# muyeon-jo/POI_recommendation_models

Hardware: NVIDIA B200
Metric: fullrank_eval_users_per_sec (higher is better)
Workload: dtype f16+e5m2-corrections/f32-accum

## Files before the change

include/nais_b200.h:

```cpp
#ifndef NAIS_B200_H_
#define NAIS_B200_H_

#include <stddef.h>
#include <stdint.h>

#ifdef __cplusplus
extern "C" {
#endif

#define NAIS_ABI_VERSION 2

#if defined(__GNUC__)
#define NAIS_API __attribute__((visibility("default")))
#else
#define NAIS_API
#endif

#define NAIS_DIST_NONE 0
#define NAIS_DIST_LATLON 1
#define NAIS_DIST_KM 2

#define NAIS_PREC_FP32 0
#define NAIS_PREC_TC_SPLIT 1
#define NAIS_PREC_TC_FAST 2
#define NAIS_PREC_TC_MIX 3
#define NAIS_PREC_TC_AUTO 4
#define NAIS_PREC_MASK 0xff
#define NAIS_PREC_FLAG_GENERIC 0x100
#define NAIS_PREC_FLAG_ONE_CTA 0x200

#define NAIS_PAIRS_AUTO 0
#define NAIS_PAIRS_FP32 1
#define NAIS_PAIRS_TC 2

#define NAIS_ERR_NULL -1
#define NAIS_ERR_SHAPE -2
#define NAIS_ERR_ALIGN -3
#define NAIS_ERR_WORKSPACE -4
#define NAIS_ERR_MODE -5
#define NAIS_ERR_ARCH -6
#define NAIS_ERR_INDEX -7

typedef void* nais_stream_t;

typedef struct NaisBranch {
  const float* hist_poi;
  const float* tgt_poi;
  const float* hist_reg;
  const float* tgt_reg;
  const float* w1;
  const float* b1;
  const float* w2;
  int32_t w_poi;
  int32_t w_reg;
} NaisBranch;

typedef struct NaisParams {
  NaisBranch branch[2];
  int32_t n_branch;
  int32_t hid;
  int32_t item_num;
  int32_t region_num;
  int32_t dist_mode;
  float dist_scale;
  const float* dist_w;
  const float* dist_b;
  const float* dist_embed;
  int32_t dist_buckets;
  float dist_bucket_km;
  float beta;
  float dropout_p;
  uint64_t dropout_seed;
  int32_t pairs_precision;
  int32_t reserved0;
} NaisParams;

typedef struct NaisPairs {
  const int64_t* hist;
  const int64_t* tgt;
  const int64_t* hreg;
  const int64_t* treg;
  const float* aux;
  int64_t B;
  int32_t H;
  int32_t n_seg;
  const int64_t* seg_offsets;
  const int64_t* row_offsets;
  const int64_t* seg_cell_offsets;
  const int32_t* tile_seg;
  const int64_t* tile_row0;
  int64_t n_tiles;
  int64_t n_cells;
  const float* hist_coords;
  const float* tgt_coords;
  float center_lat;
  float center_lon;
} NaisPairs;

typedef struct NaisGrads {
  float* hist_poi[2];
  float* tgt_poi[2];
  float* reg[2];
  float* w1[2];
  float* b1[2];
  float* w2[2];
  float* dist_w;
  float* dist_b;
  float* dist_embed;
  const int32_t* remap_hist_poi[2];
  const int32_t* remap_tgt_poi[2];
  const int32_t* remap_reg[2];
} NaisGrads;

typedef struct NaisCatalog {
  const int32_t* region;
  const float* coords;
  int64_t row_base;
  int64_t n_rows;
  float center_lat;
  float center_lon;
} NaisCatalog;

typedef struct NaisUsers {
  const int64_t* offsets;
  const int32_t* items;
  const int32_t* region;
  const float* coords;
  int32_t n_users;
} NaisUsers;

NAIS_API int nais_abi_version(void);
NAIS_API const char* nais_strerror(int code);
NAIS_API uint64_t nais_launch_count(void);

NAIS_API int nais_pairs_dispatch(const NaisParams* p, const NaisPairs* batch, int32_t* fwd_tc, int32_t* bwd_tc);

NAIS_API int nais_pairs_forward(const NaisParams* p, const NaisPairs* batch, float* score, float* row_sum, float* score_parts,
                       uint64_t* act_mask, nais_stream_t stream);

NAIS_API size_t nais_pairs_backward_workspace_bytes(const NaisParams* p, const NaisPairs* batch);
NAIS_API int nais_pairs_backward(const NaisParams* p, const NaisPairs* batch, const float* score_parts, const float* row_sum,
                        const uint64_t* act_mask, const float* dscore, const NaisGrads* grads, void* workspace,
                        size_t workspace_bytes, nais_stream_t stream);

NAIS_API int nais_pairs_forward_presort(const NaisParams* p, const NaisPairs* batch, const NaisGrads* grads, float* score,
                               float* row_sum, float* score_parts, uint64_t* act_mask, void* bwd_workspace,
                               size_t bwd_workspace_bytes, nais_stream_t stream);
NAIS_API int nais_pairs_backward_presorted(const NaisParams* p, const NaisPairs* batch, const float* score_parts, const float* row_sum,
                                  const uint64_t* act_mask, const float* dscore, const NaisGrads* grads, void* workspace,
                                  size_t workspace_bytes, nais_stream_t stream);

NAIS_API size_t nais_rows_adagrad_workspace_bytes(int64_t n, int32_t w);
NAIS_API int nais_rows_adagrad(const int32_t* keys, const float* rows, int64_t n, int32_t w, int32_t n_rows, float* grad_out,
                               float* param, float* sum, float lr, float eps, void* workspace, size_t workspace_bytes,
                               nais_stream_t stream);

NAIS_API int nais_sample_batch(const int64_t* seg_offsets, const int64_t* hist, int32_t n_seg, const int64_t* row_offsets,
                               int32_t num_ng, int32_t item_num, const int32_t* poi_region, const float* poi_coords, uint64_t seed,
                               int32_t max_hist, int64_t* tgt, float* label, int64_t* treg, float* tgt_coords, nais_stream_t stream);

typedef struct NaisAdagrad {
  float lr, eps;
  float* sum_hist_poi[2];
  float* sum_tgt_poi[2];
  float* sum_reg[2];
} NaisAdagrad;
NAIS_API int nais_pairs_backward_adagrad(const NaisParams* p, const NaisPairs* batch, const float* score_parts,
                                const float* row_sum, const uint64_t* act_mask, const float* dscore, const NaisGrads* grads,
                                const NaisAdagrad* opt, void* workspace, size_t workspace_bytes, nais_stream_t stream);

typedef struct NaisDenseAdagrad {
  float lr, eps;
  float* sum_w1;
  float* sum_b1;
  float* sum_w2;
  float* sum_dist_w;
  float* sum_dist_b;
  float* sum_region_w1;
  float* sum_region_b1;
  float* sum_region_w2;
  float* sum_dist_embed;
} NaisDenseAdagrad;
NAIS_API size_t nais_pairs_train_step_workspace_bytes(const NaisParams* p, const NaisPairs* batch);
NAIS_API int nais_pairs_train_step(const NaisParams* p, const NaisPairs* batch, const float* label, const float* row_weight,
                                   const NaisAdagrad* tables, const NaisDenseAdagrad* dense, float* loss, float* score,
                                   void* workspace, size_t workspace_bytes, nais_stream_t stream);

NAIS_API size_t nais_train_users_workspace_bytes(const NaisParams* p, int32_t max_hist, int32_t num_ng);
NAIS_API int nais_train_users(const NaisParams* p, const int64_t* host_indptr, int64_t n_rows, const int64_t* indices, const int64_t* entry_region,
                              const float* entry_coords, const int32_t* poi_region, const float* poi_coords, const int64_t* host_users,
                              int32_t n_users, int32_t num_ng, uint64_t seed, const NaisAdagrad* tables, const NaisDenseAdagrad* dense,
                              float* losses, void* workspace, size_t workspace_bytes, nais_stream_t stream);
NAIS_API int nais_train_users_centred(const NaisParams* p, const int64_t* host_indptr, int64_t n_rows, const int64_t* indices,
                                      const int64_t* entry_region, const float* entry_coords, const int32_t* poi_region,
                                      const float* poi_coords, const int64_t* host_users, int32_t n_users, int32_t num_ng, uint64_t seed,
                                      const NaisAdagrad* tables, const NaisDenseAdagrad* dense, float* losses, void* workspace,
                                      size_t workspace_bytes, float center_lat, float center_lon, nais_stream_t stream);
NAIS_API int nais_train_users_dropout(const NaisParams* p, const int64_t* host_indptr, int64_t n_rows, const int64_t* indices,
                                      const int64_t* entry_region, const float* entry_coords, const int32_t* poi_region,
                                      const float* poi_coords, const int64_t* host_users, int32_t n_users, int32_t num_ng, uint64_t seed,
                                      const NaisAdagrad* tables, const NaisDenseAdagrad* dense, float* losses, void* workspace,
                                      size_t workspace_bytes, float center_lat, float center_lon, const uint64_t* host_dropout_seeds,
                                      nais_stream_t stream);

NAIS_API size_t nais_fullrank_workspace_bytes(const NaisParams* p, int32_t n_users, int64_t nnz, int64_t poi_begin,
                                     int64_t poi_end, int32_t k, int32_t precision);
NAIS_API int nais_fullrank_topk(const NaisParams* p, const NaisCatalog* cat, const NaisUsers* users, int64_t poi_begin,
                       int64_t poi_end, int32_t k, int32_t exclude_history, int32_t precision, float* out_score, int32_t* out_id, void* workspace, size_t workspace_bytes,
                       nais_stream_t stream);

NAIS_API size_t nais_fullrank_plan_bytes(const NaisParams* p, int64_t poi_begin, int64_t poi_end, int32_t precision);
NAIS_API int nais_fullrank_prepare(const NaisParams* p, const NaisCatalog* cat, int64_t poi_begin, int64_t poi_end,
                                   int32_t precision, void* plan, size_t plan_bytes, nais_stream_t stream);
NAIS_API size_t nais_fullrank_planned_workspace_bytes(const NaisParams* p, int32_t n_users, int64_t nnz, int64_t poi_begin,
                                                      int64_t poi_end, int32_t k, int32_t precision);
NAIS_API int nais_fullrank_topk_planned(const NaisParams* p, const NaisCatalog* cat, const NaisUsers* users, int64_t poi_begin,
                                        int64_t poi_end, int32_t k, int32_t exclude_history, int32_t precision, const void* plan,
                                        size_t plan_bytes, uint64_t* out_keys, float* out_score, int32_t* out_id, void* workspace,
                                        size_t workspace_bytes, nais_stream_t stream);

NAIS_API int nais_topk_merge_keys(const uint64_t* in_keys, int64_t user_stride, int64_t list_stride, int32_t n_users,
                                  int32_t n_lists, int32_t k, uint64_t* out_keys, float* out_score, int32_t* out_id,
                                  nais_stream_t stream);

NAIS_API int nais_poll_bad_index(int32_t* host_flag, nais_stream_t stream);

NAIS_API int nais_topk_merge(const float* in_score, const int32_t* in_id, int32_t n_users, int32_t n_lists, int32_t k,
                    float* out_score, int32_t* out_id, nais_stream_t stream);

NAIS_API int nais_hits_at_k(const int32_t* rec, int32_t n_users, int32_t k_rec, const int64_t* pos_offsets,
                            const int32_t* pos_items, const int32_t* k_list, int32_t n_k, int32_t* hits,
                            nais_stream_t stream);

NAIS_API int nais_powerlaw_logscore(const NaisCatalog* cat, const NaisUsers* users, int64_t poi_begin, int64_t poi_end, float a,
                           float b, float* out_logg, nais_stream_t stream);

typedef struct NaisGeoMix {
  float a, b, alpha;
  const float* user_logmax;
} NaisGeoMix;
NAIS_API int nais_powerlaw_logmax(const NaisCatalog* cat, const NaisUsers* users, int64_t poi_begin, int64_t poi_end, float a,
                                  float b, int32_t exclude_history, float* out_logmax, nais_stream_t stream);
NAIS_API int nais_fullrank_topk_geo_planned(const NaisParams* p, const NaisCatalog* cat, const NaisUsers* users, int64_t poi_begin,
                                            int64_t poi_end, int32_t k, int32_t exclude_history, int32_t precision, const void* plan,
                                            size_t plan_bytes, const NaisGeoMix* geo, uint64_t* out_keys, float* out_score,
                                            int32_t* out_id, void* workspace, size_t workspace_bytes, nais_stream_t stream);

NAIS_API int nais_fullrank_scores(const NaisParams* p, const NaisCatalog* cat, const NaisUsers* users, int64_t poi_begin,
                         int64_t poi_end, int32_t precision, float* all_scores, void* workspace,
                         size_t workspace_bytes, nais_stream_t stream);

#ifdef __cplusplus
}
#endif
#endif
```

poi_recommendation_models_b200/_lib.py:

```python
from __future__ import annotations

import ctypes as C
import os

HERE = os.path.dirname(os.path.abspath(__file__))
LIB_PATH = os.path.join(HERE, "libnais_b200.so")

DIST_NONE, DIST_LATLON, DIST_KM = 0, 1, 2
PREC_FP32, PREC_TC_SPLIT, PREC_TC_FAST, PREC_TC_MIX, PREC_TC_AUTO = 0, 1, 2, 3, 4
PREC_FLAG_GENERIC = 0x100
PRECISIONS = {"fp32": PREC_FP32, "tc_split": PREC_TC_SPLIT, "tc_fast": PREC_TC_FAST, "tc_mix": PREC_TC_MIX,
              "tc_auto": PREC_TC_AUTO}
PREC_FLAG_ONE_CTA = 0x200
PRECISIONS.update({k + "_generic": v | PREC_FLAG_GENERIC for k, v in list(PRECISIONS.items()) if k != "fp32"})
PRECISIONS.update({k + "_onecta": v | PREC_FLAG_ONE_CTA for k, v in list(PRECISIONS.items()) if k in ("tc_auto", "tc_split", "tc_mix")})
PAIRS_PRECISIONS = {"auto": 0, "fp32": 1, "tc": 2}
ERR_INDEX = -7

ABI_VERSION = 2
c_float_p = C.c_void_p


class NaisBranch(C.Structure):
    _fields_ = [("hist_poi", C.c_void_p), ("tgt_poi", C.c_void_p), ("hist_reg", C.c_void_p), ("tgt_reg", C.c_void_p),
                ("w1", C.c_void_p), ("b1", C.c_void_p), ("w2", C.c_void_p), ("w_poi", C.c_int32), ("w_reg", C.c_int32)]


class NaisParams(C.Structure):
    _fields_ = [("branch", NaisBranch * 2), ("n_branch", C.c_int32), ("hid", C.c_int32), ("item_num", C.c_int32),
                ("region_num", C.c_int32), ("dist_mode", C.c_int32), ("dist_scale", C.c_float), ("dist_w", C.c_void_p),
                ("dist_b", C.c_void_p), ("dist_embed", C.c_void_p), ("dist_buckets", C.c_int32),
                ("dist_bucket_km", C.c_float), ("beta", C.c_float), ("dropout_p", C.c_float),
                ("dropout_seed", C.c_uint64), ("pairs_precision", C.c_int32), ("reserved0", C.c_int32)]


class NaisPairs(C.Structure):
    _fields_ = [("hist", C.c_void_p), ("tgt", C.c_void_p), ("hreg", C.c_void_p), ("treg", C.c_void_p),
                ("aux", C.c_void_p), ("B", C.c_int64), ("H", C.c_int32), ("n_seg", C.c_int32), ("seg_offsets", C.c_void_p),
                ("row_offsets", C.c_void_p), ("seg_cell_offsets", C.c_void_p), ("tile_seg", C.c_void_p), ("tile_row0", C.c_void_p),
                ("n_tiles", C.c_int64), ("n_cells", C.c_int64), ("hist_coords", C.c_void_p), ("tgt_coords", C.c_void_p),
                ("center_lat", C.c_float), ("center_lon", C.c_float)]


class NaisGrads(C.Structure):
    _fields_ = [("hist_poi", C.c_void_p * 2), ("tgt_poi", C.c_void_p * 2), ("reg", C.c_void_p * 2),
                ("w1", C.c_void_p * 2), ("b1", C.c_void_p * 2), ("w2", C.c_void_p * 2), ("dist_w", C.c_void_p),
                ("dist_b", C.c_void_p), ("dist_embed", C.c_void_p), ("remap_hist_poi", C.c_void_p * 2),
                ("remap_tgt_poi", C.c_void_p * 2), ("remap_reg", C.c_void_p * 2)]


class NaisAdagrad(C.Structure):
    _fields_ = [("lr", C.c_float), ("eps", C.c_float), ("sum_hist_poi", C.c_void_p * 2), ("sum_tgt_poi", C.c_void_p * 2),
                ("sum_reg", C.c_void_p * 2)]


class NaisDenseAdagrad(C.Structure):
    _fields_ = [("lr", C.c_float), ("eps", C.c_float), ("sum_w1", C.c_void_p), ("sum_b1", C.c_void_p), ("sum_w2", C.c_void_p),
                ("sum_dist_w", C.c_void_p), ("sum_dist_b", C.c_void_p), ("sum_region_w1", C.c_void_p), ("sum_region_b1", C.c_void_p),
                ("sum_region_w2", C.c_void_p), ("sum_dist_embed", C.c_void_p)]


class NaisCatalog(C.Structure):
    _fields_ = [("region", C.c_void_p), ("coords", C.c_void_p), ("row_base", C.c_int64), ("n_rows", C.c_int64),
                ("center_lat", C.c_float), ("center_lon", C.c_float)]


class NaisUsers(C.Structure):
    _fields_ = [("offsets", C.c_void_p), ("items", C.c_void_p), ("region", C.c_void_p), ("coords", C.c_void_p),
                ("n_users", C.c_int32)]


class NaisGeoMix(C.Structure):
    _fields_ = [("a", C.c_float), ("b", C.c_float), ("alpha", C.c_float), ("user_logmax", C.c_void_p)]


SYMBOLS = {
    "nais_abi_version": (C.c_int, []),
    "nais_strerror": (C.c_char_p, [C.c_int]),
    "nais_launch_count": (C.c_uint64, []),
    "nais_pairs_dispatch": (C.c_int, [C.POINTER(NaisParams), C.POINTER(NaisPairs), C.POINTER(C.c_int32), C.POINTER(C.c_int32)]),
    "nais_pairs_forward": (C.c_int, [C.POINTER(NaisParams), C.POINTER(NaisPairs), C.c_void_p, C.c_void_p, C.c_void_p,
                                     C.c_void_p, C.c_void_p]),
    "nais_pairs_backward_workspace_bytes": (C.c_size_t, [C.POINTER(NaisParams), C.POINTER(NaisPairs)]),
    "nais_pairs_train_step_workspace_bytes": (C.c_size_t, [C.POINTER(NaisParams), C.POINTER(NaisPairs)]),
    "nais_pairs_train_step": (C.c_int, [C.POINTER(NaisParams), C.POINTER(NaisPairs), C.c_void_p, C.c_void_p, C.POINTER(NaisAdagrad),
                                        C.POINTER(NaisDenseAdagrad), C.c_void_p, C.c_void_p, C.c_void_p, C.c_size_t, C.c_void_p]),
    "nais_train_users_workspace_bytes": (C.c_size_t, [C.POINTER(NaisParams), C.c_int32, C.c_int32]),
    "nais_train_users": (C.c_int, [C.POINTER(NaisParams), C.c_void_p, C.c_int64, C.c_void_p, C.c_void_p, C.c_void_p, C.c_void_p, C.c_void_p,
                                   C.c_void_p, C.c_int32, C.c_int32, C.c_uint64, C.POINTER(NaisAdagrad), C.POINTER(NaisDenseAdagrad),
                                   C.c_void_p, C.c_void_p, C.c_size_t, C.c_void_p]),
    "nais_train_users_centred": (C.c_int, [C.POINTER(NaisParams), C.c_void_p, C.c_int64, C.c_void_p, C.c_void_p, C.c_void_p, C.c_void_p,
                                           C.c_void_p, C.c_void_p, C.c_int32, C.c_int32, C.c_uint64, C.POINTER(NaisAdagrad),
                                           C.POINTER(NaisDenseAdagrad), C.c_void_p, C.c_void_p, C.c_size_t, C.c_float, C.c_float,
                                           C.c_void_p]),
    "nais_train_users_dropout": (C.c_int, [C.POINTER(NaisParams), C.c_void_p, C.c_int64, C.c_void_p, C.c_void_p, C.c_void_p, C.c_void_p,
                                           C.c_void_p, C.c_void_p, C.c_int32, C.c_int32, C.c_uint64, C.POINTER(NaisAdagrad),
                                           C.POINTER(NaisDenseAdagrad), C.c_void_p, C.c_void_p, C.c_size_t, C.c_float, C.c_float,
                                           C.c_void_p, C.c_void_p]),
    "nais_rows_adagrad_workspace_bytes": (C.c_size_t, [C.c_int64, C.c_int32]),
    "nais_rows_adagrad": (C.c_int, [C.c_void_p, C.c_void_p, C.c_int64, C.c_int32, C.c_int32, C.c_void_p, C.c_void_p, C.c_void_p,
                                    C.c_float, C.c_float, C.c_void_p, C.c_size_t, C.c_void_p]),
    "nais_sample_batch": (C.c_int, [C.c_void_p, C.c_void_p, C.c_int32, C.c_void_p, C.c_int32, C.c_int32, C.c_void_p, C.c_void_p,
                                    C.c_uint64, C.c_int32, C.c_void_p, C.c_void_p, C.c_void_p, C.c_void_p, C.c_void_p]),
    "nais_pairs_backward": (C.c_int, [C.POINTER(NaisParams), C.POINTER(NaisPairs), C.c_void_p, C.c_void_p, C.c_void_p, C.c_void_p,
                                      C.POINTER(NaisGrads), C.c_void_p, C.c_size_t, C.c_void_p]),
    "nais_pairs_forward_presort": (C.c_int, [C.POINTER(NaisParams), C.POINTER(NaisPairs), C.POINTER(NaisGrads), C.c_void_p, C.c_void_p,
                                             C.c_void_p, C.c_void_p, C.c_void_p, C.c_size_t, C.c_void_p]),
    "nais_pairs_backward_presorted": (C.c_int, [C.POINTER(NaisParams), C.POINTER(NaisPairs), C.c_void_p, C.c_void_p, C.c_void_p,
                                                C.c_void_p, C.POINTER(NaisGrads), C.c_void_p, C.c_size_t, C.c_void_p]),
    "nais_pairs_backward_adagrad": (C.c_int, [C.POINTER(NaisParams), C.POINTER(NaisPairs), C.c_void_p, C.c_void_p, C.c_void_p,
                                              C.c_void_p, C.POINTER(NaisGrads), C.POINTER(NaisAdagrad), C.c_void_p, C.c_size_t,
                                              C.c_void_p]),
    "nais_powerlaw_logscore": (C.c_int, [C.POINTER(NaisCatalog), C.POINTER(NaisUsers), C.c_int64, C.c_int64, C.c_float, C.c_float,
                                         C.c_void_p, C.c_void_p]),
    "nais_fullrank_workspace_bytes": (C.c_size_t, [C.POINTER(NaisParams), C.c_int32, C.c_int64, C.c_int64, C.c_int64,
                                                   C.c_int32, C.c_int32]),
    "nais_fullrank_topk": (C.c_int, [C.POINTER(NaisParams), C.POINTER(NaisCatalog), C.POINTER(NaisUsers), C.c_int64,
                                     C.c_int64, C.c_int32, C.c_int32, C.c_int32, C.c_void_p, C.c_void_p, C.c_void_p,
                                     C.c_size_t, C.c_void_p]),
    "nais_fullrank_scores": (C.c_int, [C.POINTER(NaisParams), C.POINTER(NaisCatalog), C.POINTER(NaisUsers), C.c_int64,
                                       C.c_int64, C.c_int32, C.c_void_p, C.c_void_p, C.c_size_t, C.c_void_p]),
    "nais_hits_at_k": (C.c_int, [C.c_void_p, C.c_int32, C.c_int32, C.c_void_p, C.c_void_p, C.c_void_p, C.c_int32, C.c_void_p,
                                 C.c_void_p]),
    "nais_topk_merge": (C.c_int, [C.c_void_p, C.c_void_p, C.c_int32, C.c_int32, C.c_int32, C.c_void_p, C.c_void_p,
                                  C.c_void_p]),
    "nais_fullrank_plan_bytes": (C.c_size_t, [C.POINTER(NaisParams), C.c_int64, C.c_int64, C.c_int32]),
    "nais_fullrank_prepare": (C.c_int, [C.POINTER(NaisParams), C.POINTER(NaisCatalog), C.c_int64, C.c_int64, C.c_int32,
                                        C.c_void_p, C.c_size_t, C.c_void_p]),
    "nais_fullrank_planned_workspace_bytes": (C.c_size_t, [C.POINTER(NaisParams), C.c_int32, C.c_int64, C.c_int64, C.c_int64,
                                                           C.c_int32, C.c_int32]),
    "nais_fullrank_topk_planned": (C.c_int, [C.POINTER(NaisParams), C.POINTER(NaisCatalog), C.POINTER(NaisUsers), C.c_int64,
                                             C.c_int64, C.c_int32, C.c_int32, C.c_int32, C.c_void_p, C.c_size_t, C.c_void_p,
                                             C.c_void_p, C.c_void_p, C.c_void_p, C.c_size_t, C.c_void_p]),
    "nais_powerlaw_logmax": (C.c_int, [C.POINTER(NaisCatalog), C.POINTER(NaisUsers), C.c_int64, C.c_int64, C.c_float, C.c_float,
                                       C.c_int32, C.c_void_p, C.c_void_p]),
    "nais_fullrank_topk_geo_planned": (C.c_int, [C.POINTER(NaisParams), C.POINTER(NaisCatalog), C.POINTER(NaisUsers), C.c_int64,
                                                 C.c_int64, C.c_int32, C.c_int32, C.c_int32, C.c_void_p, C.c_size_t,
                                                 C.POINTER(NaisGeoMix), C.c_void_p, C.c_void_p, C.c_void_p, C.c_void_p, C.c_size_t,
                                                 C.c_void_p]),
    "nais_topk_merge_keys": (C.c_int, [C.c_void_p, C.c_int64, C.c_int64, C.c_int32, C.c_int32, C.c_int32, C.c_void_p,
                                       C.c_void_p, C.c_void_p, C.c_void_p]),
    "nais_poll_bad_index": (C.c_int, [C.c_void_p, C.c_void_p]),
}

_lib = None


def load() -> C.CDLL:
    global _lib
    if _lib is not None:
        return _lib
    if not os.path.isfile(LIB_PATH):
        raise RuntimeError(f"{LIB_PATH} is missing: build it with `python poi_recommendation_models_b200/build_ext.py` "
                           "(nvcc, sm_100a).  There is no CPU / PyTorch fallback for the NAIS ops.")
    lib = C.CDLL(LIB_PATH)
    for name, (res, args) in SYMBOLS.items():
        fn = getattr(lib, name)
        fn.restype = res
        fn.argtypes = args
    if lib.nais_abi_version() != ABI_VERSION:
        raise RuntimeError("libnais_b200.so ABI version mismatch; rebuild")
    _lib = lib
    return lib


def check(rc: int, what: str) -> None:
    if rc != 0:
        msg = load().nais_strerror(rc).decode()
        raise RuntimeError(f"{what} failed ({rc}): {msg}")
```

poi_recommendation_models_b200/csrc/nais_capi.cu:

```cuda
#include <cstdio>

#include <cstring>
#include <mutex>

#include "nais_common.cuh"
#include "nais_pairs_tile.cuh"

namespace nais {
int launch_pairs_fwd(const NaisParams& p, const NaisPairs& b, float* score, float* row_sum, float* parts, cudaStream_t stream);
int launch_fullrank_fp32(const NaisParams& p, const NaisCatalog& cat, const NaisUsers& users, int64_t poi_begin,
                         int64_t poi_end, int k, int exclude, float* out_score, int32_t* out_id, float* all_scores,
                         void* ws, size_t ws_bytes, cudaStream_t stream, const GeoMixArgs* geo = nullptr);
int launch_topk_merge(const unsigned long long* in_keys, const float* in_score, const int32_t* in_id, int n_users,
                      int n_lists, int k, float* out_score, int32_t* out_id, cudaStream_t stream);
int launch_topk_merge_keys_multi(const unsigned long long* keys, unsigned long long* scratch, int64_t user_stride, int64_t list_stride,
                                 int n_users, int n_lists, int k, unsigned long long* out_keys, float* out_score, int32_t* out_id,
                                 cudaStream_t stream);
int merge_scratch_lists(int n_lists, int k);
int choose_splits(int n_users, int64_t range);
size_t pairs_bwd_workspace_bytes(const NaisParams& p, const NaisPairs& b);
int launch_pairs_bwd(const NaisParams& p, const NaisPairs& b, const float* score_parts, const float* row_sum,
                     const unsigned long long* act_mask, const float* dscore, const NaisGrads& g, const NaisAdagrad* opt, void* ws,
                     size_t ws_bytes, cudaStream_t stream, BwdPhase phase = BWD_ALL, const DenseAdagradLaunch* dense = nullptr);
bool pairs_tc_bwd_supported(const NaisParams& p, const NaisPairs& b);
size_t rows_adagrad_workspace_bytes(int64_t n, int w);
int launch_rows_adagrad(const int32_t* keys, const float* rows, int64_t n, int w, int n_rows, float* grad_out, float* param, float* sum,
                        float lr, float eps, void* ws, size_t ws_bytes, cudaStream_t stream);
size_t fullrank_tc_workspace_bytes(const NaisParams& p, int n_users, int64_t nnz, int64_t poi_begin, int64_t poi_end, int k,
                                   int precision);
int launch_fullrank_tc(const NaisParams& p, const NaisCatalog& cat, const NaisUsers& users, int64_t poi_begin,
                       int64_t poi_end, int k, int exclude, int precision, float* out_score, int32_t* out_id,
                       float* all_scores, void* ws, size_t ws_bytes, cudaStream_t stream);
bool tc_supported(const NaisParams& p, int precision);
size_t fullrank_tc_plan_bytes(const NaisParams& p, int64_t poi_begin, int64_t poi_end, int precision);
size_t fullrank_tc_call_workspace_bytes(const NaisParams& p, int n_users, int64_t nnz, int64_t poi_begin, int64_t poi_end, int k,
                                        int precision);
int fullrank_tc_prepare(const NaisParams& p, const NaisCatalog& cat, int64_t poi_begin, int64_t poi_end, int precision, void* plan,
                        size_t plan_bytes, cudaStream_t stream);
int fullrank_tc_run(const NaisParams& p, const NaisCatalog& cat, const NaisUsers& users, int64_t poi_begin, int64_t poi_end, int k,
                    int exclude, int precision, const void* plan, size_t plan_bytes, unsigned long long* out_keys, float* out_score,
                    int32_t* out_id, float* all_scores, void* ws, size_t ws_bytes, cudaStream_t stream,
                    const GeoMixArgs* geo = nullptr);
int launch_sample_batch(const int64_t* seg_offsets, const int64_t* hist, int n_seg, const int64_t* row_offsets, int num_ng, int item_num,
                        const int32_t* poi_region, const float* poi_coords, uint64_t seed, int max_hist, int64_t* tgt, float* label,
                        int64_t* treg, float* tgt_coords, cudaStream_t stream);
bool pairs_tc_supported(const NaisParams& p, const NaisPairs& b);
int launch_bce_dscore(const float* score, const float* label, const float* row_weight, int64_t B, float* dscore, float* loss,
                      cudaStream_t stream);
int launch_dense_adagrad(float* const* param, float* const* sum, const float* const* grad, const int* n, float lr, float eps,
                         cudaStream_t stream);
int launch_pairs_fwd_tc(const NaisParams& p, const NaisPairs& b, float* score, float* row_sum, float* parts,
                        unsigned long long* act_mask, cudaStream_t stream);
}

namespace nais {
unsigned long long g_launches = 0;
__device__ int g_bad_index = 0;
int* bad_index_flag() {
  int* ptr = nullptr;
  cudaGetSymbolAddress(reinterpret_cast<void**>(&ptr), g_bad_index);
  return ptr;
}
}
using namespace nais;

static bool aligned16(const void* p) { return (reinterpret_cast<uintptr_t>(p) & 15u) == 0; }

static int check_params(const NaisParams* p) {
  if (!p) return NAIS_ERR_NULL;
  if (p->n_branch < 1 || p->n_branch > 2) return NAIS_ERR_SHAPE;
  if (p->hid < 1 || p->hid > 1024 || p->item_num < 1) return NAIS_ERR_SHAPE;
  if (p->dist_mode < NAIS_DIST_NONE || p->dist_mode > NAIS_DIST_KM) return NAIS_ERR_MODE;
  for (int i = 0; i < p->n_branch; ++i) {
    const NaisBranch& b = p->branch[i];
    const int D = b.w_poi + b.w_reg;
    if (b.w_poi < 0 || b.w_reg < 0 || D < 4 || D > MAXD || (D & 3)) return NAIS_ERR_SHAPE;
    if (b.w_poi && (!b.hist_poi || !b.tgt_poi)) return NAIS_ERR_NULL;
    if (b.w_reg && (!b.hist_reg || !b.tgt_reg || p->region_num < 1)) return NAIS_ERR_NULL;
    if (!b.w1 || !b.b1 || !b.w2) return NAIS_ERR_NULL;
  }
  if (p->dist_mode == NAIS_DIST_LATLON && (!p->dist_w || !p->dist_b)) return NAIS_ERR_NULL;
  if (p->dist_mode == NAIS_DIST_KM && (!p->dist_embed || p->dist_buckets < 1)) return NAIS_ERR_NULL;
  if (p->dist_mode == NAIS_DIST_KM && p->dist_buckets != 1) return NAIS_ERR_MODE;
  if (p->pairs_precision < NAIS_PAIRS_AUTO || p->pairs_precision > NAIS_PAIRS_TC) return NAIS_ERR_MODE;
  return 0;
}

static int check_pairs(const NaisParams* p, const NaisPairs* b) {
  if (!b) return NAIS_ERR_NULL;
  const bool seg = b->seg_offsets != nullptr;
  if (b->B < 0 || (!seg && b->H < 1)) return NAIS_ERR_SHAPE;
  if (b->B == 0) return 0;
  if (!b->hist || !b->tgt) return NAIS_ERR_NULL;
  bool need_reg = false;
  for (int i = 0; i < p->n_branch; ++i) need_reg |= p->branch[i].w_reg > 0;
  if (need_reg && (!b->hreg || !b->treg)) return NAIS_ERR_NULL;
  if (seg) {
    if (b->n_seg < 1 || b->n_tiles < 0 || b->n_cells < 0) return NAIS_ERR_SHAPE;
    if (!b->row_offsets || !b->seg_cell_offsets || (b->n_tiles && (!b->tile_seg || !b->tile_row0))) return NAIS_ERR_NULL;
    if (b->aux) return NAIS_ERR_MODE;
    if (p->dropout_p > 0.f && p->n_branch != 1) return NAIS_ERR_MODE;
    if (p->dist_mode != NAIS_DIST_NONE && (!b->hist_coords || !b->tgt_coords)) return NAIS_ERR_NULL;
    return 0;
  }
  if (p->dist_mode != NAIS_DIST_NONE && !b->aux) return NAIS_ERR_NULL;
  return 0;
}

static size_t fp32_workspace_bytes(int n_users, int64_t poi_begin, int64_t poi_end, int k) {
  const int s = choose_splits(n_users, poi_end - poi_begin);
  return 1024 + (size_t)n_users * 8 + (s > 1 ? (size_t)n_users * s * k * sizeof(unsigned long long) : 0);
}

__global__ void pack_keys_kernel(const float* __restrict__ s, const int32_t* __restrict__ id, size_t n, unsigned long long* keys) {
  const size_t i = blockIdx.x * (size_t)blockDim.x + threadIdx.x;
  if (i < n) keys[i] = id[i] >= 0 ? make_key(s[i], id[i]) : 0ull;
}

__global__ void fill_empty_topk_kernel(float* s, int32_t* id, size_t n) {
  const size_t i = blockIdx.x * (size_t)blockDim.x + threadIdx.x;
  if (i < n) {
    s[i] = -INFINITY;
    id[i] = -1;
  }
}

template <bool kHist>
__device__ __forceinline__ float powerlaw_logg_block(const NaisCatalog& cat, const NaisUsers& users, int u, int64_t j, bool valid,
                                                     float ln_a, float b, bool* in_hist) {
  __shared__ float s_la[256], s_lo[256], s_cos[256];
  __shared__ int s_id[kHist ? 256 : 1];
  const int64_t hb = users.offsets[u];
  const int H = (int)(users.offsets[u + 1] - hb);
  float cla = 0.f, clo = 0.f, ccos = 1.f;
  if (valid) {
    cla = __ldg(cat.coords + 2 * (j - cat.row_base));
    clo = __ldg(cat.coords + 2 * (j - cat.row_base) + 1);
    ccos = cosf((cat.center_lat + cla) * 0.017453292519943295f);
  }
  float acc = 0.f;
  bool seen = false;
  for (int h0 = 0; h0 < H; h0 += 256) {
    __syncthreads();
    if (h0 + (int)threadIdx.x < H) {
      const float la = __ldg(users.coords + 2 * (hb + h0 + threadIdx.x)), lo = __ldg(users.coords + 2 * (hb + h0 + threadIdx.x) + 1);
      s_la[threadIdx.x] = la;
      s_lo[threadIdx.x] = lo;
      s_cos[threadIdx.x] = cosf((cat.center_lat + la) * 0.017453292519943295f);
      if constexpr (kHist) s_id[threadIdx.x] = __ldg(users.items + hb + h0 + threadIdx.x);
    }
    __syncthreads();
    const int n = min(256, H - h0);
    for (int i = 0; i < n; ++i) {
      acc += powerlaw_log_term(dist_km_f(cla, clo, s_la[i], s_lo[i], ccos, s_cos[i]), ln_a, b);
      if constexpr (kHist) seen = seen || (int64_t)s_id[i] == j;
    }
  }
  if (in_hist) *in_hist = seen;
  return acc;
}

__global__ void powerlaw_logscore_kernel(NaisCatalog cat, NaisUsers users, int64_t poi_begin, int64_t poi_end, float ln_a, float b,
                                         float* __restrict__ out) {
  const int u = blockIdx.x;
  const int64_t j = poi_begin + (int64_t)blockIdx.y * blockDim.x + threadIdx.x;
  const bool valid = j < poi_end;
  const float acc = powerlaw_logg_block<false>(cat, users, u, j, valid, ln_a, b, nullptr);
  if (valid) out[(size_t)u * (poi_end - poi_begin) + (j - poi_begin)] = acc;
}

__device__ __forceinline__ void atomic_max_float(float* addr, float v) {
  if (v != v) return;
  if (__float_as_int(v) >= 0) atomicMax(reinterpret_cast<int*>(addr), __float_as_int(v));
  else atomicMin(reinterpret_cast<unsigned*>(addr), __float_as_uint(v));
}

__global__ void fill_float_kernel(float* out, int n, float v) {
  const int i = blockIdx.x * blockDim.x + threadIdx.x;
  if (i < n) out[i] = v;
}

__global__ void powerlaw_logmax_kernel(NaisCatalog cat, NaisUsers users, int64_t poi_begin, int64_t poi_end, float ln_a, float b,
                                       int exclude, float* __restrict__ out) {
  __shared__ float s_max[8];
  const int u = blockIdx.x;
  float m = -INFINITY;
  for (int64_t j0 = poi_begin + (int64_t)blockIdx.y * blockDim.x; j0 < poi_end; j0 += (int64_t)gridDim.y * blockDim.x) {
    const int64_t j = j0 + threadIdx.x;
    const bool valid = j < poi_end;
    bool in_hist = false;
    const float acc = exclude ? powerlaw_logg_block<true>(cat, users, u, j, valid, ln_a, b, &in_hist)
                              : powerlaw_logg_block<false>(cat, users, u, j, valid, ln_a, b, nullptr);
    if (valid && !in_hist) m = fmaxf(m, acc);
  }
#pragma unroll
  for (int o = 16; o > 0; o >>= 1) m = fmaxf(m, __shfl_xor_sync(0xffffffffu, m, o));
  if ((threadIdx.x & 31) == 0) s_max[threadIdx.x >> 5] = m;
  __syncthreads();
  if (threadIdx.x == 0) {
    for (int w = 1; w < (int)(blockDim.x >> 5); ++w) m = fmaxf(m, s_max[w]);
    if (m > -INFINITY) atomic_max_float(out + u, m);
  }
}

__global__ void hits_at_k_kernel(const int32_t* __restrict__ rec, int n_users, int k_rec, const int64_t* __restrict__ po,
                                 const int32_t* __restrict__ pi, const int32_t* __restrict__ k_list, int n_k, int32_t* hits) {
  const int u = (blockIdx.x * blockDim.x + threadIdx.x) >> 5, lane = threadIdx.x & 31;
  if (u >= n_users) return;
  const int64_t p0 = po[u], p1 = po[u + 1];
  for (int ki = 0; ki < n_k; ++ki) {
    const int k = min(k_list[ki], k_rec);
    int cnt = 0;
    for (int r = lane; r < k; r += 32) {
      const int id = rec[(size_t)u * k_rec + r];
      if (id < 0) continue;
      bool dup = false;
      for (int q = 0; q < r && !dup; ++q) dup = rec[(size_t)u * k_rec + q] == id;
      if (dup) continue;
      bool hit = false;
      for (int64_t q = p0; q < p1 && !hit; ++q) hit = pi[q] == id;
      cnt += hit ? 1 : 0;
    }
#pragma unroll
    for (int o = 16; o > 0; o >>= 1) cnt += __shfl_xor_sync(0xffffffffu, cnt, o);
    if (lane == 0) hits[(size_t)u * n_k + ki] = cnt;
  }
}

extern "C" {

int nais_abi_version(void) { return NAIS_ABI_VERSION; }
uint64_t nais_launch_count(void) { return __atomic_load_n(&nais::g_launches, __ATOMIC_RELAXED); }

const char* nais_strerror(int code) {
  switch (code) {
    case 0: return "ok";
    case NAIS_ERR_NULL: return "nais: required pointer is NULL";
    case NAIS_ERR_SHAPE: return "nais: unsupported or inconsistent dimension";
    case NAIS_ERR_ALIGN: return "nais: pointer or row width not 16-byte aligned";
    case NAIS_ERR_WORKSPACE: return "nais: workspace too small";
    case NAIS_ERR_MODE: return "nais: unknown mode or unsupported flag combination";
    case NAIS_ERR_ARCH: return "nais: tensor path needs an sm_100 device";
    case NAIS_ERR_INDEX: return "nais: index out of range in a POI / region id tensor";
    default: break;
  }
  if (code > 0) return cudaGetErrorString(static_cast<cudaError_t>(code));
  return "nais: unknown error";
}

static bool device_is_sm100() {
  return device_info().major == 10;
}

static int choose_pairs_fwd(const NaisParams& p, const NaisPairs& b, bool* tc) {
  const bool tc_ok = pairs_tc_supported(p, b) && device_is_sm100();
  if (p.pairs_precision == NAIS_PAIRS_TC && !tc_ok) return NAIS_ERR_SHAPE;
  *tc = p.pairs_precision != NAIS_PAIRS_FP32 && tc_ok;
  return 0;
}

static int launch_chosen_fwd(bool tc, const NaisParams& p, const NaisPairs& b, float* score, float* row_sum, float* parts,
                             unsigned long long* act_mask, cudaStream_t stream) {
  return tc ? launch_pairs_fwd_tc(p, b, score, row_sum, parts, act_mask, stream) : launch_pairs_fwd(p, b, score, row_sum, parts, stream);
}

size_t nais_rows_adagrad_workspace_bytes(int64_t n, int32_t w) {
  if (n < 0 || w < 1 || w > 128) return 0;
  return rows_adagrad_workspace_bytes(n, w);
}

int nais_rows_adagrad(const int32_t* keys, const float* rows, int64_t n, int32_t w, int32_t n_rows, float* grad_out, float* param,
                      float* sum, float lr, float eps, void* workspace, size_t workspace_bytes, nais_stream_t stream) {
  if (n < 0 || w < 1 || w > 128 || n_rows < 1) return NAIS_ERR_SHAPE;
  if (n == 0) return 0;
  if (!keys || !rows || !workspace || (sum ? !param : !grad_out)) return NAIS_ERR_NULL;
  if (sum && (!(lr >= 0.f) || !(eps >= 0.f))) return NAIS_ERR_MODE;
  if (!aligned16(workspace)) return NAIS_ERR_ALIGN;
  return launch_rows_adagrad(keys, rows, n, w, n_rows, grad_out, param, sum, lr, eps, workspace, workspace_bytes,
                             static_cast<cudaStream_t>(stream));
}

int nais_sample_batch(const int64_t* seg_offsets, const int64_t* hist, int32_t n_seg, const int64_t* row_offsets, int32_t num_ng,
                      int32_t item_num, const int32_t* poi_region, const float* poi_coords, uint64_t seed, int32_t max_hist,
                      int64_t* tgt, float* label, int64_t* treg, float* tgt_coords, nais_stream_t stream) {
  if (n_seg < 0 || num_ng < 0 || item_num < 1 || max_hist < 0) return NAIS_ERR_SHAPE;
  if (n_seg == 0) return 0;
  if (!seg_offsets || !hist || !row_offsets || !tgt || !label) return NAIS_ERR_NULL;
  if ((treg && !poi_region) || (tgt_coords && !poi_coords)) return NAIS_ERR_NULL;
  if ((int64_t)max_hist * (num_ng + 1) >= item_num) return NAIS_ERR_SHAPE;
  return launch_sample_batch(seg_offsets, hist, n_seg, row_offsets, num_ng, item_num, poi_region, poi_coords, seed, max_hist, tgt,
                             label, treg, tgt_coords, static_cast<cudaStream_t>(stream));
}

int nais_pairs_dispatch(const NaisParams* p, const NaisPairs* batch, int32_t* fwd_tc, int32_t* bwd_tc) {
  int rc = check_params(p);
  if (rc) return rc;
  if (!batch || !fwd_tc || !bwd_tc) return NAIS_ERR_NULL;
  if (batch->B < 0 || (!batch->seg_offsets && batch->H < 1)) return NAIS_ERR_SHAPE;
  NaisPairs b = *batch;
  if (b.B == 0) b.B = 1;
  bool f_tc = false;
  rc = choose_pairs_fwd(*p, b, &f_tc);
  if (rc) return rc;
  *fwd_tc = f_tc ? 1 : 0;
  *bwd_tc = (p->pairs_precision != NAIS_PAIRS_FP32 && pairs_tc_bwd_supported(*p, b)) ? 1 : 0;
  return 0;
}

int nais_pairs_forward(const NaisParams* p, const NaisPairs* batch, float* score, float* row_sum, float* score_parts,
                       uint64_t* act_mask, nais_stream_t stream) {
  int rc = check_params(p);
  if (rc) return rc;
  rc = check_pairs(p, batch);
  if (rc) return rc;
  if (batch->B && !score) return NAIS_ERR_NULL;
  if (batch->B == 0) return 0;
  bool tc = false;
  rc = choose_pairs_fwd(*p, *batch, &tc);
  if (rc) return rc;
  return launch_chosen_fwd(tc, *p, *batch, score, row_sum, score_parts, reinterpret_cast<unsigned long long*>(act_mask),
                           static_cast<cudaStream_t>(stream));
}

size_t nais_pairs_backward_workspace_bytes(const NaisParams* p, const NaisPairs* batch) {
  if (check_params(p) || !batch || batch->B < 0 || (!batch->seg_offsets && batch->H < 1)) return 0;
  return pairs_bwd_workspace_bytes(*p, *batch);
}

int nais_pairs_backward(const NaisParams* p, const NaisPairs* batch, const float* score_parts, const float* row_sum,
                        const uint64_t* act_mask, const float* dscore, const NaisGrads* grads, void* workspace,
                        size_t workspace_bytes, nais_stream_t stream) {
  int rc = check_params(p);
  if (rc) return rc;
  rc = check_pairs(p, batch);
  if (rc) return rc;
  if (!grads) return NAIS_ERR_NULL;
  if (batch->B == 0) return 0;
  if (!score_parts || !row_sum || !dscore || !workspace) return NAIS_ERR_NULL;
  if (!aligned16(workspace)) return NAIS_ERR_ALIGN;
  if (workspace_bytes < pairs_bwd_workspace_bytes(*p, *batch)) return NAIS_ERR_WORKSPACE;
  return launch_pairs_bwd(*p, *batch, score_parts, row_sum, reinterpret_cast<const unsigned long long*>(act_mask), dscore, *grads,
                          nullptr, workspace, workspace_bytes, static_cast<cudaStream_t>(stream));
}

int nais_pairs_forward_presort(const NaisParams* p, const NaisPairs* batch, const NaisGrads* grads, float* score, float* row_sum,
                               float* score_parts, uint64_t* act_mask, void* bwd_workspace, size_t bwd_workspace_bytes,
                               nais_stream_t stream) {
  int rc = check_params(p);
  if (rc) return rc;
  rc = check_pairs(p, batch);
  if (rc) return rc;
  if (!grads) return NAIS_ERR_NULL;
  if (p->n_branch != 1) return NAIS_ERR_MODE;
  if (batch->B && !score) return NAIS_ERR_NULL;
  if (batch->B == 0) return 0;
  if (!bwd_workspace) return NAIS_ERR_NULL;
  if (!aligned16(bwd_workspace)) return NAIS_ERR_ALIGN;
  if (bwd_workspace_bytes < pairs_bwd_workspace_bytes(*p, *batch)) return NAIS_ERR_WORKSPACE;
  bool tc = false;
  rc = choose_pairs_fwd(*p, *batch, &tc);
  if (rc) return rc;
  cudaStream_t st = static_cast<cudaStream_t>(stream);
  rc = launch_pairs_bwd(*p, *batch, nullptr, nullptr, nullptr, nullptr, *grads, nullptr, bwd_workspace, bwd_workspace_bytes, st, BWD_SORTS);
  if (rc) return rc;
  rc = launch_chosen_fwd(tc, *p, *batch, score, row_sum, score_parts, reinterpret_cast<unsigned long long*>(act_mask), st);
  const int rj = launch_pairs_bwd(*p, *batch, nullptr, nullptr, nullptr, nullptr, *grads, nullptr, bwd_workspace, bwd_workspace_bytes, st,
                                  BWD_JOIN_SORTS);
  return rc ? rc : rj;
}

int nais_pairs_backward_presorted(const NaisParams* p, const NaisPairs* batch, const float* score_parts, const float* row_sum,
                                  const uint64_t* act_mask, const float* dscore, const NaisGrads* grads, void* workspace,
                                  size_t workspace_bytes, nais_stream_t stream) {
  int rc = check_params(p);
  if (rc) return rc;
  rc = check_pairs(p, batch);
  if (rc) return rc;
  if (!grads) return NAIS_ERR_NULL;
  if (p->n_branch != 1) return NAIS_ERR_MODE;
  if (batch->B == 0) return 0;
  if (!score_parts || !row_sum || !dscore || !workspace) return NAIS_ERR_NULL;
  if (!aligned16(workspace)) return NAIS_ERR_ALIGN;
  if (workspace_bytes < pairs_bwd_workspace_bytes(*p, *batch)) return NAIS_ERR_WORKSPACE;
  return launch_pairs_bwd(*p, *batch, score_parts, row_sum, reinterpret_cast<const unsigned long long*>(act_mask), dscore, *grads,
                          nullptr, workspace, workspace_bytes, static_cast<cudaStream_t>(stream), BWD_AFTER_JOIN);
}

int nais_pairs_backward_adagrad(const NaisParams* p, const NaisPairs* batch, const float* score_parts, const float* row_sum,
                                const uint64_t* act_mask, const float* dscore, const NaisGrads* grads, const NaisAdagrad* opt,
                                void* workspace, size_t workspace_bytes, nais_stream_t stream) {
  int rc = check_params(p);
  if (rc) return rc;
  rc = check_pairs(p, batch);
  if (rc) return rc;
  if (!grads || !opt) return NAIS_ERR_NULL;
  if (!pairs_fused_layout(*p)) return NAIS_ERR_MODE;
  if (!(opt->lr >= 0.f) || !(opt->eps >= 0.f)) return NAIS_ERR_MODE;
  if (batch->B == 0) return 0;
  if (!score_parts || !row_sum || !dscore || !workspace) return NAIS_ERR_NULL;
  if (!aligned16(workspace)) return NAIS_ERR_ALIGN;
  if (workspace_bytes < pairs_bwd_workspace_bytes(*p, *batch)) return NAIS_ERR_WORKSPACE;
  return launch_pairs_bwd(*p, *batch, score_parts, row_sum, reinterpret_cast<const unsigned long long*>(act_mask), dscore, *grads,
                          opt, workspace, workspace_bytes, static_cast<cudaStream_t>(stream));
}

namespace {
inline size_t ts_al(size_t x) { return (x + 255) / 256 * 256; }
struct TrainStepLayout {
  size_t score, row_sum, parts, dscore, mask, gw1[2], gb1[2], gw2[2], gdw, gdb, gde, bwd, total;
};
TrainStepLayout train_step_layout(const NaisParams& p, const NaisPairs& b) {
  TrainStepLayout L;
  const int64_t B = b.B, cells = pairs_n_cells(b);
  const int lanes = p.dist_mode == NAIS_DIST_LATLON ? 2 : 0;
  size_t o = 0;
  L.score = o, o += ts_al((size_t)B * 4);
  L.row_sum = o, o += ts_al((size_t)p.n_branch * B * 4);
  L.parts = o, o += ts_al((size_t)p.n_branch * B * 4);
  L.dscore = o, o += ts_al((size_t)B * 4);
  L.mask = o, o += ts_al((size_t)cells * 8);
  for (int bi = 0; bi < 2; ++bi) {
    const NaisBranch& br = p.branch[bi];
    const int ldw = br.w_poi + br.w_reg + lanes;
    const bool on = bi < p.n_branch;
    L.gw1[bi] = o, o += on ? ts_al((size_t)p.hid * ldw * 4) : 0;
    L.gb1[bi] = o, o += on ? ts_al((size_t)p.hid * 4) : 0;
    L.gw2[bi] = o, o += on ? ts_al((size_t)p.hid * 4) : 0;
  }
  L.gdw = o, o += 256;
  L.gdb = o, o += 256;
  L.gde = o, o += p.dist_mode == NAIS_DIST_KM ? ts_al((size_t)MAXD * 4) : 0;
  L.bwd = o, o += ts_al(pairs_bwd_workspace_bytes(p, b));
  L.total = o;
  return L;
}
}

size_t nais_pairs_train_step_workspace_bytes(const NaisParams* p, const NaisPairs* batch) {
  if (check_params(p) || !batch || batch->B < 0 || (!batch->seg_offsets && batch->H < 1)) return 0;
  if (!pairs_fused_layout(*p)) return 0;
  return train_step_layout(*p, *batch).total;
}

static int check_train_state(const NaisParams* p, const NaisAdagrad* tables, const NaisDenseAdagrad* dense) {
  if (!tables || !dense) return NAIS_ERR_NULL;
  if (!pairs_fused_layout(*p)) return NAIS_ERR_MODE;
  const bool two = pairs_disentangled(*p);
  if (p->n_branch == 1 && p->dist_mode == NAIS_DIST_KM) return NAIS_ERR_MODE;
  if (!(tables->lr >= 0.f) || !(tables->eps >= 0.f) || !(dense->lr >= 0.f) || !(dense->eps >= 0.f)) return NAIS_ERR_MODE;
  if (!dense->sum_w1 || !dense->sum_b1 || !dense->sum_w2) return NAIS_ERR_NULL;
  if (p->dist_mode == NAIS_DIST_LATLON && (!dense->sum_dist_w || !dense->sum_dist_b)) return NAIS_ERR_NULL;
  if (two && (!dense->sum_region_w1 || !dense->sum_region_b1 || !dense->sum_region_w2)) return NAIS_ERR_NULL;
  if (two && p->dist_mode == NAIS_DIST_KM && !dense->sum_dist_embed) return NAIS_ERR_NULL;
  return 0;
}

enum StepPart { STEP_ALL = 0, STEP_SORTS = 1, STEP_AFTER_SORTS = 2 };

static int train_step_impl(const NaisParams* p, const NaisPairs* batch, const float* label, const float* row_weight,
                           const NaisAdagrad* tables, const NaisDenseAdagrad* dense, float* loss, float* score_out, void* workspace,
                           size_t workspace_bytes, cudaStream_t st, StepPart part = STEP_ALL);

int nais_pairs_train_step(const NaisParams* p, const NaisPairs* batch, const float* label, const float* row_weight,
                          const NaisAdagrad* tables, const NaisDenseAdagrad* dense, float* loss, float* score_out, void* workspace,
                          size_t workspace_bytes, nais_stream_t stream) {
  int rc = check_params(p);
  if (rc) return rc;
  rc = check_pairs(p, batch);
  if (rc) return rc;
  if (!loss) return NAIS_ERR_NULL;
  rc = check_train_state(p, tables, dense);
  if (rc) return rc;
  if (batch->B == 0) return 0;
  if (!label || !workspace) return NAIS_ERR_NULL;
  if (!aligned16(workspace)) return NAIS_ERR_ALIGN;
  return train_step_impl(p, batch, label, row_weight, tables, dense, loss, score_out, workspace, workspace_bytes,
                         static_cast<cudaStream_t>(stream));
}

static int train_step_impl(const NaisParams* p, const NaisPairs* batch, const float* label, const float* row_weight,
                           const NaisAdagrad* tables, const NaisDenseAdagrad* dense, float* loss, float* score_out, void* workspace,
                           size_t workspace_bytes, cudaStream_t st, StepPart part) {
  int rc;
  const TrainStepLayout L = train_step_layout(*p, *batch);
  if (workspace_bytes < L.total) return NAIS_ERR_WORKSPACE;
  char* base = reinterpret_cast<char*>(workspace);
  auto F = [&](size_t off) { return reinterpret_cast<float*>(base + off); };
  NaisGrads g;
  memset(&g, 0, sizeof(g));
  for (int bi = 0; bi < p->n_branch; ++bi) {
    g.w1[bi] = F(L.gw1[bi]);
    g.b1[bi] = F(L.gb1[bi]);
    g.w2[bi] = F(L.gw2[bi]);
  }
  if (p->dist_mode == NAIS_DIST_LATLON) {
    g.dist_w = F(L.gdw);
    g.dist_b = F(L.gdb);
  }
  if (p->dist_mode == NAIS_DIST_KM) g.dist_embed = F(L.gde);
  if (part != STEP_AFTER_SORTS) {
    rc = launch_pairs_bwd(*p, *batch, nullptr, nullptr, nullptr, nullptr, g, tables, base + L.bwd, workspace_bytes - L.bwd, st, BWD_SORTS);
    if (rc) return rc;
  }
  if (part == STEP_SORTS)
    return launch_pairs_bwd(*p, *batch, nullptr, nullptr, nullptr, nullptr, g, tables, base + L.bwd, workspace_bytes - L.bwd, st,
                            BWD_JOIN_SORTS);
  bool fwd_tc = false;
  rc = choose_pairs_fwd(*p, *batch, &fwd_tc);
  if (rc) return rc;
  unsigned long long* mask = (fwd_tc && p->hid <= 64) ? reinterpret_cast<unsigned long long*>(base + L.mask) : nullptr;
  rc = launch_chosen_fwd(fwd_tc, *p, *batch, F(L.score), F(L.row_sum), F(L.parts), mask, st);
  if (rc) return rc;
  if (score_out) {
    cudaError_t e = cudaMemcpyAsync(score_out, F(L.score), (size_t)batch->B * 4, cudaMemcpyDeviceToDevice, st);
    if (e != cudaSuccess) return (int)e;
  }
  rc = launch_bce_dscore(F(L.score), label, row_weight, batch->B, F(L.dscore), loss, st);
  if (rc) return rc;
  const NaisBranch& br = p->branch[0];
  const int lanes = p->dist_mode == NAIS_DIST_LATLON ? 2 : 0, ldw = br.w_poi + br.w_reg + lanes;
  DenseAdagradLaunch da[2] = {{{const_cast<float*>(br.w1), const_cast<float*>(br.b1), const_cast<float*>(br.w2),
                                lanes ? const_cast<float*>(p->dist_w) : nullptr, lanes ? const_cast<float*>(p->dist_b) : nullptr},
                               {dense->sum_w1, dense->sum_b1, dense->sum_w2, dense->sum_dist_w, dense->sum_dist_b},
                               {g.w1[0], g.b1[0], g.w2[0], g.dist_w, g.dist_b},
                               {p->hid * ldw, p->hid, p->hid, 4, 2},
                               dense->lr, dense->eps}};
  if (p->n_branch == 2) {
    const NaisBranch& r = p->branch[1];
    const bool km = p->dist_mode == NAIS_DIST_KM;
    da[1] = {{const_cast<float*>(r.w1), const_cast<float*>(r.b1), const_cast<float*>(r.w2), km ? const_cast<float*>(p->dist_embed) : nullptr,
              nullptr},
             {dense->sum_region_w1, dense->sum_region_b1, dense->sum_region_w2, dense->sum_dist_embed, nullptr},
             {g.w1[1], g.b1[1], g.w2[1], g.dist_embed, nullptr},
             {p->hid * (r.w_poi + r.w_reg), p->hid, p->hid, r.w_poi + r.w_reg, 0},
             dense->lr, dense->eps};
  }
  return launch_pairs_bwd(*p, *batch, F(L.parts), F(L.row_sum), mask, F(L.dscore), g, tables, base + L.bwd, workspace_bytes - L.bwd, st,
                          part == STEP_AFTER_SORTS ? BWD_AFTER_JOIN : BWD_AFTER_SORTS, da);
}

namespace {
__global__ void single_segment_kernel(int H, int R, int rpt, int n_tiles, int64_t* seg_offsets, int64_t* row_offsets, int64_t* cell_offsets,
                                      int32_t* tile_seg, int64_t* tile_row0) {
  const int i = blockIdx.x * blockDim.x + threadIdx.x;
  if (i == 0) {
    seg_offsets[0] = 0, seg_offsets[1] = H;
    row_offsets[0] = 0, row_offsets[1] = R;
    cell_offsets[0] = 0, cell_offsets[1] = (int64_t)R * H;
  }
  if (i < n_tiles) {
    tile_seg[i] = 0;
    tile_row0[i] = (int64_t)i * rpt;
  }
}
struct UsersLayout {
  size_t seg, row, cell, tseg, trow, tgt, label, treg, tco, step, total;
};
inline int host_rows_per_tile(int H) {
  int r = H <= 128 ? 128 / (H > 0 ? H : 1) : 1;
  return r > 16 ? 16 : r;
}
NaisPairs max_user_batch(int max_hist, int num_ng) {
  NaisPairs b;
  memset(&b, 0, sizeof(b));
  static const int64_t dummy[2] = {0, 0};
  b.seg_offsets = dummy;
  b.n_seg = 1;
  b.B = (int64_t)max_hist * (num_ng + 1);
  b.n_cells = b.B * max_hist;
  b.n_tiles = b.B;
  return b;
}
UsersLayout users_layout(const NaisParams& p, int max_hist, int num_ng) {
  UsersLayout L;
  const NaisPairs b = max_user_batch(max_hist, num_ng);
  size_t o = 0;
  L.seg = o, o += 256;
  L.row = o, o += 256;
  L.cell = o, o += 256;
  L.tseg = o, o += ts_al((size_t)b.n_tiles * 4);
  L.trow = o, o += ts_al((size_t)b.n_tiles * 8);
  L.tgt = o, o += ts_al((size_t)b.B * 8);
  L.label = o, o += ts_al((size_t)b.B * 4);
  L.treg = o, o += ts_al((size_t)b.B * 8);
  L.tco = o, o += ts_al((size_t)b.B * 8);
  L.step = o, o += train_step_layout(p, b).total;
  L.total = o;
  return L;
}

std::mutex g_prep_mu;
cudaStream_t prep_stream() {
  static cudaStream_t pool[64] = {};
  int dev = 0;
  if (cudaGetDevice(&dev) != cudaSuccess || dev < 0 || dev >= 64) return nullptr;
  std::lock_guard<std::mutex> lock(g_prep_mu);
  if (!pool[dev] && cudaStreamCreateWithFlags(&pool[dev], cudaStreamNonBlocking) != cudaSuccess) pool[dev] = nullptr;
  return pool[dev];
}
}

size_t nais_train_users_workspace_bytes(const NaisParams* p, int32_t max_hist, int32_t num_ng) {
  if (check_params(p) || !pairs_fused_layout(*p) || max_hist < 1 || num_ng < 0) return 0;
  return 2 * users_layout(*p, max_hist, num_ng).total;
}

int nais_train_users(const NaisParams* p, const int64_t* host_indptr, int64_t n_rows, const int64_t* indices, const int64_t* entry_region,
                     const float* entry_coords, const int32_t* poi_region, const float* poi_coords, const int64_t* host_users,
                     int32_t n_users, int32_t num_ng, uint64_t seed, const NaisAdagrad* tables, const NaisDenseAdagrad* dense, float* losses,
                     void* workspace, size_t workspace_bytes, nais_stream_t stream) {
  return nais_train_users_centred(p, host_indptr, n_rows, indices, entry_region, entry_coords, poi_region, poi_coords, host_users, n_users,
                                  num_ng, seed, tables, dense, losses, workspace, workspace_bytes, 0.f, 0.f, stream);
}

int nais_train_users_centred(const NaisParams* p, const int64_t* host_indptr, int64_t n_rows, const int64_t* indices,
                             const int64_t* entry_region, const float* entry_coords, const int32_t* poi_region, const float* poi_coords,
                             const int64_t* host_users, int32_t n_users, int32_t num_ng, uint64_t seed, const NaisAdagrad* tables,
                             const NaisDenseAdagrad* dense, float* losses, void* workspace, size_t workspace_bytes, float center_lat,
                             float center_lon, nais_stream_t stream) {
  if (p && p->dropout_p > 0.f) return NAIS_ERR_MODE;
  return nais_train_users_dropout(p, host_indptr, n_rows, indices, entry_region, entry_coords, poi_region, poi_coords, host_users, n_users,
                                  num_ng, seed, tables, dense, losses, workspace, workspace_bytes, center_lat, center_lon, nullptr, stream);
}

int nais_train_users_dropout(const NaisParams* p, const int64_t* host_indptr, int64_t n_rows, const int64_t* indices,
                             const int64_t* entry_region, const float* entry_coords, const int32_t* poi_region, const float* poi_coords,
                             const int64_t* host_users, int32_t n_users, int32_t num_ng, uint64_t seed, const NaisAdagrad* tables,
                             const NaisDenseAdagrad* dense, float* losses, void* workspace, size_t workspace_bytes, float center_lat,
                             float center_lon, const uint64_t* host_dropout_seeds, nais_stream_t stream) {
  int rc = check_params(p);
  if (rc) return rc;
  rc = check_train_state(p, tables, dense);
  if (rc) return rc;
  if (n_users < 0 || num_ng < 0) return NAIS_ERR_SHAPE;
  if (p->dropout_p > 0.f && !host_dropout_seeds) return NAIS_ERR_NULL;
  if (n_users == 0) return 0;
  if (!host_indptr || !indices || !host_users || !losses || !workspace) return NAIS_ERR_NULL;
  bool need_reg = false;
  for (int i = 0; i < p->n_branch; ++i) need_reg |= p->branch[i].w_reg > 0;
  const bool need_co = p->dist_mode != NAIS_DIST_NONE;
  if ((need_reg && (!entry_region || !poi_region)) || (need_co && (!entry_coords || !poi_coords))) return NAIS_ERR_NULL;
  if (!aligned16(workspace)) return NAIS_ERR_ALIGN;
  int max_hist = 0;
  for (int i = 0; i < n_users; ++i) {
    const int64_t u = host_users[i];
    if (u < 0 || u >= n_rows) return NAIS_ERR_SHAPE;
    const int64_t H = host_indptr[u + 1] - host_indptr[u];
    if (H < 0 || H > 0x7fffffff / (num_ng + 2)) return NAIS_ERR_SHAPE;
    if ((int)H > max_hist) max_hist = (int)H;
  }
  if (max_hist == 0) return (int)cudaMemsetAsync(losses, 0, (size_t)n_users * 4, static_cast<cudaStream_t>(stream));
  if ((int64_t)max_hist * (num_ng + 1) >= p->item_num) return NAIS_ERR_SHAPE;
  const UsersLayout L = users_layout(*p, max_hist, num_ng);
  if (workspace_bytes < 2 * L.total) return NAIS_ERR_WORKSPACE;
  cudaStream_t st = static_cast<cudaStream_t>(stream);
  cudaStream_t ps = prep_stream();
  if (!ps) return (int)cudaErrorUnknown;
  cudaEvent_t prepared[2] = {nullptr, nullptr}, stepped[2] = {nullptr, nullptr}, begin = nullptr;
  bool ev_ok = cudaEventCreateWithFlags(&begin, cudaEventDisableTiming) == cudaSuccess;
  for (int i = 0; i < 2 && ev_ok; ++i)
    ev_ok = cudaEventCreateWithFlags(&prepared[i], cudaEventDisableTiming) == cudaSuccess &&
            cudaEventCreateWithFlags(&stepped[i], cudaEventDisableTiming) == cudaSuccess;
  auto release = [&]() {
    if (begin) cudaEventDestroy(begin);
    for (int i = 0; i < 2; ++i) {
      if (prepared[i]) cudaEventDestroy(prepared[i]);
      if (stepped[i]) cudaEventDestroy(stepped[i]);
    }
  };
  if (!ev_ok) {
    release();
    return (int)cudaErrorUnknown;
  }
  auto bail = [&](int code) {
    if (cudaEventRecord(begin, ps) == cudaSuccess) cudaStreamWaitEvent(st, begin, 0);
    release();
    return code;
  };
  struct UserBatch {
    NaisPairs b;
    const float* label;
    char* step;
  };
  auto buffers = [&](int i, int slot, UserBatch& ub) {
    char* base = reinterpret_cast<char*>(workspace) + (size_t)slot * L.total;
    auto I64 = [&](size_t off) { return reinterpret_cast<int64_t*>(base + off); };
    const int64_t u = host_users[i], a = host_indptr[u];
    const int H = (int)(host_indptr[u + 1] - a);
    const int R = H * (num_ng + 1), rpt = host_rows_per_tile(H), n_tiles = (R + rpt - 1) / rpt;
    NaisPairs& b = ub.b;
    memset(&b, 0, sizeof(b));
    b.hist = indices + a;
    b.tgt = I64(L.tgt);
    b.hreg = need_reg ? entry_region + a : nullptr;
    b.treg = need_reg ? I64(L.treg) : nullptr;
    b.B = R;
    b.n_seg = 1;
    b.seg_offsets = I64(L.seg);
    b.row_offsets = I64(L.row);
    b.seg_cell_offsets = I64(L.cell);
    b.tile_seg = reinterpret_cast<int32_t*>(base + L.tseg);
    b.tile_row0 = I64(L.trow);
    b.n_tiles = n_tiles;
    b.n_cells = (int64_t)R * H;
    b.hist_coords = need_co ? entry_coords + 2 * a : nullptr;
    b.tgt_coords = need_co ? reinterpret_cast<float*>(base + L.tco) : nullptr;
    b.center_lat = center_lat;
    b.center_lon = center_lon;
    ub.label = reinterpret_cast<float*>(base + L.label);
    ub.step = base + L.step;
  };
  auto prepare = [&](int i, int slot) -> int {
    UserBatch ub;
    buffers(i, slot, ub);
    const int64_t u = host_users[i], a = host_indptr[u];
    const int H = (int)(host_indptr[u + 1] - a);
    char* base = reinterpret_cast<char*>(workspace) + (size_t)slot * L.total;
    single_segment_kernel<<<((int)ub.b.n_tiles + 255) / 256, 256, 0, ps>>>(
        H, (int)ub.b.B, host_rows_per_tile(H), (int)ub.b.n_tiles, const_cast<int64_t*>(ub.b.seg_offsets), const_cast<int64_t*>(ub.b.row_offsets),
        const_cast<int64_t*>(ub.b.seg_cell_offsets), const_cast<int32_t*>(ub.b.tile_seg), const_cast<int64_t*>(ub.b.tile_row0));
    NAIS_COUNT_LAUNCH(1);
    int r = launch_sample_batch(ub.b.seg_offsets, indices + a, 1, ub.b.row_offsets, num_ng, p->item_num, need_reg ? poi_region : nullptr,
                                need_co ? poi_coords : nullptr, seed + (uint64_t)u, H, const_cast<int64_t*>(ub.b.tgt),
                                reinterpret_cast<float*>(base + L.label), need_reg ? const_cast<int64_t*>(ub.b.treg) : nullptr,
                                need_co ? const_cast<float*>(ub.b.tgt_coords) : nullptr, ps);
    if (r) return r;
    return train_step_impl(p, &ub.b, ub.label, nullptr, tables, dense, nullptr, nullptr, ub.step, L.total - L.step, ps, STEP_SORTS);
  };
  int next = 0;
  auto advance = [&](int from) {
    while (from < n_users && host_indptr[host_users[from] + 1] == host_indptr[host_users[from]]) ++from;
    return from;
  };
  for (int i = 0; i < n_users; ++i)
    if (host_indptr[host_users[i] + 1] == host_indptr[host_users[i]]) {
      cudaError_t e = cudaMemsetAsync(losses + i, 0, 4, st);
      if (e != cudaSuccess) return bail((int)e);
    }
  if (cudaEventRecord(begin, st) != cudaSuccess || cudaStreamWaitEvent(ps, begin, 0) != cudaSuccess) return bail((int)cudaErrorUnknown);
  next = advance(0);
  int slot = 0;
  if (next < n_users) {
    rc = prepare(next, slot);
    if (rc) return bail(rc);
    cudaEventRecord(prepared[slot], ps);
  }
  int done = 0;
  while (next < n_users) {
    const int cur = next, cur_slot = slot;
    next = advance(cur + 1);
    slot ^= 1;
    if (next < n_users) {
      if (done >= 1) cudaStreamWaitEvent(ps, stepped[slot], 0);
      rc = prepare(next, slot);
      if (rc) return bail(rc);
      cudaEventRecord(prepared[slot], ps);
    }
    UserBatch ub;
    buffers(cur, cur_slot, ub);
    NaisParams pu = *p;
    if (p->dropout_p > 0.f) pu.dropout_seed = host_dropout_seeds[cur];
    cudaStreamWaitEvent(st, prepared[cur_slot], 0);
    rc = train_step_impl(&pu, &ub.b, ub.label, nullptr, tables, dense, losses + cur, nullptr, ub.step, L.total - L.step, st, STEP_AFTER_SORTS);
    if (rc) return bail(rc);
    cudaEventRecord(stepped[cur_slot], st);
    ++done;
  }
  cudaError_t e = cudaGetLastError();
  release();
  return e == cudaSuccess ? 0 : (int)e;
}

static int check_fullrank(const NaisParams* p, const NaisCatalog* cat, const NaisUsers* users, int64_t poi_begin,
                          int64_t poi_end, int precision) {
  int rc = check_params(p);
  if (rc) return rc;
  if (!cat || !users) return NAIS_ERR_NULL;
  if (users->n_users < 0 || poi_begin < 0 || poi_end < poi_begin || poi_end > p->item_num) return NAIS_ERR_SHAPE;
  if (poi_begin < cat->row_base || poi_end > cat->row_base + cat->n_rows) return NAIS_ERR_SHAPE;
  if (users->n_users && (!users->offsets || !users->items)) return NAIS_ERR_NULL;
  bool need_reg = false;
  for (int i = 0; i < p->n_branch; ++i) need_reg |= p->branch[i].w_reg > 0;
  const bool work = users->n_users > 0 && poi_end > poi_begin;
  if (work && need_reg && (!cat->region || !users->region)) return NAIS_ERR_NULL;
  if (work && p->dist_mode != NAIS_DIST_NONE && (!cat->coords || !users->coords)) return NAIS_ERR_NULL;
  const int prec = precision & NAIS_PREC_MASK;
  if (precision & ~(NAIS_PREC_MASK | NAIS_PREC_FLAG_GENERIC | NAIS_PREC_FLAG_ONE_CTA)) return NAIS_ERR_MODE;
  if (prec < NAIS_PREC_FP32 || prec > NAIS_PREC_TC_AUTO) return NAIS_ERR_MODE;
  if (prec != NAIS_PREC_FP32 && !tc_supported(*p, precision)) return NAIS_ERR_SHAPE;
  return 0;
}

size_t nais_fullrank_workspace_bytes(const NaisParams* p, int32_t n_users, int64_t nnz, int64_t poi_begin,
                                     int64_t poi_end, int32_t k, int32_t precision) {
  if (check_params(p) || n_users < 0 || poi_end < poi_begin || k < 1) return 0;
  if ((precision & NAIS_PREC_MASK) != NAIS_PREC_FP32) return fullrank_tc_workspace_bytes(*p, n_users, nnz, poi_begin, poi_end, k, precision);
  return fp32_workspace_bytes(n_users, poi_begin, poi_end, k);
}

size_t nais_fullrank_plan_bytes(const NaisParams* p, int64_t poi_begin, int64_t poi_end, int32_t precision) {
  if (check_params(p) || poi_end < poi_begin || (precision & NAIS_PREC_MASK) == NAIS_PREC_FP32) return 0;
  return fullrank_tc_plan_bytes(*p, poi_begin, poi_end, precision);
}

size_t nais_fullrank_planned_workspace_bytes(const NaisParams* p, int32_t n_users, int64_t nnz, int64_t poi_begin, int64_t poi_end,
                                             int32_t k, int32_t precision) {
  if (check_params(p) || n_users < 0 || poi_end < poi_begin || k < 1) return 0;
  if ((precision & NAIS_PREC_MASK) != NAIS_PREC_FP32)
    return fullrank_tc_call_workspace_bytes(*p, n_users, nnz, poi_begin, poi_end, k, precision) + 1024 + (size_t)n_users * 8;
  return fp32_workspace_bytes(n_users, poi_begin, poi_end, k) + (size_t)n_users * k * 12 + 512;
}

int nais_fullrank_prepare(const NaisParams* p, const NaisCatalog* cat, int64_t poi_begin, int64_t poi_end, int32_t precision,
                          void* plan, size_t plan_bytes, nais_stream_t stream) {
  NaisUsers none = {};
  int rc = check_fullrank(p, cat, &none, poi_begin, poi_end, precision);
  if (rc) return rc;
  if ((precision & NAIS_PREC_MASK) == NAIS_PREC_FP32 || poi_end == poi_begin) return 0;
  if (!plan) return NAIS_ERR_NULL;
  if (!aligned16(plan)) return NAIS_ERR_ALIGN;
  const NaisBranch& br = p->branch[0];
  if (br.w_reg > 0 && !cat->region) return NAIS_ERR_NULL;
  return fullrank_tc_prepare(*p, *cat, poi_begin, poi_end, precision, plan, plan_bytes, static_cast<cudaStream_t>(stream));
}

static int check_geo(const NaisCatalog* cat, const NaisUsers* users, int64_t poi_begin, int64_t poi_end, const NaisGeoMix* geo) {
  if (!geo) return NAIS_ERR_NULL;
  if (!(geo->a > 0.f) || !isfinite(geo->a) || !isfinite(geo->b) || !isfinite(geo->alpha)) return NAIS_ERR_MODE;
  if (users->n_users > 0 && poi_end > poi_begin && (!cat->coords || !users->coords || !geo->user_logmax)) return NAIS_ERR_NULL;
  return 0;
}

static int fullrank_topk_planned_impl(const NaisParams* p, const NaisCatalog* cat, const NaisUsers* users, int64_t poi_begin,
                                      int64_t poi_end, int32_t k, int32_t exclude_history, int32_t precision, const void* plan,
                                      size_t plan_bytes, const NaisGeoMix* geo, uint64_t* out_keys, float* out_score, int32_t* out_id,
                                      void* workspace, size_t workspace_bytes, nais_stream_t stream) {
  int rc = check_fullrank(p, cat, users, poi_begin, poi_end, precision);
  if (rc) return rc;
  if (k < 1 || k > KCAP) return NAIS_ERR_SHAPE;
  if (geo && (rc = check_geo(cat, users, poi_begin, poi_end, geo))) return rc;
  if (users->n_users == 0) return 0;
  if ((!out_score) != (!out_id) || (!out_score && !out_keys) || !workspace) return NAIS_ERR_NULL;
  if (!aligned16(workspace)) return NAIS_ERR_ALIGN;
  GeoMixArgs gm = {};
  if (geo) gm = GeoMixArgs{logf(geo->a), geo->b, geo->alpha, geo->user_logmax};
  const GeoMixArgs* gp = geo ? &gm : nullptr;
  cudaStream_t st = static_cast<cudaStream_t>(stream);
  unsigned long long* keys = reinterpret_cast<unsigned long long*>(out_keys);
  const size_t n = (size_t)users->n_users * k;
  if (poi_end == poi_begin) {
    if (out_score) {
      fill_empty_topk_kernel<<<(unsigned)((n + 255) / 256), 256, 0, st>>>(out_score, out_id, n);
      NAIS_COUNT_LAUNCH(1);
    }
    if (keys) {
      cudaError_t e = cudaMemsetAsync(keys, 0, n * 8, st);
      if (e != cudaSuccess) return (int)e;
    }
    return (int)cudaGetLastError();
  }
  if ((precision & NAIS_PREC_MASK) != NAIS_PREC_FP32)
    return fullrank_tc_run(*p, *cat, *users, poi_begin, poi_end, k, exclude_history, precision, plan, plan_bytes, keys, out_score,
                           out_id, nullptr, workspace, workspace_bytes, st, gp);
  float* sc = out_score;
  int32_t* id = out_id;
  char* rest = reinterpret_cast<char*>(workspace);
  size_t rest_bytes = workspace_bytes;
  if (!sc) {
    const size_t head = (n * 8 + 255) & ~size_t(255);
    if (workspace_bytes < head) return NAIS_ERR_WORKSPACE;
    sc = reinterpret_cast<float*>(workspace);
    id = reinterpret_cast<int32_t*>(sc + n);
    rest += head;
    rest_bytes -= head;
  }
  rc = launch_fullrank_fp32(*p, *cat, *users, poi_begin, poi_end, k, exclude_history, sc, id, nullptr, rest, rest_bytes, st, gp);
  if (rc || !keys) return rc;
  pack_keys_kernel<<<(unsigned)((n + 255) / 256), 256, 0, st>>>(sc, id, n, keys);
  NAIS_COUNT_LAUNCH(1);
  return (int)cudaGetLastError();
}

int nais_fullrank_topk_planned(const NaisParams* p, const NaisCatalog* cat, const NaisUsers* users, int64_t poi_begin,
                               int64_t poi_end, int32_t k, int32_t exclude_history, int32_t precision, const void* plan,
                               size_t plan_bytes, uint64_t* out_keys, float* out_score, int32_t* out_id, void* workspace,
                               size_t workspace_bytes, nais_stream_t stream) {
  return fullrank_topk_planned_impl(p, cat, users, poi_begin, poi_end, k, exclude_history, precision, plan, plan_bytes, nullptr, out_keys,
                                    out_score, out_id, workspace, workspace_bytes, stream);
}

int nais_fullrank_topk_geo_planned(const NaisParams* p, const NaisCatalog* cat, const NaisUsers* users, int64_t poi_begin,
                                   int64_t poi_end, int32_t k, int32_t exclude_history, int32_t precision, const void* plan,
                                   size_t plan_bytes, const NaisGeoMix* geo, uint64_t* out_keys, float* out_score, int32_t* out_id,
                                   void* workspace, size_t workspace_bytes, nais_stream_t stream) {
  if (!geo) return NAIS_ERR_NULL;
  return fullrank_topk_planned_impl(p, cat, users, poi_begin, poi_end, k, exclude_history, precision, plan, plan_bytes, geo, out_keys,
                                    out_score, out_id, workspace, workspace_bytes, stream);
}

int nais_topk_merge_keys(const uint64_t* in_keys, int64_t user_stride, int64_t list_stride, int32_t n_users, int32_t n_lists,
                         int32_t k, uint64_t* out_keys, float* out_score, int32_t* out_id, nais_stream_t stream) {
  if (n_users < 0 || n_lists < 1 || k < 1 || k > KCAP || user_stride < k || list_stride < k) return NAIS_ERR_SHAPE;
  if (n_users == 0) return 0;
  if (!in_keys || (!out_score) != (!out_id) || (!out_score && !out_keys)) return NAIS_ERR_NULL;
  if (merge_scratch_lists(n_lists, k) != 0) return NAIS_ERR_SHAPE;
  return launch_topk_merge_keys_multi(reinterpret_cast<const unsigned long long*>(in_keys), nullptr, user_stride, list_stride, n_users,
                                      n_lists, k, reinterpret_cast<unsigned long long*>(out_keys), out_score, out_id,
                                      static_cast<cudaStream_t>(stream));
}

int nais_poll_bad_index(int32_t* host_flag, nais_stream_t stream) {
  if (!host_flag) return NAIS_ERR_NULL;
  cudaStream_t st = static_cast<cudaStream_t>(stream);
  int* flag = bad_index_flag();
  if (!flag) return (int)cudaGetLastError();
  cudaError_t e = cudaMemcpyAsync(host_flag, flag, sizeof(int), cudaMemcpyDeviceToHost, st);
  if (e != cudaSuccess) return (int)e;
  e = cudaMemsetAsync(flag, 0, sizeof(int), st);
  return (int)e;
}

int nais_fullrank_topk(const NaisParams* p, const NaisCatalog* cat, const NaisUsers* users, int64_t poi_begin,
                       int64_t poi_end, int32_t k, int32_t exclude_history, int32_t precision, float* out_score,
                       int32_t* out_id, void* workspace, size_t workspace_bytes, nais_stream_t stream) {
  int rc = check_fullrank(p, cat, users, poi_begin, poi_end, precision);
  if (rc) return rc;
  if (k < 1 || k > KCAP) return NAIS_ERR_SHAPE;
  if (users->n_users && (!out_score || !out_id || !workspace)) return NAIS_ERR_NULL;
  if (!aligned16(workspace)) return NAIS_ERR_ALIGN;
  cudaStream_t st = static_cast<cudaStream_t>(stream);
  if (users->n_users && poi_end == poi_begin) {
    const size_t n = (size_t)users->n_users * k;
    fill_empty_topk_kernel<<<(unsigned)((n + 255) / 256), 256, 0, st>>>(out_score, out_id, n);
    NAIS_COUNT_LAUNCH(1);
    return (int)cudaGetLastError();
  }
  if ((precision & NAIS_PREC_MASK) == NAIS_PREC_FP32)
    return launch_fullrank_fp32(*p, *cat, *users, poi_begin, poi_end, k, exclude_history, out_score, out_id, nullptr,
                                workspace, workspace_bytes, st);
  return launch_fullrank_tc(*p, *cat, *users, poi_begin, poi_end, k, exclude_history, precision, out_score, out_id,
                            nullptr, workspace, workspace_bytes, st);
}

int nais_fullrank_scores(const NaisParams* p, const NaisCatalog* cat, const NaisUsers* users, int64_t poi_begin,
                         int64_t poi_end, int32_t precision, float* all_scores, void* workspace,
                         size_t workspace_bytes, nais_stream_t stream) {
  int rc = check_fullrank(p, cat, users, poi_begin, poi_end, precision);
  if (rc) return rc;
  if (users->n_users && (!all_scores || !workspace)) return NAIS_ERR_NULL;
  if (!aligned16(workspace)) return NAIS_ERR_ALIGN;
  const size_t head = ((size_t)users->n_users * (sizeof(float) + sizeof(int32_t)) + 255) & ~size_t(255);
  if (workspace_bytes < head) return NAIS_ERR_WORKSPACE;
  float* sc = reinterpret_cast<float*>(workspace);
  int32_t* id = reinterpret_cast<int32_t*>(sc + users->n_users);
  char* rest = reinterpret_cast<char*>(workspace) + head;
  cudaStream_t st = static_cast<cudaStream_t>(stream);
  if ((precision & NAIS_PREC_MASK) == NAIS_PREC_FP32)
    return launch_fullrank_fp32(*p, *cat, *users, poi_begin, poi_end, 1, 0, sc, id, all_scores, rest,
                                workspace_bytes - head, st);
  return launch_fullrank_tc(*p, *cat, *users, poi_begin, poi_end, 1, 0, precision, sc, id, all_scores, rest,
                            workspace_bytes - head, st);
}

int nais_hits_at_k(const int32_t* rec, int32_t n_users, int32_t k_rec, const int64_t* pos_offsets, const int32_t* pos_items,
                   const int32_t* k_list, int32_t n_k, int32_t* hits, nais_stream_t stream) {
  if (n_users < 0 || k_rec < 1 || n_k < 1) return NAIS_ERR_SHAPE;
  if (n_users == 0) return 0;
  if (!rec || !pos_offsets || !k_list || !hits) return NAIS_ERR_NULL;
  const int64_t threads = (int64_t)n_users * 32;
  hits_at_k_kernel<<<(unsigned)((threads + 255) / 256), 256, 0, static_cast<cudaStream_t>(stream)>>>(rec, n_users, k_rec, pos_offsets,
                                                                                                  pos_items, k_list, n_k, hits);
  NAIS_COUNT_LAUNCH(1);
  return (int)cudaGetLastError();
}

int nais_powerlaw_logscore(const NaisCatalog* cat, const NaisUsers* users, int64_t poi_begin, int64_t poi_end, float a, float b,
                           float* out_logg, nais_stream_t stream) {
  if (!cat || !users) return NAIS_ERR_NULL;
  if (users->n_users < 0 || poi_begin < cat->row_base || poi_end < poi_begin || poi_end > cat->row_base + cat->n_rows) return NAIS_ERR_SHAPE;
  if (!(a > 0.f)) return NAIS_ERR_MODE;
  if (users->n_users == 0 || poi_end == poi_begin) return 0;
  if (!cat->coords || !users->coords || !users->offsets || !out_logg) return NAIS_ERR_NULL;
  if ((poi_end - poi_begin + 255) / 256 > 65535) return NAIS_ERR_SHAPE;
  dim3 grid((unsigned)users->n_users, (unsigned)((poi_end - poi_begin + 255) / 256));
  powerlaw_logscore_kernel<<<grid, 256, 0, static_cast<cudaStream_t>(stream)>>>(*cat, *users, poi_begin, poi_end, logf(a), b, out_logg);
  NAIS_COUNT_LAUNCH(1);
  return (int)cudaGetLastError();
}

int nais_powerlaw_logmax(const NaisCatalog* cat, const NaisUsers* users, int64_t poi_begin, int64_t poi_end, float a, float b,
                         int32_t exclude_history, float* out_logmax, nais_stream_t stream) {
  if (!cat || !users) return NAIS_ERR_NULL;
  if (users->n_users < 0 || poi_begin < cat->row_base || poi_end < poi_begin || poi_end > cat->row_base + cat->n_rows) return NAIS_ERR_SHAPE;
  if (!(a > 0.f) || !isfinite(a) || !isfinite(b)) return NAIS_ERR_MODE;
  if (users->n_users == 0) return 0;
  if (!out_logmax || !users->offsets) return NAIS_ERR_NULL;
  if (poi_end > poi_begin && (!cat->coords || !users->coords || (exclude_history && !users->items))) return NAIS_ERR_NULL;
  cudaStream_t st = static_cast<cudaStream_t>(stream);
  fill_float_kernel<<<(users->n_users + 255) / 256, 256, 0, st>>>(out_logmax, users->n_users, -INFINITY);
  NAIS_COUNT_LAUNCH(1);
  if (poi_end > poi_begin) {
    const int64_t blocks = (poi_end - poi_begin + 255) / 256;
    dim3 grid((unsigned)users->n_users, (unsigned)(blocks < 64 ? blocks : 64));
    powerlaw_logmax_kernel<<<grid, 256, 0, st>>>(*cat, *users, poi_begin, poi_end, logf(a), b, exclude_history ? 1 : 0, out_logmax);
    NAIS_COUNT_LAUNCH(1);
  }
  return (int)cudaGetLastError();
}

int nais_topk_merge(const float* in_score, const int32_t* in_id, int32_t n_users, int32_t n_lists, int32_t k,
                    float* out_score, int32_t* out_id, nais_stream_t stream) {
  if (n_users < 0 || n_lists < 1 || k < 1) return NAIS_ERR_SHAPE;
  if (n_users == 0) return 0;
  if (!in_score || !in_id || !out_score || !out_id) return NAIS_ERR_NULL;
  return launch_topk_merge(nullptr, in_score, in_id, n_users, n_lists, k, out_score, out_id,
                           static_cast<cudaStream_t>(stream));
}

}
```

poi_recommendation_models_b200/csrc/nais_tc.cu:

```cuda
#include <cuda_fp16.h>
#include <cuda_fp8.h>

#include <type_traits>

#include "nais_common.cuh"
#include "umma.cuh"

namespace nais {

using namespace umma;

namespace tc {

constexpr int TM = 128;
constexpr int NBUF = 3;
constexpr int ACC_STRIDE = 160;
constexpr int TPC = 3;
constexpr int EPI_WARPS = 16;
constexpr int EPI_THREADS = EPI_WARPS * 32;
constexpr int ARRIVE_WARPS = 8;
constexpr int THREADS = (EPI_WARPS + 2) * 32;
constexpr int MAX_STAGES = 4;
constexpr int SORTN = 512;
constexpr int HMETA = 512;

struct Geo {
  int D, hid, lanes, split;
  int pair;
  int km;
  int mix;
  int kx;
  int hsplit;
  int hch;
  int aux0;
  int nrow;
  int tpc;
  int stages;
  int kp;
  int kc_part;
  int part_bytes, part_last_bytes, stage_bytes;
  int a_plane, a_tile;
  int b_hi, b_lo, b_chunk;
  int smem_bytes;
};

__host__ __device__ inline int pad16(int x) { return (x + 15) / 16 * 16; }

__host__ inline bool make_geo(const NaisParams& p, int precision, Geo& g) {
  if (p.n_branch != 1) return false;
  const NaisBranch& br = p.branch[0];
  g.D = br.w_poi + br.w_reg;
  g.hsplit = p.hid == 256 ? 2 : 1;
  g.hid = p.hid / g.hsplit;
  g.lanes = p.dist_mode == NAIS_DIST_LATLON ? 2 : 0;
  g.split = precision == NAIS_PREC_TC_SPLIT;
  g.mix = precision == NAIS_PREC_TC_MIX;
  g.pair = 0;
  g.km = p.dist_mode == NAIS_DIST_KM ? 1 : 0;
  if (g.km && p.dist_buckets != 1) return false;
  if (precision == NAIS_PREC_TC_AUTO) {
    g.mix = g.D % 32 == 0;
    g.split = !g.mix;
  }
  if (g.mix && g.D % 32) return false;
  if (g.D % 16 || g.D < 16 || g.D > 256 || (g.D > 64 && g.D % 32) || g.hid % 16 || g.hid < 16 || g.hid > 128) return false;
  g.hch = g.hid <= 64 ? 2 : 1;
  if (g.hch == 1 && g.hid % 32) return false;
  g.kx = g.D / 8;
  g.aux0 = g.hch * g.hid;
  g.nrow = pad16(g.aux0 + 2 * g.hch);
  if (g.nrow < g.aux0 + 16) g.nrow = g.aux0 + 16;
  if (g.nrow > ACC_STRIDE) return false;
  g.a_plane = g.kx * TM * 16;
  g.a_tile = 2 * g.a_plane;
  g.b_hi = (g.kx + 1 + g.mix) * g.nrow * 16;
  g.b_lo = g.split ? g.b_hi : (g.mix ? g.kx * g.nrow * 16 : (g.kx + 1) * 16 * 16);
  g.b_chunk = g.b_hi + g.b_lo;
  if (g.D <= 64) {
    g.kp = 1;
    g.kc_part = g.kx;
    g.part_bytes = g.part_last_bytes = g.stage_bytes = g.b_chunk;
    g.stages = (g.split || g.mix) ? 2 : 3;
  } else {
    g.kp = g.D / 32;
    g.kc_part = 4;
    const int lo4 = (g.split || g.mix) ? 4 * g.nrow * 16 : 4 * 16 * 16;
    const int lo5 = g.split ? 5 * g.nrow * 16 : (g.mix ? lo4 : 5 * 16 * 16);
    g.part_bytes = 4 * g.nrow * 16 + lo4;
    g.part_last_bytes = g.stage_bytes = (5 + g.mix) * g.nrow * 16 + lo5;
    g.stages = 3;
  }
  g.tpc = g.kp == 1 ? TPC : (g.D > 128 ? 1 : 2);
  g.smem_bytes = g.tpc * g.a_tile + g.stages * g.stage_bytes + NBUF * 2 * TM * 16 + 4096 + SORTN * 8 + 3 * HMETA * 4 + 6 * TM * 4 + 256 + 128 +
                 (g.kp == 1 ? 9 * TPC * TM * 4 : 0) +
                 (g.km ? HMETA * 4 : 0);
  return g.smem_bytes <= 227 * 1024;
}

struct Scales {
  float sA, sS, sB, sAe, sBe, inv_sigma, inv_s;
  int npos;
  float omega0, omega1, omegab;
  float rho;
  int use_mix;
};
constexpr float kMixRhoMax = 128.f;
constexpr int kMixMinHist = 16;
__device__ __forceinline__ bool user_in_pass(int gate, int use_mix, int H) {
  return gate < 0 || ((use_mix && H >= kMixMinHist) ? 1 : 0) == gate;
}
constexpr int HDR_BYTES = 4096;
constexpr int HDR_PERM = 128, HDR_CK = HDR_PERM + 256 * 4, HDR_U = HDR_CK + 256 * 4;
static_assert(HDR_U + 256 * 4 <= HDR_BYTES, "header");

__global__ void absmax_kernel(const float* __restrict__ x, size_t n, unsigned* out) {
  float m = 0.f;
  for (size_t i = blockIdx.x * (size_t)blockDim.x + threadIdx.x; i < n; i += (size_t)gridDim.x * blockDim.x) m = fmaxf(m, fabsf(x[i]));
#pragma unroll
  for (int o = 16; o > 0; o >>= 1) m = fmaxf(m, __shfl_xor_sync(0xffffffffu, m, o));
  if ((threadIdx.x & 31) == 0) atomicMax(out, __float_as_uint(m));
}

__device__ __forceinline__ float pow2floor(float x) { return exp2f(floorf(log2f(x))); }

__global__ void scales_kernel(NaisParams p, unsigned char* hdr) {
  const NaisBranch& br = p.branch[0];
  const int D = br.w_poi + br.w_reg, hid = p.hid;
  const int lanes = p.dist_mode == NAIS_DIST_LATLON ? 2 : 0, ldw = D + lanes;
  const unsigned* mx = reinterpret_cast<const unsigned*>(hdr);
  Scales* sc = reinterpret_cast<Scales*>(hdr + 64);
  int* perm = reinterpret_cast<int*>(hdr + HDR_PERM);
  float* ck = reinterpret_cast<float*>(hdr + HDR_CK);
  float* u = reinterpret_cast<float*>(hdr + HDR_U);
  __shared__ float red[8];
  __shared__ int s_npos;
  if (threadIdx.x == 0) {
    int n = 0;
    for (int k = 0; k < hid; ++k)
      if (br.w2[k] >= 0.f) perm[n++] = k;
    s_npos = n;
    for (int k = 0; k < hid; ++k)
      if (!(br.w2[k] >= 0.f)) perm[n++] = k;
    for (int i = 0; i < 8; ++i) red[i] = 0.f;
  }
  __syncthreads();
  for (int k = threadIdx.x; k < hid; k += blockDim.x) ck[k] = 0.5f * fabsf(br.w2[k]);
  for (int d = threadIdx.x; d < D; d += blockDim.x) {
    float a = 0.f;
    for (int k = 0; k < hid; ++k) a += 0.5f * br.w2[k] * br.w1[(size_t)k * ldw + d];
    u[d] = a;
  }
  __syncthreads();
  float mcw = 0.f, mbe = 0.f;
  for (int i = threadIdx.x; i < hid * D; i += blockDim.x) {
    int k = i / D, d = i - k * D;
    mcw = fmaxf(mcw, fabsf(ck[k] * br.w1[(size_t)k * ldw + d]));
  }
  for (int d = threadIdx.x; d < D; d += blockDim.x) mcw = fmaxf(mcw, fabsf(u[d]));
  for (int k = threadIdx.x; k < hid; k += blockDim.x) {
    mbe = fmaxf(mbe, fabsf(ck[k] * br.b1[k]));
    if (lanes) {
      mbe = fmaxf(mbe, fabsf(ck[k] * br.w1[(size_t)k * ldw + D]));
      mbe = fmaxf(mbe, fabsf(ck[k] * br.w1[(size_t)k * ldw + D + 1]));
    }
  }
  atomicMax(reinterpret_cast<unsigned*>(&red[0]), __float_as_uint(mcw));
  atomicMax(reinterpret_cast<unsigned*>(&red[1]), __float_as_uint(mbe));
  __syncthreads();
  if (threadIdx.x == 0) {
    float o0 = 0.f, o1 = 0.f, ob = 0.f;
    for (int k = 0; k < hid; ++k) {
      const float hv = 0.5f * br.w2[k];
      ob += hv * br.b1[k];
      if (lanes) {
        o0 += hv * br.w1[(size_t)k * ldw + D];
        o1 += hv * br.w1[(size_t)k * ldw + D + 1];
      }
    }
    const float tiny = 1e-30f;
    const float maxP = fmaxf(fmaxf(__uint_as_float(mx[0]), __uint_as_float(mx[1])), tiny);
    const float maxQ = fmaxf(fmaxf(__uint_as_float(mx[2]), __uint_as_float(mx[3])), tiny);
    const float maxB = fmaxf(maxQ * red[0], tiny);
    const float maxBe = fmaxf(fmaxf(red[1], fmaxf(fabsf(o0), fmaxf(fabsf(o1), fabsf(ob)))), tiny);
    float sA = pow2floor(512.f / maxP), sS = pow2floor(512.f / maxQ), sB = pow2floor(512.f / maxB);
    const float sAe = 256.f;
    float sBe = sA * sB / sAe;
    while (maxBe * sBe > 16384.f) {
      sB *= 0.5f;
      sBe *= 0.5f;
    }
    sc->sA = sA;
    sc->sS = sS;
    sc->sB = sB;
    sc->sAe = sAe;
    sc->sBe = sBe;
    sc->inv_sigma = 1.f / (sA * sB);
    sc->inv_s = 1.f / (sA * sS);
    sc->npos = s_npos;
    sc->omega0 = o0;
    sc->omega1 = o1;
    sc->omegab = ob;
    sc->rho = maxP * maxB * sqrtf((float)(hid * D));
    sc->use_mix = sc->rho <= kMixRhoMax ? 1 : 0;
  }
}

__device__ __forceinline__ uint2 pack_e5m2(const __half* h) {
  unsigned char b[8];
#pragma unroll
  for (int e = 0; e < 8; ++e) b[e] = (unsigned char)__nv_cvt_halfraw_to_fp8(static_cast<__half_raw>(h[e]), __NV_SATFINITE, __NV_E5M2);
  uint2 r;
  r.x = b[0] | (b[1] << 8) | (b[2] << 16) | ((unsigned)b[3] << 24);
  r.y = b[4] | (b[5] << 8) | (b[6] << 16) | ((unsigned)b[7] << 24);
  return r;
}

__global__ void pack_candidates_kernel(NaisParams p, NaisCatalog cat, int64_t poi_begin, int64_t poi_end, Geo g,
                                       const unsigned char* hdr, unsigned char* Pimg) {
  const NaisBranch& br = p.branch[0];
  const Scales* sc = reinterpret_cast<const Scales*>(hdr + 64);
  const float sA = sc->sA;
  const int tile = blockIdx.x;
  for (int i = threadIdx.x; i < TM * g.kx; i += blockDim.x) {
    const int c = i / TM, r = i - c * TM;
    const int64_t j = poi_begin + (int64_t)tile * TM + r;
    __half hi[8], lo[8];
    if (j < poi_end) {
      const int64_t jl = j - cat.row_base;
      for (int e = 0; e < 8; ++e) {
        const int d = c * 8 + e;
        const float v = (d < br.w_poi) ? __ldg(br.tgt_poi + (size_t)j * br.w_poi + d)
                                       : __ldg(br.tgt_reg + (size_t)__ldg(cat.region + jl) * br.w_reg + (d - br.w_poi));
        split_f16(v * sA, hi[e], lo[e]);
      }
    } else {
      for (int e = 0; e < 8; ++e) hi[e] = lo[e] = __float2half(0.f);
    }
    unsigned char* base = Pimg + (size_t)tile * g.a_tile + ((size_t)c * TM + r) * 16;
    *reinterpret_cast<uint4*>(base) = *reinterpret_cast<uint4*>(hi);
    if (g.mix) {
      unsigned char* b8 = Pimg + (size_t)tile * g.a_tile + g.a_plane + ((size_t)(c >> 1) * TM + r) * 16 + (c & 1) * 8;
      *reinterpret_cast<uint2*>(b8) = pack_e5m2(hi);
      *reinterpret_cast<uint2*>(b8 + g.a_plane / 2) = pack_e5m2(lo);
    } else {
      *reinterpret_cast<uint4*>(base + g.a_plane) = *reinterpret_cast<uint4*>(lo);
    }
  }
}

__device__ __forceinline__ int64_t chunk_base(const int64_t* offsets, int u, int hch, int hsplit = 1) {
  return hch == 2 ? (offsets[u] + u) >> 1 : offsets[u] * hsplit;
}

__global__ void pack_users_kernel(NaisParams p, NaisUsers users, Geo g_mix, Geo g_split, int two_pass, const unsigned char* hdr,
                                  unsigned char* Bimg, int64_t max_chunks, int* pass_flags, int* bad) {
  const NaisBranch& br = p.branch[0];
  const Scales* sc = reinterpret_cast<const Scales*>(hdr + 64);
  const int* perm = reinterpret_cast<const int*>(hdr + HDR_PERM);
  const float* ck = reinterpret_cast<const float*>(hdr + HDR_CK);
  const float* uu = reinterpret_cast<const float*>(hdr + HDR_U);
  const int u = blockIdx.x;
  const int64_t hb = users.offsets[u];
  const int H = (int)(users.offsets[u + 1] - hb);
  int pass = 1;
  if (two_pass) {
    pass = user_in_pass(1, sc->use_mix, H) ? 1 : 0;
    if (threadIdx.x == 0 && blockIdx.y == 0) pass_flags[pass] = 1;
  }
  const Geo& g = pass ? g_mix : g_split;
  const int hch = g.hch, aux0 = g.aux0, hsplit = g.hsplit;
  const int nchunks = (H + hch - 1) / hch * hsplit;
  const int D = g.D, hid = g.hid, ldw = D + g.lanes;
  __shared__ float q[2][256];
  for (int chunk = blockIdx.y; chunk < nchunks; chunk += gridDim.y) {
    const int hc = chunk / hsplit, half = chunk - hc * hsplit;
    __syncthreads();
    for (int i = threadIdx.x; i < hch * D; i += blockDim.x) {
      const int hs = i / D, d = i - hs * D, h = hch * hc + hs;
      float v = 0.f;
      if (h < H) {
        const int64_t e = hb + h;
        v = (d < br.w_poi) ? __ldg(br.hist_poi + (size_t)checked_id(__ldg(users.items + e), p.item_num, bad) * br.w_poi + d)
                           : __ldg(br.hist_reg + (size_t)checked_id(__ldg(users.region + e), p.region_num, bad) * br.w_reg + (d - br.w_poi));
      }
      q[hs][d] = v;
    }
    __syncthreads();
    const int64_t slot = chunk_base(users.offsets, u, hch, hsplit) - chunk_base(users.offsets, 0, hch, hsplit) + chunk;
    if (slot >= max_chunks) continue;
    unsigned char* cb = Bimg + (size_t)slot * g.b_chunk;
    for (int i = threadIdx.x; i < g.nrow * (g.kx + 1); i += blockDim.x) {
      const int c = i / g.nrow, n = i - c * g.nrow;
      float v[8];
#pragma unroll
      for (int e = 0; e < 8; ++e) v[e] = 0.f;
      int hs = -1, kind = -1, k = 0;
      if (n < aux0) {
        hs = n / hid;
        kind = 0;
        k = perm[half * hid + n - hs * hid];
      } else if (n < aux0 + 2 * hch && half == 0) {
        hs = (n - aux0) >> 1;
        kind = 1 + ((n - aux0) & 1);
      }
      if (kind >= 0 && hch * hc + hs < H) {
        if (c < g.kx) {
#pragma unroll
          for (int e = 0; e < 8; ++e) {
            const int d = c * 8 + e;
            const float qd = q[hs][d];
            if (kind == 0) v[e] = ck[k] * __ldg(br.w1 + (size_t)k * ldw + d) * qd * sc->sB;
            else if (kind == 1) v[e] = qd * sc->sS;
            else v[e] = uu[d] * qd * sc->sB;
          }
        } else if (g.mix) {
        } else {
          if (kind == 0) {
            if (g.lanes) {
              v[2 * hs] = ck[k] * __ldg(br.w1 + (size_t)k * ldw + D) * sc->sBe;
              v[2 * hs + 1] = ck[k] * __ldg(br.w1 + (size_t)k * ldw + D + 1) * sc->sBe;
            }
            v[4] = ck[k] * __ldg(br.b1 + k) * sc->sBe;
          } else if (kind == 2) {
            v[2 * hs] = sc->omega0 * sc->sBe;
            v[2 * hs + 1] = sc->omega1 * sc->sBe;
            v[4] = sc->omegab * sc->sBe;
          }
        }
      }
      __half hi[8], lo[8];
#pragma unroll
      for (int e = 0; e < 8; ++e) split_f16(v[e], hi[e], lo[e]);
      const int part = g.kp == 1 ? 0 : min(c / g.kc_part, g.kp - 1);
      const int cp = c - part * g.kc_part;
      const int nkc = g.kc_part + (part == g.kp - 1 ? 1 + g.mix : 0);
      const int nrw = g.pair ? g.nrow / 2 : g.nrow;
      const int nn = g.pair ? n % nrw : n;
      unsigned char* pb = cb + (size_t)part * g.part_bytes + (g.pair ? (size_t)(n / nrw) * (g.b_chunk / 2) : 0);
      unsigned char* lb = pb + (size_t)nkc * nrw * 16;
      if (g.mix && c == g.kx) {
        float w0 = 0.f, w1 = 0.f, wb = 0.f;
        if (kind == 0 && hch * hc + hs < H) {
          if (g.lanes) {
            w0 = ck[k] * __ldg(br.w1 + (size_t)k * ldw + D) * sc->sBe;
            w1 = ck[k] * __ldg(br.w1 + (size_t)k * ldw + D + 1) * sc->sBe;
          }
          wb = ck[k] * __ldg(br.b1 + k) * sc->sBe;
        } else if (kind == 2 && hch * hc + hs < H) {
          w0 = sc->omega0 * sc->sBe;
          w1 = sc->omega1 * sc->sBe;
          wb = sc->omegab * sc->sBe;
        }
        __half e0[8], e1[8], h0, l0, h1, l1, hb, lb2;
#pragma unroll
        for (int e = 0; e < 8; ++e) e0[e] = e1[e] = __float2half(0.f);
        split_f16(w0, h0, l0);
        split_f16(w1, h1, l1);
        split_f16(wb, hb, lb2);
        if (hs >= 0) {
          e0[2 * hs] = h0;
          e0[2 * hs + 1] = h1;
          e0[4] = hb;
          e0[5] = lb2;
          e1[2 * hs] = h0;
          e1[2 * hs + 1] = h1;
          e1[4 + 2 * hs] = l0;
          e1[5 + 2 * hs] = l1;
        }
        *reinterpret_cast<uint4*>(pb + ((size_t)cp * nrw + nn) * 16) = *reinterpret_cast<uint4*>(e0);
        *reinterpret_cast<uint4*>(pb + ((size_t)(cp + 1) * nrw + nn) * 16) = *reinterpret_cast<uint4*>(e1);
        continue;
      }
      *reinterpret_cast<uint4*>(pb + ((size_t)cp * nrw + nn) * 16) = *reinterpret_cast<uint4*>(hi);
      if (g.mix) {
        unsigned char* b8 = lb + ((size_t)(cp >> 1) * nrw + nn) * 16 + (cp & 1) * 8;
        *reinterpret_cast<uint2*>(b8) = pack_e5m2(hi);
        *reinterpret_cast<uint2*>(b8 + (size_t)(g.kc_part / 2) * nrw * 16) = pack_e5m2(lo);
      } else if (g.split) {
        *reinterpret_cast<uint4*>(lb + ((size_t)cp * nrw + nn) * 16) = *reinterpret_cast<uint4*>(lo);
      } else if (n >= aux0 && n < aux0 + 16) {
        *reinterpret_cast<uint4*>(lb + ((size_t)cp * 16 + (n - aux0)) * 16) = *reinterpret_cast<uint4*>(lo);
      }
    }
  }
}

__device__ __forceinline__ int user_chunks(const int64_t* offsets, int u, int hch, int64_t cb0, int64_t max_chunks, int hsplit = 1) {
  const int H = (int)(offsets[u + 1] - offsets[u]);
  const int64_t room = max_chunks - (chunk_base(offsets, u, hch, hsplit) - cb0);
  const int n = (H + hch - 1) / hch * hsplit;
  const int m = (int)(room < n ? (room < 0 ? 0 : room) : n);
  return m - m % hsplit;
}

struct MainArgs {
  NaisParams p;
  NaisCatalog cat;
  NaisUsers users;
  Geo g;
  int64_t poi_begin, poi_end;
  int k, exclude, groups;
  int groups_real;
  int64_t n_items;
  const unsigned char* hdr;
  const unsigned char* Pimg;
  const unsigned char* Bimg;
  unsigned long long* part_keys;
  float* all_scores;
  const float* score_in;
  int64_t max_chunks;
  int gate;
  const int* pass_flags;
  GeoMixArgs geo;
};

__device__ __forceinline__ void epi_bar() { asm volatile("bar.sync 1, 512;" ::: "memory"); }

__device__ __forceinline__ unsigned long long warp_sort_desc(unsigned long long v, int lane) {
#pragma unroll
  for (int k = 2; k <= 32; k <<= 1) {
#pragma unroll
    for (int j = k >> 1; j > 0; j >>= 1) {
      const unsigned long long o = __shfl_xor_sync(0xffffffffu, v, j);
      const bool desc = k == 32 || (lane & k) == 0, lower = (lane & j) == 0;
      v = (lower == desc) ? (v > o ? v : o) : (v < o ? v : o);
    }
  }
  return v;
}
__device__ __forceinline__ unsigned long long warp_fold_top32(unsigned long long a, unsigned long long b, int lane) {
  const unsigned long long br = __shfl_sync(0xffffffffu, b, 31 - lane);
  unsigned long long v = a > br ? a : br;
#pragma unroll
  for (int j = 16; j > 0; j >>= 1) {
    const unsigned long long o = __shfl_xor_sync(0xffffffffu, v, j);
    v = ((lane & j) == 0) ? (v > o ? v : o) : (v < o ? v : o);
  }
  return v;
}

template <bool kSinglePart, int kHch, int kFix, int kS = 64, bool kGeo = false>
__global__ void __launch_bounds__(THREADS, 1) fullrank_tc_kernel(const __grid_constant__ MainArgs A) {
  constexpr bool kPair = kFix == 5 || kFix == 6;
  constexpr bool kFastEpi = kFix == 1 || kFix == 2 || kPair;
  constexpr bool kD128 = kFix == 3;
  static_assert(!kGeo || kFix == 0 || kFix == 4, "geo mode lives in the run-time-shape epilogue");
  constexpr int kCombA = kGeo ? 4 : 3, kCombT = (kGeo && !kSinglePart) ? 2 : TPC;
  extern __shared__ __align__(128) unsigned char smem[];
  const Geo& g = A.g;
  unsigned char* sA = smem;
  unsigned char* sB = sA + g.tpc * g.a_tile;
  unsigned char* sE = sB + g.stages * g.stage_bytes;
  unsigned char* sZ = sE + NBUF * 2 * TM * 16;
  unsigned long long* keys = reinterpret_cast<unsigned long long*>(sZ + 4096);
  float* comb = kSinglePart ? reinterpret_cast<float*>(keys + SORTN) : reinterpret_cast<float*>(sE);
  int* hm_id = reinterpret_cast<int*>(reinterpret_cast<unsigned char*>(keys + SORTN) + (kSinglePart ? 3 * kCombA * TPC * TM * 4 : 0));
  float* hm_la = reinterpret_cast<float*>(hm_id + HMETA);
  float* hm_lo = hm_la + HMETA;
  float* xch = hm_lo + HMETA;
  uint64_t* bars = reinterpret_cast<uint64_t*>(xch + 6 * TM);
  uint64_t* a_full = bars + 0;
  uint64_t* a_empty = bars + 1;
  uint64_t* b_full = bars + 2;
  uint64_t* b_empty = bars + 2 + MAX_STAGES;
  uint64_t* e_full = bars + 2 + 2 * MAX_STAGES;
  uint64_t* acc_full = e_full + NBUF;
  uint64_t* acc_empty = acc_full + 2 * NBUF;
  uint32_t* tslot = reinterpret_cast<uint32_t*>(acc_empty + NBUF);
  float* hm_cos = reinterpret_cast<float*>(reinterpret_cast<unsigned char*>(bars) + 384);
  uint64_t* a_full_peer = reinterpret_cast<uint64_t*>(tslot + 2);
  uint64_t* b_full_peer = a_full_peer + 1;
  uint32_t crank = 0;
  if constexpr (kPair) asm volatile("mov.u32 %0, %%cluster_ctarank;" : "=r"(crank));
  const int64_t item0 = kPair ? (int64_t)(blockIdx.x >> 1) : (int64_t)blockIdx.x, item_step = kPair ? (int64_t)(gridDim.x >> 1) : (int64_t)gridDim.x;
  const int groups_it = kPair ? A.groups / 2 : A.groups;

  const int tid = threadIdx.x, warp = tid >> 5, lane = tid & 31;
  const Scales sc = *reinterpret_cast<const Scales*>(A.hdr + 64);
  if (A.gate >= 0 && !A.pass_flags[A.gate]) return;

  auto init_ext_word = [&](int i) {
    const int byte = i * 4, in_buf = byte % (2 * TM * 16);
    const bool bias = byte < NBUF * 2 * TM * 16 && in_buf < TM * 16 && (in_buf & 15) == 8;
    const uint32_t one = (uint32_t)__half_as_ushort(__float2half(sc.sAe));
    reinterpret_cast<uint32_t*>(sE)[i] = bias ? (g.mix ? (one | (one << 16)) : one) : 0u;
  };
  for (int i = tid; i < (NBUF * 2 * TM * 16 + 4096) / 4; i += THREADS) init_ext_word(i);
  if (kFastEpi && tid < 16) xch[tid] = ((sc.npos & ~15) + tid < sc.npos) ? 1.f : -1.f;
  if (tid == 0) {
    mbar_init(a_full, 1);
    mbar_init(a_empty, 1);
    for (int i = 0; i < MAX_STAGES; ++i) {
      mbar_init(&b_full[i], 1);
      mbar_init(&b_empty[i], 1);
    }
    for (int i = 0; i < NBUF; ++i) {
      mbar_init(&e_full[i], kPair ? 2 * ARRIVE_WARPS : ARRIVE_WARPS);
      mbar_init(&acc_full[i], 1);
      mbar_init(&acc_full[NBUF + i], 1);
      mbar_init(&acc_empty[i], kPair ? 2 * ARRIVE_WARPS : ARRIVE_WARPS);
    }
    if (kPair) {
      mbar_init(a_full_peer, 1);
      for (int i = 0; i < MAX_STAGES; ++i) mbar_init(&b_full_peer[i], 1);
    }
    fence_barrier_init();
  }
  if (warp == EPI_WARPS) {
    if constexpr (kPair) tmem_alloc2(tslot, 512);
    else tmem_alloc(tslot, 512);
  }
  fence_proxy_async();
  tc_fence_before();
  __syncthreads();
  if constexpr (kPair) cluster_sync_all();
  tc_fence_after();
  const uint32_t tmem = *tslot;

  constexpr int tpc = kSinglePart ? TPC : (kFix == 4 ? 1 : 2);
  const int hsplit = kHch == 1 ? g.hsplit : 1;
  const int64_t cb0 = chunk_base(A.users.offsets, 0, kHch, hsplit);

  if (warp == EPI_WARPS + 1) {
    {
      uint32_t it_n = 0, bstep = 0;
      for (int64_t item = item0; item < A.n_items; item += item_step) {
        const int u = (int)(item / groups_it), grp = kPair ? 2 * (int)(item % groups_it) + (int)crank : (int)(item % groups_it);
        if (!user_in_pass(A.gate, sc.use_mix, (int)(A.users.offsets[u + 1] - A.users.offsets[u]))) continue;
        const uint32_t it = it_n++;
        const int64_t cbu = __shfl_sync(0xffffffffu, chunk_base(A.users.offsets, u, kHch, hsplit) - cb0, 0);
        const int nchunks = __shfl_sync(0xffffffffu, user_chunks(A.users.offsets, u, kHch, cb0, A.max_chunks, hsplit), 0);
        mbar_wait(a_empty, (it & 1) ^ 1);
        if (elect_one()) {
          mbar_expect_tx(a_full, (uint32_t)(tpc * g.a_tile));
          for (int t = 0; t < tpc; ++t)
            bulk_g2s(sA + (size_t)t * g.a_tile, A.Pimg + ((size_t)grp * tpc + t) * g.a_tile, (uint32_t)g.a_tile, a_full);
        }
        __syncwarp();
        const unsigned char* src = A.Bimg + (size_t)cbu * g.b_chunk + (kPair ? (size_t)crank * (g.b_chunk / 2) : 0);
        for (int c = 0; c < nchunks; ++c) {
          const int kp_t = kSinglePart ? 1 : g.kp;
          for (int pp = 0; pp < kp_t; ++pp, ++bstep) {
            const int st = bstep % g.stages;
            const uint32_t bytes = kPair ? (uint32_t)(g.b_chunk / 2) : (uint32_t)(pp == kp_t - 1 ? g.part_last_bytes : g.part_bytes);
            mbar_wait(&b_empty[st], ((bstep / g.stages) & 1) ^ 1);
            if (elect_one()) {
              mbar_expect_tx(&b_full[st], bytes);
              bulk_g2s(sB + (size_t)st * g.stage_bytes, src + (size_t)c * g.b_chunk + (size_t)pp * g.part_bytes, bytes, &b_full[st]);
            }
            __syncwarp();
          }
        }
      }
    }
  } else if (warp == EPI_WARPS) {
    if constexpr (kFastEpi) {
      constexpr bool kMix = kFix == 2 || kFix == 6;
      constexpr uint32_t kStages = kPair ? 4u : 2u;
      constexpr uint32_t kKx = kS / 8, kK16 = kS / 16, kK32 = kS / 32;
      constexpr uint32_t kNrow = 2 * kS + 16, kALbo = TM * 16;
      constexpr uint32_t kBLbo = (kPair ? kNrow / 2 : kNrow) * 16;
      constexpr uint32_t kAStep = (2 * kALbo) >> 4, kBStep = (2 * kBLbo) >> 4;
      constexpr uint32_t kAPlane = kKx * TM * 16, kATile = (2 * kAPlane) >> 4;
      constexpr uint32_t kStage = (2 * (kKx + 1) * kBLbo) >> 4;
      constexpr uint32_t kExtBuf = (2 * TM * 16) >> 4;
      constexpr uint32_t idN = idesc_f16(kPair ? 2 * TM : TM, kNrow), idN8 = idesc_e5m2(kPair ? 2 * TM : TM, kNrow);
      auto mmaH = [](uint32_t d, uint64_t a, uint64_t b, uint32_t id, uint32_t acc) {
        if constexpr (kPair) mma2_f16(d, a, b, id, acc);
        else mma_f16(d, a, b, id, acc);
      };
      auto mmaQ = [](uint32_t d, uint64_t a, uint64_t b, uint32_t id, uint32_t acc) {
        if constexpr (kPair) mma2_f8(d, a, b, id, acc);
        else mma_f8(d, a, b, id, acc);
      };
      auto commit = [](uint64_t* bar) {
        if constexpr (kPair) mma2_commit_multicast(bar, 3);
        else mma_commit(bar);
      };
      const uint32_t zaddr = smem_u32(sZ);
      const uint32_t hi_word = (uint32_t)(smem_desc(0, 0, 128) >> 32);
      auto lo_of = [](uint32_t addr, uint32_t lbo) { return ((addr >> 4) & 0x3FFFu) | (((lbo >> 4) & 0x3FFFu) << 16); };
      auto mk = [&](uint32_t lo) { return ((uint64_t)hi_word << 32) | lo; };
      const uint32_t sa0 = smem_u32(sA), sb0 = smem_u32(sB), se0 = smem_u32(sE);
      const uint32_t A_hi = lo_of(sa0, kALbo);
      const uint32_t A_lo = lo_of(sa0 + kAPlane, kALbo);
      const uint32_t A_l8 = lo_of(sa0 + kAPlane + kAPlane / 2, kALbo);
      const uint32_t E_hi = lo_of(se0, zaddr - se0), E_lo = lo_of(se0 + TM * 16, zaddr - se0 - TM * 16);
      constexpr uint32_t kEz = kExtBuf - (kExtBuf << 16), kBz = kStage - (kStage << 16);
      const uint32_t E_mx = lo_of(se0, TM * 16);
      const uint32_t B_hi = lo_of(sb0, kBLbo);
      const uint32_t Bx_hi = lo_of(sb0 + kKx * kBLbo, zaddr - (sb0 + kKx * kBLbo));
      const uint32_t Bx_lo = lo_of(sb0 + (2 * kKx + 1) * kBLbo, zaddr - (sb0 + (2 * kKx + 1) * kBLbo));
      uint32_t it_n = 0, cc = 0, st = 0, stph = 0;
      for (int64_t item = item0; item < A.n_items; item += item_step) {
        const int u = (int)(item / groups_it);
        if (!user_in_pass(A.gate, sc.use_mix, (int)(A.users.offsets[u + 1] - A.users.offsets[u]))) continue;
        const uint32_t it = it_n++;
        const int nchunks = __shfl_sync(0xffffffffu, user_chunks(A.users.offsets, u, kHch, cb0, A.max_chunks, hsplit), 0);
        mbar_wait(a_full, it & 1);
        if constexpr (kPair) {
          if (crank != 0) {
            if (elect_one()) mbar_arrive_cluster(a_full_peer, 0);
            __syncwarp();
            for (int c = 0; c < nchunks; ++c) {
              mbar_wait(&b_full[st], stph);
              if (elect_one()) mbar_arrive_cluster(&b_full_peer[st], 0);
              __syncwarp();
              st = (st + 1u) % kStages;
              stph ^= (st == 0);
            }
            continue;
          }
          mbar_wait_cluster(a_full_peer, it & 1);
        }
        for (int c = 0; c < nchunks; ++c, ++cc) {
          mbar_wait(&b_full[st], stph);
          if constexpr (kPair) mbar_wait_cluster(&b_full_peer[st], stph);
          const uint32_t cph = cc & 1u;
          const uint32_t bh = B_hi + st * kStage;
          const uint32_t bxh = Bx_hi + st * kBz, bxl = Bx_lo + st * kBz;
          uint64_t* const accf = &acc_full[(c & 1) * NBUF];
#pragma unroll
          for (int t = 0; t < TPC; ++t) {
            const uint32_t d_t = tmem + t * ACC_STRIDE;
            const uint32_t ah = A_hi + t * kATile, al = A_lo + t * kATile, al8 = A_l8 + t * kATile;
            if constexpr (kPair) {
              mbar_wait_cluster(&acc_empty[t], cph ^ 1u);
              mbar_wait_cluster(&e_full[t], cph);
            } else {
              mbar_wait(&acc_empty[t], cph ^ 1u);
              mbar_wait(&e_full[t], cph);
            }
            tc_fence_after();
            if (elect_one()) {
#pragma unroll
              for (int s2 = 0; s2 < (int)kK16; ++s2) mmaH(d_t, mk(ah + s2 * kAStep), mk(bh + s2 * kBStep), idN, s2 != 0);
              if constexpr (kMix) {
                mmaH(d_t, mk(E_mx + t * kExtBuf), mk(bh + kK16 * kBStep), idN, 1);
                constexpr uint32_t b8h = ((kKx + 2) * kBLbo) >> 4, b8l = ((kKx + 2 + kKx / 2) * kBLbo) >> 4;
#pragma unroll
                for (int s8 = 0; s8 < (int)kK32; ++s8) mmaQ(d_t, mk(al + s8 * kAStep), mk(bh + b8l + s8 * kBStep), idN8, 1);
#pragma unroll
                for (int s8 = 0; s8 < (int)kK32; ++s8) mmaQ(d_t, mk(al8 + s8 * kAStep), mk(bh + b8h + s8 * kBStep), idN8, 1);
              } else {
                constexpr uint32_t blo = ((kKx + 1) * kBLbo) >> 4;
                mmaH(d_t, mk(E_hi + t * kEz), mk(bxh), idN, 1);
#pragma unroll
                for (int s2 = 0; s2 < (int)kK16; ++s2) mmaH(d_t, mk(ah + s2 * kAStep), mk(bh + blo + s2 * kBStep), idN, 1);
                mmaH(d_t, mk(E_hi + t * kEz), mk(bxl), idN, 1);
#pragma unroll
                for (int s2 = 0; s2 < (int)kK16; ++s2) mmaH(d_t, mk(al + s2 * kAStep), mk(bh + s2 * kBStep), idN, 1);
                mmaH(d_t, mk(E_lo + t * kEz), mk(bxh), idN, 1);
              }
              commit(&accf[t]);
            }
            __syncwarp();
          }
          if (elect_one()) commit(&b_empty[st]);
          __syncwarp();
          st = (st + 1u) % kStages;
          stph ^= (st == 0);
        }
        if (elect_one()) commit(a_empty);
        __syncwarp();
      }
    } else
    {
      const int nrow_c = kD128 ? 144 : g.nrow, a_plane_c = kD128 ? 16 * TM * 16 : g.a_plane, a_tile_c = kD128 ? 32 * TM * 16 : g.a_tile;
      const int stage_bytes_c = kD128 ? 10 * 144 * 16 : g.stage_bytes, stages_c = kD128 ? 3 : g.stages;
      const uint32_t idN = idesc_f16(TM, nrow_c), id16 = idesc_f16(TM, 16), idN8 = idesc_e5m2(TM, nrow_c);
      const uint32_t zaddr = smem_u32(sZ);
      const uint32_t a_lbo = TM * 16, b_lbo = nrow_c * 16, l_lbo = 16 * 16;
      const uint32_t a_step = (2 * a_lbo) >> 4, b_step = (2 * b_lbo) >> 4, l_step = (2 * l_lbo) >> 4;
      const uint32_t hi_word = (uint32_t)(smem_desc(0, 0, 128) >> 32);
      auto lo_of = [](uint32_t addr, uint32_t lbo) { return ((addr >> 4) & 0x3FFFu) | (((lbo >> 4) & 0x3FFFu) << 16); };
      auto mk = [&](uint32_t lo) { return ((uint64_t)hi_word << 32) | lo; };
      const uint32_t sa0 = smem_u32(sA), sb0 = smem_u32(sB), se0 = smem_u32(sE);
      const uint32_t A_hi0 = lo_of(sa0, a_lbo), A_lo0 = lo_of(sa0 + a_plane_c, a_lbo), A_d = (uint32_t)a_tile_c >> 4;
      const uint32_t E_hi0 = lo_of(se0, zaddr - se0), E_lo0 = lo_of(se0 + TM * 16, zaddr - se0 - TM * 16);
      const uint32_t E_d = (uint32_t)((2 * TM * 16) >> 4) - ((uint32_t)((2 * TM * 16) >> 4) << 16);
      const uint32_t sbytes = (uint32_t)stage_bytes_c >> 4;
      const uint32_t B_d = sbytes, Bz_d = sbytes - (sbytes << 16);
      const int kcp = kD128 ? 4 : g.kc_part, ks_part = kcp / 2;
      const bool split = g.split != 0, mix = g.mix != 0;
      const uint32_t B_hi0 = lo_of(sb0, b_lbo);
      const uint32_t lo_off_mid = (uint32_t)kcp * b_lbo, lo_off_last = (uint32_t)(kcp + 1 + g.mix) * b_lbo;
      const int ks8 = kcp / 4;
      const uint32_t A8_0 = lo_of(sa0 + a_plane_c, a_lbo), A8l_0 = lo_of(sa0 + a_plane_c + a_plane_c / 2, a_lbo);
      const uint32_t Em_0 = lo_of(se0, TM * 16), Em_d = (uint32_t)((2 * TM * 16) >> 4);
      const uint32_t Bem_0 = lo_of(sb0 + kcp * b_lbo, b_lbo);
      const uint32_t bex = sb0 + kcp * b_lbo;
      const uint32_t Be_hi0 = lo_of(bex, zaddr - bex);
      const uint32_t belx = sb0 + lo_off_last + kcp * b_lbo;
      const uint32_t Be_lo0 = lo_of(belx, zaddr - belx);
      const uint32_t bha = sb0 + g.aux0 * 16;
      const uint32_t Ba_hi0 = lo_of(bha, b_lbo), Bae_hi0 = lo_of(bha + kcp * b_lbo, zaddr - (bha + kcp * b_lbo));
      const uint32_t baelx = sb0 + lo_off_last + kcp * l_lbo;
      const uint32_t Bae_lo0 = lo_of(baelx, zaddr - baelx);
      uint32_t it_n = 0, n = 0, st = 0, stph = 0;
      for (int64_t item = blockIdx.x; item < A.n_items; item += gridDim.x) {
        const int u = (int)(item / A.groups);
        if (!user_in_pass(A.gate, sc.use_mix, (int)(A.users.offsets[u + 1] - A.users.offsets[u]))) continue;
        const uint32_t it = it_n++;
        const int nchunks = __shfl_sync(0xffffffffu, user_chunks(A.users.offsets, u, kHch, cb0, A.max_chunks, hsplit), 0);
        mbar_wait(a_full, it & 1);
        for (int c = 0; c < nchunks; ++c, n += (uint32_t)tpc) {
          const int kp_m = kSinglePart ? 1 : (kD128 ? 4 : g.kp);
#pragma unroll
          for (int pp = 0; pp < (kD128 ? 4 : kp_m); ++pp) {
            const bool lastp = kSinglePart ? true : pp == kp_m - 1;
            mbar_wait(&b_full[st], stph);
            const uint32_t lo_off = lastp ? lo_off_last : lo_off_mid;
            const uint32_t bh = B_hi0 + st * B_d;
            const uint32_t bl = lo_of(sb0 + lo_off, b_lbo) + st * B_d;
            const uint32_t bal = lo_of(sb0 + lo_off, l_lbo) + st * B_d;
            const uint32_t bah = Ba_hi0 + st * B_d;
            const uint32_t beh = Be_hi0 + st * Bz_d, bel = Be_lo0 + st * Bz_d;
            const uint32_t baeh = Bae_hi0 + st * Bz_d, bael = Bae_lo0 + st * Bz_d;
            const uint32_t ka = (uint32_t)(pp * ks_part) * a_step;
            const uint32_t ka8 = (uint32_t)(pp * ks8) * a_step;
            const uint32_t b8h = bl, b8l = bl + (uint32_t)((kcp / 2) * b_lbo >> 4);
            const uint32_t bem = Bem_0 + st * B_d;
#pragma unroll
            for (int t = 0; t < TPC; ++t) {
              if (t >= tpc) break;
              const uint32_t nn = n + (uint32_t)t, buf = nn % NBUF, ph = (nn / NBUF) & 1u;
              const uint32_t ah = A_hi0 + t * A_d + ka, al = A_lo0 + t * A_d + ka;
              const uint32_t eh = E_hi0 + buf * E_d, el = E_lo0 + buf * E_d;
              const uint32_t d_t = tmem + buf * ACC_STRIDE, d_aux = d_t + g.aux0;
              if (pp == 0) mbar_wait(&acc_empty[buf], ph ^ 1);
              if (lastp) mbar_wait(&e_full[buf], ph);
              tc_fence_after();
              if (elect_one()) {
                for (int s2 = 0; s2 < ks_part; ++s2) mma_f16(d_t, mk(ah + s2 * a_step), mk(bh + s2 * b_step), idN, (pp | s2) != 0);
                if (mix) {
                  if (lastp) mma_f16(d_t, mk(Em_0 + buf * Em_d), mk(bem), idN, 1);
                  const uint32_t a8h = A8_0 + t * A_d + ka8, a8l = A8l_0 + t * A_d + ka8;
                  for (int s8 = 0; s8 < ks8; ++s8) mma_f8(d_t, mk(a8h + s8 * a_step), mk(b8l + s8 * b_step), idN8, 1);
                  for (int s8 = 0; s8 < ks8; ++s8) mma_f8(d_t, mk(a8l + s8 * a_step), mk(b8h + s8 * b_step), idN8, 1);
                } else if (split) {
                  if (lastp) mma_f16(d_t, mk(eh), mk(beh), idN, 1);
                  for (int s2 = 0; s2 < ks_part; ++s2) mma_f16(d_t, mk(ah + s2 * a_step), mk(bl + s2 * b_step), idN, 1);
                  if (lastp) mma_f16(d_t, mk(eh), mk(bel), idN, 1);
                  for (int s2 = 0; s2 < ks_part; ++s2) mma_f16(d_t, mk(al + s2 * a_step), mk(bh + s2 * b_step), idN, 1);
                  if (lastp) mma_f16(d_t, mk(el), mk(beh), idN, 1);
                } else {
                  if (lastp) mma_f16(d_t, mk(eh), mk(beh), idN, 1);
                  for (int s2 = 0; s2 < ks_part; ++s2) mma_f16(d_aux, mk(ah + s2 * a_step), mk(bal + s2 * l_step), id16, 1);
                  if (lastp) mma_f16(d_aux, mk(eh), mk(bael), id16, 1);
                  for (int s2 = 0; s2 < ks_part; ++s2) mma_f16(d_aux, mk(al + s2 * a_step), mk(bah + s2 * b_step), id16, 1);
                  if (lastp) mma_f16(d_aux, mk(el), mk(baeh), id16, 1);
                }
                if (lastp) mma_commit(&acc_full[(c & 1) * NBUF + buf]);
              }
              __syncwarp();
            }
            if (elect_one()) mma_commit(&b_empty[st]);
            __syncwarp();
            if (++st == (uint32_t)stages_c) {
              st = 0;
              stph ^= 1;
            }
          }
        }
        if (elect_one()) mma_commit(a_empty);
        __syncwarp();
      }
    }
  } else {
    const int egrp = warp >> 3;
    const int qd = warp & 3, hs = (warp >> 2) & 1;
    const int r = qd * 32 + lane;
    const uint32_t lane_addr = (uint32_t)(qd * 32) << 16;
    const float nl2e = -1.4426950408889634f, dsc = A.p.dist_scale * nl2e;
    const float w00 = g.lanes ? __ldg(A.p.dist_w + 0) * dsc : 0.f, w01 = g.lanes ? __ldg(A.p.dist_w + 1) * dsc : 0.f;
    const float w10 = g.lanes ? __ldg(A.p.dist_w + 2) * dsc : 0.f, w11 = g.lanes ? __ldg(A.p.dist_w + 3) * dsc : 0.f;
    const float bd0 = g.lanes ? __ldg(A.p.dist_b + 0) * nl2e : 0.f, bd1 = g.lanes ? __ldg(A.p.dist_b + 1) * nl2e : 0.f;
    const float beta = A.p.beta;
    const bool geo = g.lanes || g.km;
    float ckm = 0.f;
    if constexpr (!kFastEpi)
      if (g.km)
        for (int d = 0; d < g.D; ++d) ckm += __ldg(A.p.dist_embed + d);
    const int npos = sc.npos, hid = g.hid;
    constexpr int hch = kHch;
    const int ncols = hch == 2 ? hid : hid / 2;
    const int col0 = hs * ncols;
    const int kidx0 = hch == 2 ? 0 : col0 + (hsplit == 2 ? egrp * hid : 0);
    auto div_tpc = [&](int x) { return x / tpc; };
    uint32_t n0 = 0;
    uint32_t phbits = 0;
    uint32_t fph = 0;
    const float c_a2 = sc.inv_sigma * 1.4426950408889634f, inv_sAe = 1.f / sc.sAe;
    const float bd0s = bd0 - log2f(sc.sAe), bd1s = bd1 - log2f(sc.sAe);
    const int nposb = npos >> 4, nposm = npos & 15;
    const float* sgn_mixed = xch;

    auto arrive_mma = [&](uint64_t* bar) {
      if constexpr (kPair) mbar_arrive_cluster(bar, 0);
      else mbar_arrive(bar);
    };
    for (int64_t item = item0; item < A.n_items; item += item_step) {
      const int u = (int)(item / groups_it), grp = kPair ? 2 * (int)(item % groups_it) + (int)crank : (int)(item % groups_it);
      const int64_t hb = A.users.offsets[u];
      const int H = (int)(A.users.offsets[u + 1] - hb);
      if (!user_in_pass(A.gate, sc.use_mix, H)) continue;
      const int nchunks = user_chunks(A.users.offsets, u, hch, cb0, A.max_chunks, hsplit);
      const int nsteps = nchunks * tpc;
      epi_bar();
      for (int i = tid; i < H && i < HMETA; i += EPI_THREADS) {
        hm_id[i] = __ldg(A.users.items + hb + i);
        hm_la[i] = (geo || kGeo) ? __ldg(A.users.coords + 2 * (hb + i)) : 0.f;
        hm_lo[i] = (geo || kGeo) ? __ldg(A.users.coords + 2 * (hb + i) + 1) : 0.f;
        if constexpr (!kFastEpi)
          if (g.km || kGeo) hm_cos[i] = cosf((A.cat.center_lat + hm_la[i]) * 0.017453292519943295f);
      }
      float clat[TPC], clon[TPC], ccos[TPC], sumE[TPC], sumES[TPC], sumL[TPC];
      int64_t jid[TPC];
      bool excl[TPC];
#pragma unroll
      for (int t = 0; t < TPC; ++t) {
        jid[t] = t < tpc ? A.poi_begin + ((int64_t)grp * tpc + t) * TM + r : A.poi_end;
        const bool v = jid[t] < A.poi_end;
        clat[t] = (v && (geo || kGeo)) ? __ldg(A.cat.coords + 2 * (jid[t] - A.cat.row_base)) : 0.f;
        clon[t] = (v && (geo || kGeo)) ? __ldg(A.cat.coords + 2 * (jid[t] - A.cat.row_base) + 1) : 0.f;
        ccos[t] = 1.f;
        if constexpr (!kFastEpi)
          if (g.km || kGeo) ccos[t] = cosf((A.cat.center_lat + clat[t]) * 0.017453292519943295f);
        sumE[t] = 0.f;
        sumES[t] = 0.f;
        sumL[t] = 0.f;
        excl[t] = false;
      }
      epi_bar();
      if constexpr (kFastEpi) {
        const unsigned char* ebase = sE + r * 16 + hs * 4;
        auto produce_f = [&](int t, bool on, float hla, float hlo, float cla, float clo) {
          float g0 = 0.f, g1 = 0.f;
          if (on) {
            const float l0 = fabsf(cla - hla), l1 = fabsf(clo - hlo);
            const float z0 = fmaf(l1, w01, fmaf(l0, w00, bd0s)), z1 = fmaf(l1, w11, fmaf(l0, w10, bd1s));
            g0 = rcp_approx(ex2_approx(z0) + inv_sAe);
            g1 = rcp_approx(ex2_approx(z1) + inv_sAe);
          }
          const __half2 hi2 = __floats2half2_rn(g0, g1);
          const float2 hif = __half22float2(hi2);
          const __half2 lo2 = __floats2half2_rn(g0 - hif.x, g1 - hif.y);
          unsigned char* eb = const_cast<unsigned char*>(ebase) + t * (2 * TM * 16);
          *reinterpret_cast<__half2*>(eb) = hi2;
          *reinterpret_cast<__half2*>(eb + TM * 16) = lo2;
          if (g.mix) *reinterpret_cast<__half2*>(eb + TM * 16 + 8) = hi2;
          fence_proxy_async();
          __syncwarp();
          if (lane == 0) arrive_mma(&e_full[t]);
        };
        auto hist_coords = [&](int h, float& la, float& lo) {
          if (h < HMETA) {
            la = hm_la[h];
            lo = hm_lo[h];
          } else {
            la = __ldg(A.users.coords + 2 * (hb + h));
            lo = __ldg(A.users.coords + 2 * (hb + h) + 1);
          }
        };
        int jt[TPC];
#pragma unroll
        for (int t = 0; t < TPC; ++t) jt[t] = jid[t] < A.poi_end ? (int)jid[t] : -2;
        if (egrp == 0 && nchunks > 0) {
          const bool on = g.lanes && hs < H;
          float la = 0.f, lo = 0.f;
          if (on) hist_coords(hs, la, lo);
#pragma unroll
          for (int t = 0; t < TPC; ++t) produce_f(t, on, la, lo, clat[t], clon[t]);
        }
        const uint32_t tb_main = tmem + lane_addr + (uint32_t)(hs * kS), tb_aux = tmem + lane_addr + (uint32_t)(2 * kS) + (uint32_t)(2 * hs);
        for (int c = egrp; c < nchunks; c += 2) {
          const int h = 2 * c + hs;
          const bool hvalid = h < H;
          int hist_id = -1;
          if (hvalid) hist_id = h < HMETA ? hm_id[h] : __ldg(A.users.items + hb + h);
          const bool pn = c + 1 < nchunks;
          const bool pon = pn && g.lanes && (h + 2 < H);
          float nla = 0.f, nlo = 0.f;
          if (pon) hist_coords(h + 2, nla, nlo);
#pragma unroll
          for (int t = 0; t < TPC; ++t) {
            mbar_wait(&acc_full[egrp * NBUF + t], fph);
            tc_fence_after();
            uint32_t aux[2], va[16], vb[16];
            float p0 = 0.f, p1 = 0.f, p2 = 0.f, p3 = 0.f, q0 = 0.f, q1 = 0.f, q2 = 0.f, q3 = 0.f;
            auto blk = [&](const uint32_t(&v)[16], int b) {
              if (b < nposb) {
#pragma unroll
                for (int i = 0; i < 16; i += 4) {
                  p0 += fabsf(__uint_as_float(v[i]));
                  p1 += fabsf(__uint_as_float(v[i + 1]));
                  p2 += fabsf(__uint_as_float(v[i + 2]));
                  p3 += fabsf(__uint_as_float(v[i + 3]));
                }
              } else if (b > nposb || nposm == 0) {
#pragma unroll
                for (int i = 0; i < 16; i += 4) {
                  q0 += fabsf(__uint_as_float(v[i]));
                  q1 += fabsf(__uint_as_float(v[i + 1]));
                  q2 += fabsf(__uint_as_float(v[i + 2]));
                  q3 += fabsf(__uint_as_float(v[i + 3]));
                }
              } else {
#pragma unroll
                for (int i = 0; i < 16; i += 4) {
                  const float4 sg = *reinterpret_cast<const float4*>(sgn_mixed + i);
                  p0 = fmaf(fabsf(__uint_as_float(v[i])), sg.x, p0);
                  p1 = fmaf(fabsf(__uint_as_float(v[i + 1])), sg.y, p1);
                  p2 = fmaf(fabsf(__uint_as_float(v[i + 2])), sg.z, p2);
                  p3 = fmaf(fabsf(__uint_as_float(v[i + 3])), sg.w, p3);
                }
              }
            };
            tmem_ld2(tb_aux + t * ACC_STRIDE, aux);
            tmem_ld16(tb_main + t * ACC_STRIDE, va);
            tmem_ld16(tb_main + t * ACC_STRIDE + 16, vb);
            if (pn) produce_f(t, pon, nla, nlo, clat[t], clon[t]);
            tmem_wait_ld16(va);
            tmem_wait_ld16(vb);
            if constexpr (kS == 64) {
              blk(va, 0);
              tmem_ld16(tb_main + t * ACC_STRIDE + 32, va);
              blk(vb, 1);
              tmem_ld16(tb_main + t * ACC_STRIDE + 48, vb);
              tmem_wait_ld16(va);
              tmem_wait_ld16(vb);
            }
            tc_fence_before();
            __syncwarp();
            if (lane == 0) arrive_mma(&acc_empty[t]);
            if constexpr (kS == 64) {
              blk(va, 2);
              blk(vb, 3);
            } else {
              blk(va, 0);
              blk(vb, 1);
            }
            const float asum = ((p0 + p1) + (p2 + p3)) - ((q0 + q1) + (q2 + q3));
            const float S = __uint_as_float(aux[0]) * sc.inv_s;
            const float a2 = (__uint_as_float(aux[1]) + asum) * c_a2;
            const bool same = hist_id == jt[t];
            const float e = (hvalid && !same) ? ex2_approx(a2) : 0.f;
            sumE[t] += e;
            sumES[t] = fmaf(e, S, sumES[t]);
            excl[t] = excl[t] || (hvalid && same);
          }
          fph ^= 1u;
        }
      } else {
        auto produce = [&](int m) {
          const int pc = div_tpc(m), pt = m - pc * tpc;
          const uint32_t pbuf = (n0 + (uint32_t)m) % NBUF;
          const int h = hch == 2 ? 2 * pc + hs : pc / hsplit;
          float g0 = 0.f, g1 = 0.f;
          if (g.lanes && h < H && (hch == 2 || hs == 0)) {
            float hla, hlo;
            if (h < HMETA) {
              hla = hm_la[h];
              hlo = hm_lo[h];
            } else {
              hla = __ldg(A.users.coords + 2 * (hb + h));
              hlo = __ldg(A.users.coords + 2 * (hb + h) + 1);
            }
            const float ct_la = pt == 0 ? clat[0] : (pt == 1 ? clat[1] : clat[2]);
            const float ct_lo = pt == 0 ? clon[0] : (pt == 1 ? clon[1] : clon[2]);
            const float l0 = fabsf(ct_la - hla), l1 = fabsf(ct_lo - hlo);
            const float z0 = fmaf(l1, w01, fmaf(l0, w00, bd0)), z1 = fmaf(l1, w11, fmaf(l0, w10, bd1));
            g0 = __fdividef(sc.sAe, 1.f + exp2f(z0));
            g1 = __fdividef(sc.sAe, 1.f + exp2f(z1));
          }
          const __half2 hi2 = __floats2half2_rn(g0, g1);
          const float2 hif = __half22float2(hi2);
          const __half2 lo2 = __floats2half2_rn(g0 - hif.x, g1 - hif.y);
          if (hch == 2 || hs == 0) {
            unsigned char* eb = sE + (size_t)pbuf * 2 * TM * 16 + r * 16 + hs * 4;
            *reinterpret_cast<__half2*>(eb) = hi2;
            *reinterpret_cast<__half2*>(eb + TM * 16) = lo2;
            if (g.mix) *reinterpret_cast<__half2*>(eb + TM * 16 + 8) = hi2;
          }
          fence_proxy_async();
          __syncwarp();
          if (lane == 0) mbar_arrive(&e_full[pbuf]);
        };
        if (egrp == 0)
          for (int m = 0; m < NBUF && m < nsteps; ++m) produce(m);

        for (int c = egrp, t = 0; c < nchunks; (t + 1 == tpc) ? (t = 0, c += 2) : ++t) {
          const int ls = c * tpc + t;
          const uint32_t n = n0 + (uint32_t)ls;
          const uint32_t buf = n % NBUF;
          const int h = hch == 2 ? 2 * c + hs : c / hsplit;
          int hist_id = -1;
          if (h < H) hist_id = h < HMETA ? hm_id[h] : __ldg(A.users.items + hb + h);
          mbar_wait(&acc_full[egrp * NBUF + buf], (phbits >> buf) & 1u);
          phbits ^= 1u << buf;
          tc_fence_after();
          if (ls + NBUF < nsteps) produce(ls + NBUF);
          const uint32_t t_main = tmem + lane_addr + buf * ACC_STRIDE + col0;
          uint32_t aux[2], v[32];
          float accp = 0.f, accn = 0.f;
          tmem_ld2(tmem + lane_addr + buf * ACC_STRIDE + g.aux0 + (hch == 2 ? 2 * hs : 0), aux);
          if (ncols >= 32) tmem_ld32(t_main, v);
          else tmem_ld16(t_main, *reinterpret_cast<uint32_t(*)[16]>(&v[0]));
          tmem_wait_ld();
          auto absum = [&](int c0, int cnt) {
  #pragma unroll
            for (int g16 = 0; g16 < 32; g16 += 16) {
              if (g16 < cnt) {
                const int cc = kidx0 + c0 + g16;
                if (cc + 16 <= npos || cc >= npos) {
                  float s0 = 0.f, s1 = 0.f, s2 = 0.f, s3 = 0.f;
  #pragma unroll
                  for (int i = 0; i < 16; i += 4) {
                    s0 += fabsf(__uint_as_float(v[g16 + i]));
                    s1 += fabsf(__uint_as_float(v[g16 + i + 1]));
                    s2 += fabsf(__uint_as_float(v[g16 + i + 2]));
                    s3 += fabsf(__uint_as_float(v[g16 + i + 3]));
                  }
                  const float ssum = (s0 + s1) + (s2 + s3);
                  if (cc >= npos) accn += ssum;
                  else accp += ssum;
                } else {
  #pragma unroll
                  for (int i = 0; i < 16; ++i) {
                    const float av = fabsf(__uint_as_float(v[g16 + i]));
                    if (cc + i < npos) accp += av;
                    else accn += av;
                  }
                }
              }
            }
          };
          absum(0, ncols >= 32 ? 32 : 16);
          if (ncols > 32) {
            if (ncols >= 64) tmem_ld32(t_main + 32, v);
            else tmem_ld16(t_main + 32, *reinterpret_cast<uint32_t(*)[16]>(&v[0]));
            tmem_wait_ld();
          }
          tc_fence_before();
          __syncwarp();
          if (lane == 0) mbar_arrive(&acc_empty[buf]);
          if (ncols > 32) absum(32, ncols >= 64 ? 32 : 16);
          float asum = accp - accn;
          if (hch == 1 && hsplit == 1) {
            float* slot = xch + ((ls & 1) * 2 + egrp) * TM + r;
            if (hs == 1) *slot = asum;
            asm volatile("bar.sync %0, 64;" ::"r"(2 + egrp * 4 + qd) : "memory");
            if (hs == 0) asum += *slot;
          } else if (hch == 1) {
            const int par = ((c >> 1) * tpc + t) & 1;
            float* slots = xch + par * 3 * TM + r;
            const int sender = egrp * 2 + hs - 1;
            if (sender >= 0) slots[sender * TM] = asum;
            asm volatile("bar.sync %0, 128;" ::"r"(10 + qd) : "memory");
            if (sender < 0) asum = ((asum + slots[0]) + slots[TM]) + slots[2 * TM];
          }
          const float S = __uint_as_float(aux[0]) * sc.inv_s;
          const float a = (__uint_as_float(aux[1]) + asum) * sc.inv_sigma;
          if (h < H && (hch == 2 || hs == 0) && (hsplit == 1 || egrp == 0)) {
            const int64_t j = t == 0 ? jid[0] : (t == 1 ? jid[1] : jid[2]);
            if constexpr (kGeo) {
              float hla, hlo, hcs;
              if (h < HMETA) {
                hla = hm_la[h];
                hlo = hm_lo[h];
                hcs = hm_cos[h];
              } else {
                hla = __ldg(A.users.coords + 2 * (hb + h));
                hlo = __ldg(A.users.coords + 2 * (hb + h) + 1);
                hcs = cosf((A.cat.center_lat + hla) * 0.017453292519943295f);
              }
              const float cla = t == 0 ? clat[0] : (t == 1 ? clat[1] : clat[2]), clo = t == 0 ? clon[0] : (t == 1 ? clon[1] : clon[2]);
              const float ccs = t == 0 ? ccos[0] : (t == 1 ? ccos[1] : ccos[2]);
              const float lt = powerlaw_log_term(dist_km_f(cla, clo, hla, hlo, ccs, hcs), A.geo.ln_a, A.geo.b);
              if (t == 0) sumL[0] += lt;
              else if (t == 1) sumL[1] += lt;
              else sumL[2] += lt;
            }
            if ((int64_t)hist_id != j) {
              float a_km = a;
              if (g.km) {
                float hla, hlo, hcs;
                if (h < HMETA) {
                  hla = hm_la[h];
                  hlo = hm_lo[h];
                  hcs = hm_cos[h];
                } else {
                  hla = __ldg(A.users.coords + 2 * (hb + h));
                  hlo = __ldg(A.users.coords + 2 * (hb + h) + 1);
                  hcs = cosf((A.cat.center_lat + hla) * 0.017453292519943295f);
                }
                const float cla = t == 0 ? clat[0] : (t == 1 ? clat[1] : clat[2]), clo = t == 0 ? clon[0] : (t == 1 ? clon[1] : clon[2]);
                const float ccs = t == 0 ? ccos[0] : (t == 1 ? ccos[1] : ccos[2]);
                const float km = dist_km_f(cla, clo, hla, hlo, ccs, hcs);
                a_km = fmaf(km, ckm, a);
              }
              const float e = g.km ? expf(a_km) : __expf(a);
              if (t == 0) { sumE[0] += e; sumES[0] = fmaf(e, S, sumES[0]); }
              else if (t == 1) { sumE[1] += e; sumES[1] = fmaf(e, S, sumES[1]); }
              else { sumE[2] += e; sumES[2] = fmaf(e, S, sumES[2]); }
            } else {
              if (t == 0) excl[0] = true;
              else if (t == 1) excl[1] = true;
              else excl[2] = true;
            }
          }
        }
        n0 += (uint32_t)nsteps;
      }
      const int part = egrp * 2 + hs;
      const bool small_k = A.k <= 32;
      unsigned long long kreg[TPC];
      if (!kSinglePart) epi_bar();
      if (part != 0) {
#pragma unroll
        for (int t2 = 0; t2 < kCombT; ++t2) {
          comb[((part - 1) * kCombA + 0) * kCombT * TM + t2 * TM + r] = sumE[t2];
          comb[((part - 1) * kCombA + 1) * kCombT * TM + t2 * TM + r] = sumES[t2];
          comb[((part - 1) * kCombA + 2) * kCombT * TM + t2 * TM + r] = excl[t2] ? 1.f : 0.f;
          if constexpr (kGeo) comb[((part - 1) * kCombA + 3) * kCombT * TM + t2 * TM + r] = sumL[t2];
        }
      }
      epi_bar();
      if (part == 0) {
#pragma unroll
        for (int t2 = 0; t2 < TPC; ++t2) {
          float E = sumE[t2], ES = sumES[t2], Lg = sumL[t2];
          bool ex = excl[t2];
          if (t2 < kCombT) {
#pragma unroll
            for (int q = 0; q < 3; ++q) {
              E += comb[(q * kCombA + 0) * kCombT * TM + t2 * TM + r];
              ES += comb[(q * kCombA + 1) * kCombT * TM + t2 * TM + r];
              ex = ex || comb[(q * kCombA + 2) * kCombT * TM + t2 * TM + r] != 0.f;
              if constexpr (kGeo) Lg += comb[(q * kCombA + 3) * kCombT * TM + t2 * TM + r];
            }
          }
          float score = ES / powf(E, beta);
          const bool valid = jid[t2] < A.poi_end;
          if (A.score_in && valid) score += A.score_in[(size_t)u * (A.poi_end - A.poi_begin) + (jid[t2] - A.poi_begin)];
          if constexpr (kGeo) score = geo_mixed(score, Lg, __ldg(A.geo.user_logmax + u), A.geo.alpha);
          if (A.all_scores && valid) A.all_scores[(size_t)u * (A.poi_end - A.poi_begin) + (jid[t2] - A.poi_begin)] = score;
          kreg[t2] = (valid && !(A.exclude && ex)) ? make_key(score, (int)jid[t2]) : 0ull;
          if (!small_k) keys[t2 * TM + r] = kreg[t2];
        }
        if (small_k) {
          unsigned long long a = warp_sort_desc(kreg[0], lane);
          a = warp_fold_top32(a, warp_sort_desc(kreg[1], lane), lane);
          a = warp_fold_top32(a, warp_sort_desc(kreg[2], lane), lane);
          keys[r] = a;
        } else {
          for (int i = TPC * TM + r; i < SORTN; i += TM) keys[i] = 0ull;
        }
      }
      epi_bar();
      if (!kSinglePart) {
        for (int i = tid; i < (NBUF * 2 * TM * 16 + 4096) / 4; i += EPI_THREADS) init_ext_word(i);
        fence_proxy_async();
      }
      if (small_k) {
        if (warp == 0) {
          unsigned long long a = warp_fold_top32(keys[lane], keys[32 + lane], lane);
          a = warp_fold_top32(a, warp_fold_top32(keys[64 + lane], keys[96 + lane], lane), lane);
          if (lane < A.k && grp < A.groups_real) A.part_keys[((size_t)u * A.groups_real + grp) * A.k + lane] = a;
        }
        continue;
      }
      for (int kk = 2; kk <= SORTN; kk <<= 1) {
        for (int jj = kk >> 1; jj > 0; jj >>= 1) {
          for (int i = tid; i < SORTN; i += EPI_THREADS) {
            const int ixj = i ^ jj;
            if (ixj > i) {
              const unsigned long long x = keys[i], y = keys[ixj];
              const bool desc = (i & kk) == 0;
              if (desc ? (x < y) : (x > y)) {
                keys[i] = y;
                keys[ixj] = x;
              }
            }
          }
          epi_bar();
        }
      }
      if (grp < A.groups_real)
        for (int i = tid; i < A.k; i += EPI_THREADS) A.part_keys[((size_t)u * A.groups_real + grp) * A.k + i] = keys[i];
    }
  }
  tc_fence_before();
  __syncthreads();
  if constexpr (kPair) cluster_sync_all();
  if (warp == EPI_WARPS) {
    if constexpr (kPair) tmem_dealloc2(tmem, 512);
    else tmem_dealloc(tmem, 512);
  }
}


}

int launch_topk_merge(const unsigned long long* in_keys, const float* in_score, const int32_t* in_id, int n_users,
                      int n_lists, int k, float* out_score, int32_t* out_id, cudaStream_t stream);
int launch_topk_merge_keys_multi(const unsigned long long* keys, unsigned long long* scratch, int64_t user_stride, int64_t list_stride,
                                 int n_users, int n_lists, int k, unsigned long long* out_keys, float* out_score, int32_t* out_id,
                                 cudaStream_t stream);
int merge_scratch_lists(int n_lists, int k);

static inline size_t al256(size_t x) { return (x + 255) / 256 * 256; }

struct PlanLayout {
  tc::Geo g, gs;
  bool two_pass;
  bool pair;
  tc::Geo gp, gsp;
  int groups, n_tiles_pad;
  size_t hdr, pimg, pimg2, total;
};

static bool plan_layout(const NaisParams& p, int64_t poi_begin, int64_t poi_end, int precision, PlanLayout& L) {
  const int prec = precision & NAIS_PREC_MASK;
  if (!tc::make_geo(p, prec, L.g)) return false;
  L.two_pass = false;
  if (prec == NAIS_PREC_TC_AUTO) {
    if (!tc::make_geo(p, NAIS_PREC_TC_SPLIT, L.gs)) return false;
    L.two_pass = L.g.mix != 0;
    if (L.two_pass && (L.gs.a_tile != L.g.a_tile || L.gs.b_chunk != L.g.b_chunk || L.gs.tpc != L.g.tpc || L.gs.hch != L.g.hch ||
                       L.gs.hsplit != L.g.hsplit))
      return false;
  } else {
    L.gs = L.g;
  }
  const int64_t range = poi_end - poi_begin;
  const int64_t tiles = (range + tc::TM - 1) / tc::TM;
  L.groups = (int)((tiles + L.g.tpc - 1) / L.g.tpc);
  if (L.groups < 1) L.groups = 1;
  auto pair_shape = [](const tc::Geo& q) {
    return q.D == 64 && q.hid == 64 && q.nrow == 144 && q.kp == 1 && q.hch == 2 && q.stages == 2 && !q.km && (q.mix || q.split);
  };
  L.pair = !(precision & (NAIS_PREC_FLAG_ONE_CTA | NAIS_PREC_FLAG_GENERIC)) && pair_shape(L.g) && pair_shape(L.gs) && L.groups >= 2;
  L.gp = L.g;
  L.gsp = L.gs;
  if (L.pair)
    for (tc::Geo* q : {&L.gp, &L.gsp}) {
      q->pair = 1;
      q->smem_bytes -= q->stages * q->stage_bytes;
      q->stage_bytes = q->b_chunk / 2;
      q->stages = 4;
      q->smem_bytes += q->stages * q->stage_bytes;
    }
  L.n_tiles_pad = (L.pair ? (L.groups + 1) / 2 * 2 : L.groups) * L.g.tpc;
  size_t o = 0;
  L.hdr = o;
  o += tc::HDR_BYTES;
  L.pimg = o;
  o += al256((size_t)L.n_tiles_pad * L.g.a_tile);
  L.pimg2 = o;
  if (L.two_pass) o += al256((size_t)L.n_tiles_pad * L.g.a_tile);
  L.total = o;
  return true;
}

static inline size_t call_keys_bytes(int n_users, int groups, int k) { return al256((size_t)n_users * groups * k * 8); }
static inline size_t call_scratch_bytes(int n_users, int groups, int k) {
  return al256((size_t)n_users * merge_scratch_lists(groups, k) * k * 8 + 8);
}

static NaisParams branch_view(const NaisParams& p, int bi) {
  NaisParams q = p;
  q.n_branch = 1;
  q.branch[0] = p.branch[bi];
  return q;
}
static inline size_t branch_scores_bytes(const NaisParams& p, int n_users, int64_t poi_begin, int64_t poi_end) {
  return p.n_branch > 1 ? al256((size_t)n_users * (size_t)(poi_end - poi_begin) * 4) : 0;
}

bool tc_supported(const NaisParams& p, int precision) {
  for (int bi = 0; bi < p.n_branch; ++bi) {
    tc::Geo g;
    if (!tc::make_geo(branch_view(p, bi), precision & NAIS_PREC_MASK, g)) return false;
  }
  return true;
}

static size_t plan_bytes_1(const NaisParams& p, int64_t poi_begin, int64_t poi_end, int precision) {
  PlanLayout L;
  return plan_layout(p, poi_begin, poi_end, precision, L) ? L.total : 0;
}
size_t fullrank_tc_plan_bytes(const NaisParams& p, int64_t poi_begin, int64_t poi_end, int precision) {
  size_t total = 0;
  for (int bi = 0; bi < p.n_branch; ++bi) {
    const size_t b = plan_bytes_1(branch_view(p, bi), poi_begin, poi_end, precision);
    if (!b) return 0;
    total += b;
  }
  return total;
}

static size_t call_workspace_bytes_1(const NaisParams& p, int n_users, int64_t nnz, int64_t poi_begin, int64_t poi_end, int k,
                                     int precision) {
  PlanLayout L;
  if (!plan_layout(p, poi_begin, poi_end, precision, L)) return 0;
  const int64_t max_chunks = (L.g.hch == 2 ? (nnz + n_users) / 2 : nnz * L.g.hsplit) + 2;
  return 256 + al256((size_t)max_chunks * L.g.b_chunk) + call_keys_bytes(n_users, L.groups, k) + call_scratch_bytes(n_users, L.groups, k);
}
size_t fullrank_tc_call_workspace_bytes(const NaisParams& p, int n_users, int64_t nnz, int64_t poi_begin, int64_t poi_end, int k,
                                        int precision) {
  size_t most = 0;
  for (int bi = 0; bi < p.n_branch; ++bi) {
    const size_t b = call_workspace_bytes_1(branch_view(p, bi), n_users, nnz, poi_begin, poi_end, k, precision);
    if (!b) return 0;
    most = b > most ? b : most;
  }
  return most + branch_scores_bytes(p, n_users, poi_begin, poi_end);
}

size_t fullrank_tc_workspace_bytes(const NaisParams& p, int n_users, int64_t nnz, int64_t poi_begin, int64_t poi_end, int k,
                                   int precision) {
  const size_t a = fullrank_tc_plan_bytes(p, poi_begin, poi_end, precision);
  const size_t b = fullrank_tc_call_workspace_bytes(p, n_users, nnz, poi_begin, poi_end, k, precision);
  return (a && b) ? a + b + 1024 + (size_t)n_users * 8 : 0;
}

static int check_arch(int& sms) {
  int dev = 0, major = 0;
  cudaGetDevice(&dev);
  cudaDeviceGetAttribute(&major, cudaDevAttrComputeCapabilityMajor, dev);
  if (major != 10) return NAIS_ERR_ARCH;
  sms = 148;
  cudaDeviceGetAttribute(&sms, cudaDevAttrMultiProcessorCount, dev);
  return 0;
}

static int prepare_1(const NaisParams& p, const NaisCatalog& cat, int64_t poi_begin, int64_t poi_end, int precision, void* plan,
                     size_t plan_bytes, cudaStream_t stream) {
  if (poi_end <= poi_begin) return 0;
  int sms;
  int rc = check_arch(sms);
  if (rc) return rc;
  PlanLayout L;
  if (!plan_layout(p, poi_begin, poi_end, precision, L)) return NAIS_ERR_SHAPE;
  if (plan_bytes < L.total) return NAIS_ERR_WORKSPACE;
  unsigned char* base = reinterpret_cast<unsigned char*>(plan);
  unsigned char* hdr = base + L.hdr;
  const NaisBranch& br = p.branch[0];
  cudaError_t e = cudaMemsetAsync(hdr, 0, tc::HDR_BYTES, stream);
  if (e != cudaSuccess) return (int)e;
  unsigned* mx = reinterpret_cast<unsigned*>(hdr);
  auto amax = [&](const float* x, size_t n, unsigned* out) {
    if (!x || n == 0) return;
    int blocks = (int)((n + 255) / 256);
    if (blocks > 4 * sms) blocks = 4 * sms;
    tc::absmax_kernel<<<blocks, 256, 0, stream>>>(x, n, out);
    NAIS_COUNT_LAUNCH(1);
  };
  amax(br.tgt_poi, (size_t)p.item_num * br.w_poi, mx + 0);
  amax(br.tgt_reg, (size_t)p.region_num * br.w_reg, mx + 1);
  amax(br.hist_poi, (size_t)p.item_num * br.w_poi, mx + 2);
  amax(br.hist_reg, (size_t)p.region_num * br.w_reg, mx + 3);
  tc::scales_kernel<<<1, 256, 0, stream>>>(p, hdr);
  NAIS_COUNT_LAUNCH(1);
  tc::pack_candidates_kernel<<<L.n_tiles_pad, 256, 0, stream>>>(p, cat, poi_begin, poi_end, L.g, hdr, base + L.pimg);
  NAIS_COUNT_LAUNCH(1);
  if (L.two_pass) {
    tc::pack_candidates_kernel<<<L.n_tiles_pad, 256, 0, stream>>>(p, cat, poi_begin, poi_end, L.gs, hdr, base + L.pimg2);
    NAIS_COUNT_LAUNCH(1);
  }
  e = cudaGetLastError();
  return e == cudaSuccess ? 0 : (int)e;
}

int fullrank_tc_prepare(const NaisParams& p, const NaisCatalog& cat, int64_t poi_begin, int64_t poi_end, int precision, void* plan,
                        size_t plan_bytes, cudaStream_t stream) {
  size_t off = 0;
  for (int bi = 0; bi < p.n_branch; ++bi) {
    const NaisParams q = branch_view(p, bi);
    const size_t b = plan_bytes_1(q, poi_begin, poi_end, precision);
    if (!b) return NAIS_ERR_SHAPE;
    if (plan_bytes < off + b) return NAIS_ERR_WORKSPACE;
    const int rc = prepare_1(q, cat, poi_begin, poi_end, precision, reinterpret_cast<unsigned char*>(plan) + off, b, stream);
    if (rc) return rc;
    off += b;
  }
  return 0;
}

typedef void (*MainKernel)(const tc::MainArgs);

static MainKernel pick_kernel(const tc::Geo& gg, bool generic) {
  const bool s64 = gg.D == 64 && gg.hid == 64 && gg.nrow == 144, s32 = gg.D == 32 && gg.hid == 32 && gg.nrow == 80;
  if (gg.km) generic = true;
  const int fix = ((s64 || s32) && gg.kp == 1 && gg.hch == 2 && gg.stages == 2 && !generic) ? (gg.mix ? 2 : (gg.split ? 1 : 0)) : 0;
  if (gg.pair) return gg.mix ? tc::fullrank_tc_kernel<true, 2, 6, 64> : tc::fullrank_tc_kernel<true, 2, 5, 64>;
  if (gg.kp == 1) {
    if (gg.hch != 2) return tc::fullrank_tc_kernel<true, 1, 0>;
    if (fix == 2) return s64 ? tc::fullrank_tc_kernel<true, 2, 2, 64> : tc::fullrank_tc_kernel<true, 2, 2, 32>;
    if (fix == 1) return s64 ? tc::fullrank_tc_kernel<true, 2, 1, 64> : tc::fullrank_tc_kernel<true, 2, 1, 32>;
    return tc::fullrank_tc_kernel<true, 2, 0>;
  }
  if (gg.tpc == 1) return gg.hch == 2 ? tc::fullrank_tc_kernel<false, 2, 4> : tc::fullrank_tc_kernel<false, 1, 4>;
  if (gg.hch == 2) return tc::fullrank_tc_kernel<false, 2, 0>;
  if (gg.D == 128 && gg.hid == 128 && gg.kp == 4 && gg.nrow == 144 && gg.stages == 3 && (gg.mix || gg.split) && !generic)
    return tc::fullrank_tc_kernel<false, 1, 3>;
  return tc::fullrank_tc_kernel<false, 1, 0>;
}

static MainKernel pick_geo_kernel(const tc::Geo& gg) {
  if (gg.kp == 1) return gg.hch == 2 ? tc::fullrank_tc_kernel<true, 2, 0, 64, true> : tc::fullrank_tc_kernel<true, 1, 0, 64, true>;
  if (gg.tpc == 1) return gg.hch == 2 ? tc::fullrank_tc_kernel<false, 2, 4, 64, true> : tc::fullrank_tc_kernel<false, 1, 4, 64, true>;
  return gg.hch == 2 ? tc::fullrank_tc_kernel<false, 2, 0, 64, true> : tc::fullrank_tc_kernel<false, 1, 0, 64, true>;
}
static int geo_extra_smem(const tc::Geo& gg) { return (gg.kp == 1 ? 3 * tc::TPC * tc::TM * 4 : 0) + (gg.km ? 0 : tc::HMETA * 4); }

static int run_1(const NaisParams& p, const NaisCatalog& cat, const NaisUsers& users, int64_t poi_begin, int64_t poi_end, int k,
                 int exclude, int precision, const void* plan, size_t plan_bytes, unsigned long long* out_keys, float* out_score,
                 int32_t* out_id, float* all_scores, const float* score_in, bool merge, void* ws, size_t ws_bytes, cudaStream_t stream,
                 const GeoMixArgs* geo = nullptr) {
  if (users.n_users == 0 || poi_end <= poi_begin) return 0;
  int sms;
  int rc = check_arch(sms);
  if (rc) return rc;
  PlanLayout L;
  if (!plan_layout(p, poi_begin, poi_end, precision, L)) return NAIS_ERR_SHAPE;
  if (!plan || plan_bytes < L.total) return NAIS_ERR_WORKSPACE;
  const unsigned char* pbase = reinterpret_cast<const unsigned char*>(plan);
  const unsigned char* hdr = pbase + L.hdr;
  const size_t keys_bytes = call_keys_bytes(users.n_users, L.groups, k), scratch_bytes = call_scratch_bytes(users.n_users, L.groups, k);
  if (ws_bytes < 256 + keys_bytes + scratch_bytes + (size_t)L.g.b_chunk) return NAIS_ERR_WORKSPACE;
  unsigned char* base = reinterpret_cast<unsigned char*>(ws);
  int* pass_flags = reinterpret_cast<int*>(base);
  const size_t bimg_bytes = (ws_bytes - 256 - keys_bytes - scratch_bytes) / 256 * 256;
  unsigned char* bimg = base + 256;
  unsigned long long* keys = reinterpret_cast<unsigned long long*>(base + 256 + bimg_bytes);
  unsigned long long* scratch = reinterpret_cast<unsigned long long*>(base + 256 + bimg_bytes + keys_bytes);
  const int64_t max_chunks = (int64_t)(bimg_bytes / L.g.b_chunk);
  cudaError_t e;
  if (L.two_pass) {
    e = cudaMemsetAsync(pass_flags, 0, 8, stream);
    if (e != cudaSuccess) return (int)e;
  }
  const bool generic = (precision & NAIS_PREC_FLAG_GENERIC) != 0;
  bool use_pair = L.pair && !geo;
  if (geo) {
    if (L.g.smem_bytes + geo_extra_smem(L.g) > 227 * 1024 || (L.two_pass && L.gs.smem_bytes + geo_extra_smem(L.gs) > 227 * 1024))
      return NAIS_ERR_SHAPE;
  }
  if (use_pair) {
    static int pair_ok[64];
    int dev = 0;
    cudaGetDevice(&dev);
    int& st = pair_ok[dev & 63];
    if (st == 0) {
      cudaLaunchConfig_t cfg = {};
      cfg.gridDim = dim3(2);
      cfg.blockDim = dim3(tc::THREADS);
      cfg.dynamicSmemBytes = L.gp.smem_bytes;
      cudaLaunchAttribute at[1];
      at[0].id = cudaLaunchAttributeClusterDimension;
      at[0].val.clusterDim.x = 2;
      at[0].val.clusterDim.y = 1;
      at[0].val.clusterDim.z = 1;
      cfg.attrs = at;
      cfg.numAttrs = 1;
      MainKernel kp = pick_kernel(L.gp, false);
      int n = 0;
      const bool ok = cudaFuncSetAttribute(kp, cudaFuncAttributeMaxDynamicSharedMemorySize, L.gp.smem_bytes) == cudaSuccess &&
                      cudaOccupancyMaxActiveClusters(&n, kp, &cfg) == cudaSuccess && n >= 1;
      if (!ok) cudaGetLastError();
      st = ok ? 1 : -1;
    }
    use_pair = st == 1;
  }
  const tc::Geo& g1 = use_pair ? L.gp : L.g;
  const tc::Geo& g2 = use_pair ? L.gsp : L.gs;
  {
    dim3 grid(users.n_users, 64);
    tc::pack_users_kernel<<<grid, 256, 0, stream>>>(p, users, g1, g2, L.two_pass ? 1 : 0, hdr, bimg, max_chunks, pass_flags,
                                                   bad_index_flag());
    NAIS_COUNT_LAUNCH(1);
  }
  auto run = [&](const tc::Geo& gg, const unsigned char* pimg, int gate) -> int {
    tc::MainArgs A;
    A.p = p;
    A.cat = cat;
    A.users = users;
    A.g = gg;
    A.poi_begin = poi_begin;
    A.poi_end = poi_end;
    A.k = k;
    A.exclude = exclude;
    A.groups = gg.pair ? (L.groups + 1) / 2 * 2 : L.groups;
    A.groups_real = L.groups;
    A.n_items = (int64_t)users.n_users * (gg.pair ? A.groups / 2 : A.groups);
    A.hdr = hdr;
    A.Pimg = pimg;
    A.Bimg = bimg;
    A.part_keys = keys;
    A.all_scores = all_scores;
    A.score_in = score_in;
    A.max_chunks = max_chunks;
    A.gate = gate;
    A.pass_flags = pass_flags;
    A.geo = geo ? *geo : GeoMixArgs{};
    MainKernel kern = geo ? pick_geo_kernel(gg) : pick_kernel(gg, generic);
    const int smem = gg.smem_bytes + (geo ? geo_extra_smem(gg) : 0);
    cudaError_t e2 = cudaFuncSetAttribute(kern, cudaFuncAttributeMaxDynamicSharedMemorySize, smem);
    if (e2 != cudaSuccess) return (int)e2;
    if (gg.pair) {
      const int pairs = (int)(A.n_items < sms / 2 ? A.n_items : sms / 2);
      cudaLaunchConfig_t cfg = {};
      cfg.gridDim = dim3(2 * pairs);
      cfg.blockDim = dim3(tc::THREADS);
      cfg.dynamicSmemBytes = gg.smem_bytes;
      cfg.stream = stream;
      cudaLaunchAttribute at[1];
      at[0].id = cudaLaunchAttributeClusterDimension;
      at[0].val.clusterDim.x = 2;
      at[0].val.clusterDim.y = 1;
      at[0].val.clusterDim.z = 1;
      cfg.attrs = at;
      cfg.numAttrs = 1;
      e2 = cudaLaunchKernelEx(&cfg, kern, A);
      NAIS_COUNT_LAUNCH(1);
      return e2 == cudaSuccess ? 0 : (int)e2;
    }
    const int grid = (int)(A.n_items < sms ? A.n_items : sms);
    kern<<<grid, tc::THREADS, smem, stream>>>(A);
    NAIS_COUNT_LAUNCH(1);
    e2 = cudaGetLastError();
    return e2 == cudaSuccess ? 0 : (int)e2;
  };
  if (L.two_pass) {
    rc = run(g1, pbase + L.pimg, 1);
    if (rc) return rc;
    rc = run(g2, pbase + L.pimg2, 0);
  } else {
    rc = run(g1, pbase + L.pimg, -1);
  }
  if (rc || !merge) return rc;
  return launch_topk_merge_keys_multi(keys, scratch, (int64_t)L.groups * k, k, users.n_users, L.groups, k, out_keys, out_score, out_id,
                                      stream);
}

int fullrank_tc_run(const NaisParams& p, const NaisCatalog& cat, const NaisUsers& users, int64_t poi_begin, int64_t poi_end, int k,
                    int exclude, int precision, const void* plan, size_t plan_bytes, unsigned long long* out_keys, float* out_score,
                    int32_t* out_id, float* all_scores, void* ws, size_t ws_bytes, cudaStream_t stream, const GeoMixArgs* geo) {
  if (users.n_users == 0 || poi_end <= poi_begin) return 0;
  if (p.n_branch == 1)
    return run_1(p, cat, users, poi_begin, poi_end, k, exclude, precision, plan, plan_bytes, out_keys, out_score, out_id, all_scores,
                 nullptr, true, ws, ws_bytes, stream, geo);
  const size_t sbytes = branch_scores_bytes(p, users.n_users, poi_begin, poi_end);
  if (!plan || ws_bytes < sbytes + 512) return NAIS_ERR_WORKSPACE;
  float* sbuf = reinterpret_cast<float*>(ws);
  unsigned char* rest = reinterpret_cast<unsigned char*>(ws) + sbytes;
  size_t off = 0;
  for (int bi = 0; bi < p.n_branch; ++bi) {
    const NaisParams q = branch_view(p, bi);
    const size_t b = plan_bytes_1(q, poi_begin, poi_end, precision);
    if (!b) return NAIS_ERR_SHAPE;
    if (plan_bytes < off + b) return NAIS_ERR_WORKSPACE;
    const bool last = bi == p.n_branch - 1;
    const int rc = run_1(q, cat, users, poi_begin, poi_end, k, exclude, precision, reinterpret_cast<const unsigned char*>(plan) + off, b,
                         out_keys, out_score, out_id, last ? all_scores : sbuf, bi ? sbuf : nullptr, last, rest, ws_bytes - sbytes, stream,
                         last ? geo : nullptr);
    if (rc) return rc;
    off += b;
  }
  return 0;
}

int launch_fullrank_tc(const NaisParams& p, const NaisCatalog& cat, const NaisUsers& users, int64_t poi_begin,
                       int64_t poi_end, int k, int exclude, int precision, float* out_score, int32_t* out_id,
                       float* all_scores, void* ws, size_t ws_bytes, cudaStream_t stream) {
  if (users.n_users == 0 || poi_end <= poi_begin) return 0;
  const size_t plan_bytes = fullrank_tc_plan_bytes(p, poi_begin, poi_end, precision);
  if (!plan_bytes) return NAIS_ERR_SHAPE;
  if (ws_bytes < plan_bytes + 512) return NAIS_ERR_WORKSPACE;
  int rc = fullrank_tc_prepare(p, cat, poi_begin, poi_end, precision, ws, plan_bytes, stream);
  if (rc) return rc;
  return fullrank_tc_run(p, cat, users, poi_begin, poi_end, k, exclude, precision, ws, plan_bytes, nullptr, out_score, out_id,
                         all_scores, reinterpret_cast<unsigned char*>(ws) + plan_bytes, ws_bytes - plan_bytes, stream, nullptr);
}

}
```

Measured before the change: 12450.

## Add bound-based tile screening pass to skip candidate tiles in fullrank TC eval

Adds a two-phase screened full-rank path. A cheap high-precision-only pass computes approximate scores and per-tile error bounds. A top-k merge then gives a per-user threshold, and a compaction kernel keeps only tiles whose upper bound can reach that threshold. A list-driven main kernel then runs the full mixed-precision scoring only over the surviving tiles. This aims to cut most of the expensive correction MMA work and B traffic, but it adds extra kernels, workspace and a merge. It relies on rigorous error-bound constants to stay exact.

```diff
diff --git a/include/nais_b200.h b/include/nais_b200.h
--- a/include/nais_b200.h
+++ b/include/nais_b200.h
@@ -28,6 +28,7 @@
 #define NAIS_PREC_MASK 0xff
 #define NAIS_PREC_FLAG_GENERIC 0x100
 #define NAIS_PREC_FLAG_ONE_CTA 0x200
+#define NAIS_PREC_NO_SCREEN 0x400
 
 #define NAIS_PAIRS_AUTO 0
 #define NAIS_PAIRS_FP32 1
diff --git a/poi_recommendation_models_b200/_lib.py b/poi_recommendation_models_b200/_lib.py
--- a/poi_recommendation_models_b200/_lib.py
+++ b/poi_recommendation_models_b200/_lib.py
@@ -14,6 +14,9 @@
 PREC_FLAG_ONE_CTA = 0x200
 PRECISIONS.update({k + "_generic": v | PREC_FLAG_GENERIC for k, v in list(PRECISIONS.items()) if k != "fp32"})
 PRECISIONS.update({k + "_onecta": v | PREC_FLAG_ONE_CTA for k, v in list(PRECISIONS.items()) if k in ("tc_auto", "tc_split", "tc_mix")})
+PREC_FLAG_NO_SCREEN = 0x400
+PRECISIONS.update({k + "_noscreen": v | PREC_FLAG_NO_SCREEN for k, v in list(PRECISIONS.items())
+                   if k in ("tc_auto", "tc_mix", "tc_auto_onecta", "tc_mix_onecta")})
 PAIRS_PRECISIONS = {"auto": 0, "fp32": 1, "tc": 2}
 ERR_INDEX = -7
 
diff --git a/poi_recommendation_models_b200/csrc/nais_capi.cu b/poi_recommendation_models_b200/csrc/nais_capi.cu
--- a/poi_recommendation_models_b200/csrc/nais_capi.cu
+++ b/poi_recommendation_models_b200/csrc/nais_capi.cu
@@ -785,7 +785,7 @@
   if (work && need_reg && (!cat->region || !users->region)) return NAIS_ERR_NULL;
   if (work && p->dist_mode != NAIS_DIST_NONE && (!cat->coords || !users->coords)) return NAIS_ERR_NULL;
   const int prec = precision & NAIS_PREC_MASK;
-  if (precision & ~(NAIS_PREC_MASK | NAIS_PREC_FLAG_GENERIC | NAIS_PREC_FLAG_ONE_CTA)) return NAIS_ERR_MODE;
+  if (precision & ~(NAIS_PREC_MASK | NAIS_PREC_FLAG_GENERIC | NAIS_PREC_FLAG_ONE_CTA | NAIS_PREC_NO_SCREEN)) return NAIS_ERR_MODE;
   if (prec < NAIS_PREC_FP32 || prec > NAIS_PREC_TC_AUTO) return NAIS_ERR_MODE;
   if (prec != NAIS_PREC_FP32 && !tc_supported(*p, precision)) return NAIS_ERR_SHAPE;
   return 0;
diff --git a/poi_recommendation_models_b200/csrc/nais_tc.cu b/poi_recommendation_models_b200/csrc/nais_tc.cu
--- a/poi_recommendation_models_b200/csrc/nais_tc.cu
+++ b/poi_recommendation_models_b200/csrc/nais_tc.cu
@@ -182,7 +182,8 @@
     const float maxQ = fmaxf(fmaxf(__uint_as_float(mx[2]), __uint_as_float(mx[3])), tiny);
     const float maxB = fmaxf(maxQ * red[0], tiny);
     const float maxBe = fmaxf(fmaxf(red[1], fmaxf(fabsf(o0), fmaxf(fabsf(o1), fabsf(ob)))), tiny);
-    float sA = pow2floor(512.f / maxP), sS = pow2floor(512.f / maxQ), sB = pow2floor(512.f / maxB);
+    const float smax = 0x1p40f;
+    float sA = fminf(pow2floor(512.f / maxP), smax), sS = fminf(pow2floor(512.f / maxQ), smax), sB = fminf(pow2floor(512.f / maxB), smax);
     const float sAe = 256.f;
     float sBe = sA * sB / sAe;
     while (maxBe * sBe > 16384.f) {
@@ -412,6 +413,14 @@
   int gate;
   const int* pass_flags;
   GeoMixArgs geo;
+  const float* alpha;
+  const float4* ubc;
+  unsigned* tile_ub;
+  int n_tiles_pad;
+  const int* tile_list;
+  const int* tile_count;
+  const int2* list_items;
+  const int* list_n;
 };
 
 __device__ __forceinline__ void epi_bar() { asm volatile("bar.sync 1, 512;" ::: "memory"); }
@@ -439,13 +448,160 @@
   return v;
 }
 
+constexpr float kScreenKappa = 3.25f;
+
+__device__ __forceinline__ float screen_bound(float score, float E, float ES, float EA, float pw, float alpha, float4 c, int H,
+                                              float beta) {
+  if (!(fabsf(score) < INFINITY) || !(E >= 0x1p-60f) || !(E <= 0x1p60f)) return INFINITY;
+  const float rs = fmaf((float)H, 0.25f, 8.f) * 0x1p-24f;
+  const float eps = fmaf(alpha, c.x, c.y) + 0x1p-20f + 2.f * rs;
+  const float eta = fmaf(alpha, c.z, c.w);
+  const float x = expm1f(eps) * 1.0001f, y = expm1f(fabsf(beta) * eps) * 1.0001f;
+  const float dES = fmaf(x, EA, fmaf((1.f + x) * E, eta, 2.f * rs * EA));
+  const float B0 = fmaf(1.f + y, dES, fabsf(ES) * y) / pw;
+  return (B0 + 0x1p-19f * (fabsf(score) + B0)) * 1.0001f;
+}
+
+__global__ void screen_bounds_kernel(NaisParams p, NaisUsers users, const unsigned char* hdr, float4* ubc, unsigned* tile_ub,
+                                     int n_tiles_pad, int* list_n) {
+  const NaisBranch& br = p.branch[0];
+  const Scales* sc = reinterpret_cast<const Scales*>(hdr + 64);
+  const float* ck = reinterpret_cast<const float*>(hdr + HDR_CK);
+  const float* uu = reinterpret_cast<const float*>(hdr + HDR_U);
+  const int D = br.w_poi + br.w_reg, hid = p.hid, lanes = p.dist_mode == NAIS_DIST_LATLON ? 2 : 0, ldw = D + lanes;
+  const int u = blockIdx.x, tid = threadIdx.x, lane = tid & 31, warp = tid >> 5, nw = blockDim.x >> 5;
+  __shared__ float wbar[256];
+  __shared__ float red[4][32];
+  for (int i = tid; i < n_tiles_pad; i += blockDim.x) tile_ub[(size_t)u * n_tiles_pad + i] = 0u;
+  if (u == 0 && tid == 0) *list_n = 0;
+  for (int d = tid; d < D; d += blockDim.x) {
+    float a = fabsf(uu[d]);
+    for (int k = 0; k < hid; ++k) a += ck[k] * fabsf(__ldg(br.w1 + (size_t)k * ldw + d));
+    wbar[d] = a;
+  }
+  __syncthreads();
+  const int64_t hb = users.offsets[u];
+  const int H = (int)(users.offsets[u + 1] - hb);
+  float m_w2 = 0.f, m_w1 = 0.f, m_q2 = 0.f, m_q1 = 0.f;
+  for (int h = warp; h < H; h += nw) {
+    const int64_t e = hb + h;
+    const int it = checked_id(__ldg(users.items + e), p.item_num, nullptr);
+    const int rg = br.w_reg ? checked_id(__ldg(users.region + e), p.region_num, nullptr) : 0;
+    float w2 = 0.f, w1 = 0.f, q2 = 0.f, q1 = 0.f;
+    for (int d = lane; d < D; d += 32) {
+      const float q = fabsf(d < br.w_poi ? __ldg(br.hist_poi + (size_t)it * br.w_poi + d) : __ldg(br.hist_reg + (size_t)rg * br.w_reg + (d - br.w_poi)));
+      const float qw = q * wbar[d];
+      w2 = fmaf(qw, qw, w2);
+      w1 += qw;
+      q2 = fmaf(q, q, q2);
+      q1 += q;
+    }
+#pragma unroll
+    for (int o = 16; o > 0; o >>= 1) {
+      w2 += __shfl_xor_sync(0xffffffffu, w2, o);
+      w1 += __shfl_xor_sync(0xffffffffu, w1, o);
+      q2 += __shfl_xor_sync(0xffffffffu, q2, o);
+      q1 += __shfl_xor_sync(0xffffffffu, q1, o);
+    }
+    m_w2 = fmaxf(m_w2, w2);
+    m_w1 = fmaxf(m_w1, w1);
+    m_q2 = fmaxf(m_q2, q2);
+    m_q1 = fmaxf(m_q1, q1);
+  }
+  if (lane == 0) {
+    red[0][warp] = m_w2;
+    red[1][warp] = m_w1;
+    red[2][warp] = m_q2;
+    red[3][warp] = m_q1;
+  }
+  __syncthreads();
+  if (tid == 0) {
+    for (int w = 1; w < nw; ++w) {
+      m_w2 = fmaxf(m_w2, red[0][w]);
+      m_w1 = fmaxf(m_w1, red[1][w]);
+      m_q2 = fmaxf(m_q2, red[2][w]);
+      m_q1 = fmaxf(m_q1, red[3][w]);
+    }
+    float X = fabsf(sc->omegab) + (lanes ? fabsf(sc->omega0) + fabsf(sc->omega1) : 0.f);
+    for (int k = 0; k < hid; ++k) {
+      X += ck[k] * fabsf(__ldg(br.b1 + k));
+      if (lanes) X += ck[k] * (fabsf(__ldg(br.w1 + (size_t)k * ldw + D)) + fabsf(__ldg(br.w1 + (size_t)k * ldw + D + 1)));
+    }
+    const float rows = (float)(hid + 1), sq = sqrtf((float)D), up = 1.0001f;
+    float4 c;
+    c.x = (kScreenKappa * 0x1p-11f * sqrtf(m_w2) + rows * sq * 0x1p-16f / sc->sB) * up;
+    c.y = (0x1p-16f * m_w1 / sc->sA + 0x1p-12f * X + rows * (float)D * 0x1p-32f * sc->inv_sigma) * up;
+    c.z = (kScreenKappa * 0x1p-11f * sqrtf(m_q2) + sq * 0x1p-16f / sc->sS) * up;
+    c.w = (0x1p-16f * m_q1 / sc->sA + (float)D * 0x1p-32f * sc->inv_s) * up;
+    ubc[u] = c;
+  }
+}
+
+__global__ void candidate_norms_kernel(NaisParams p, NaisCatalog cat, int64_t poi_begin, int64_t poi_end, int64_t n_rows, float* alpha) {
+  const NaisBranch& br = p.branch[0];
+  const int64_t i = blockIdx.x * (int64_t)blockDim.x + threadIdx.x;
+  if (i >= n_rows) return;
+  const int64_t j = poi_begin + i;
+  float s = 0.f;
+  if (j < poi_end) {
+    for (int d = 0; d < br.w_poi; ++d) {
+      const float v = __ldg(br.tgt_poi + (size_t)j * br.w_poi + d);
+      s = fmaf(v, v, s);
+    }
+    const int rg = br.w_reg ? __ldg(cat.region + (j - cat.row_base)) : 0;
+    for (int d = 0; d < br.w_reg; ++d) {
+      const float v = __ldg(br.tgt_reg + (size_t)rg * br.w_reg + d);
+      s = fmaf(v, v, s);
+    }
+  }
+  alpha[i] = sqrtf(s) * 1.0001f;
+}
+
+__global__ void screen_compact_kernel(NaisUsers users, const unsigned char* hdr, int gate, int k, const unsigned long long* tau,
+                                      const unsigned* tile_ub, int n_tiles_pad, int n_tiles, int groups_real, int pair,
+                                      unsigned long long* part_keys, int* tile_list, int* tile_count, int2* list_items, int* list_n) {
+  const Scales* sc = reinterpret_cast<const Scales*>(hdr + 64);
+  const int u = blockIdx.x, tid = threadIdx.x, lane = tid & 31, warp = tid >> 5;
+  if (!user_in_pass(gate, sc->use_mix, (int)(users.offsets[u + 1] - users.offsets[u]))) return;
+  const unsigned long long kth = tau[(size_t)u * k + k - 1];
+  const unsigned thr = kth ? (unsigned)(kth >> 32) : 1u;
+  for (int i = tid; i < groups_real * k; i += blockDim.x) part_keys[(size_t)u * groups_real * k + i] = 0ull;
+  __shared__ int wcnt[32];
+  __shared__ int s_base;
+  if (tid == 0) s_base = 0;
+  __syncthreads();
+  for (int i0 = 0; i0 < n_tiles; i0 += blockDim.x) {
+    const int i = i0 + tid;
+    const bool keep = i < n_tiles && tile_ub[(size_t)u * n_tiles_pad + i] >= thr;
+    const unsigned bal = __ballot_sync(0xffffffffu, keep);
+    if (lane == 0) wcnt[warp] = __popc(bal);
+    __syncthreads();
+    int before = s_base;
+    for (int w = 0; w < warp; ++w) before += wcnt[w];
+    if (keep) tile_list[(size_t)u * n_tiles_pad + before + __popc(bal & ((1u << lane) - 1u))] = i;
+    __syncthreads();
+    if (tid == 0)
+      for (int w = 0; w < (int)(blockDim.x >> 5); ++w) s_base += wcnt[w];
+    __syncthreads();
+  }
+  if (tid == 0) {
+    const int cnt = s_base, per = pair ? 2 * TPC : TPC;
+    tile_count[u] = cnt;
+    const int n = (cnt + per - 1) / per;
+    const int b = atomicAdd(list_n, n);
+    for (int i = 0; i < n; ++i) list_items[b + i] = make_int2(u, i * (pair ? 2 : 1));
+  }
+}
+
 template <bool kSinglePart, int kHch, int kFix, int kS = 64, bool kGeo = false>
 __global__ void __launch_bounds__(THREADS, 1) fullrank_tc_kernel(const __grid_constant__ MainArgs A) {
-  constexpr bool kPair = kFix == 5 || kFix == 6;
-  constexpr bool kFastEpi = kFix == 1 || kFix == 2 || kPair;
+  constexpr bool kScr = kFix == 7 || kFix == 8;
+  constexpr bool kList = kFix == 9 || kFix == 10;
+  constexpr bool kPair = kFix == 5 || kFix == 6 || kFix == 8 || kFix == 10;
+  constexpr bool kFastEpi = kFix == 1 || kFix == 2 || kPair || kFix == 7 || kFix == 9;
   constexpr bool kD128 = kFix == 3;
   static_assert(!kGeo || kFix == 0 || kFix == 4, "geo mode lives in the run-time-shape epilogue");
-  constexpr int kCombA = kGeo ? 4 : 3, kCombT = (kGeo && !kSinglePart) ? 2 : TPC;
+  constexpr int kCombA = (kGeo || kScr) ? 4 : 3, kCombT = (kGeo && !kSinglePart) ? 2 : TPC;
   extern __shared__ __align__(128) unsigned char smem[];
   const Geo& g = A.g;
   unsigned char* sA = smem;
@@ -474,6 +630,10 @@
   if constexpr (kPair) asm volatile("mov.u32 %0, %%cluster_ctarank;" : "=r"(crank));
   const int64_t item0 = kPair ? (int64_t)(blockIdx.x >> 1) : (int64_t)blockIdx.x, item_step = kPair ? (int64_t)(gridDim.x >> 1) : (int64_t)gridDim.x;
   const int groups_it = kPair ? A.groups / 2 : A.groups;
+  auto list_tile = [&](int u, int grp, int t) {
+    const int i = grp * TPC + t;
+    return i < A.tile_count[u] ? A.tile_list[(size_t)u * A.n_tiles_pad + i] : -1;
+  };
 
   const int tid = threadIdx.x, warp = tid >> 5, lane = tid & 31;
   const Scales sc = *reinterpret_cast<const Scales*>(A.hdr + 64);
@@ -520,21 +680,34 @@
   constexpr int tpc = kSinglePart ? TPC : (kFix == 4 ? 1 : 2);
   const int hsplit = kHch == 1 ? g.hsplit : 1;
   const int64_t cb0 = chunk_base(A.users.offsets, 0, kHch, hsplit);
+  int64_t n_list = 0;
+  if constexpr (kList) n_list = *A.list_n;
 
   if (warp == EPI_WARPS + 1) {
     {
       uint32_t it_n = 0, bstep = 0;
-      for (int64_t item = item0; item < A.n_items; item += item_step) {
-        const int u = (int)(item / groups_it), grp = kPair ? 2 * (int)(item % groups_it) + (int)crank : (int)(item % groups_it);
+      for (int64_t item = item0; item < (kList ? n_list : A.n_items); item += item_step) {
+        const int u = kList ? A.list_items[item].x : (int)(item / groups_it);
+        const int grp = kList ? A.list_items[item].y + (int)crank : (kPair ? 2 * (int)(item % groups_it) + (int)crank : (int)(item % groups_it));
         if (!user_in_pass(A.gate, sc.use_mix, (int)(A.users.offsets[u + 1] - A.users.offsets[u]))) continue;
         const uint32_t it = it_n++;
         const int64_t cbu = __shfl_sync(0xffffffffu, chunk_base(A.users.offsets, u, kHch, hsplit) - cb0, 0);
         const int nchunks = __shfl_sync(0xffffffffu, user_chunks(A.users.offsets, u, kHch, cb0, A.max_chunks, hsplit), 0);
         mbar_wait(a_empty, (it & 1) ^ 1);
         if (elect_one()) {
-          mbar_expect_tx(a_full, (uint32_t)(tpc * g.a_tile));
-          for (int t = 0; t < tpc; ++t)
-            bulk_g2s(sA + (size_t)t * g.a_tile, A.Pimg + ((size_t)grp * tpc + t) * g.a_tile, (uint32_t)g.a_tile, a_full);
+          if constexpr (kScr) {
+            mbar_expect_tx(a_full, (uint32_t)(tpc * g.a_plane));
+            for (int t = 0; t < tpc; ++t)
+              bulk_g2s(sA + (size_t)t * g.a_tile, A.Pimg + ((size_t)grp * tpc + t) * g.a_tile, (uint32_t)g.a_plane, a_full);
+          } else if constexpr (kList) {
+            mbar_expect_tx(a_full, (uint32_t)(tpc * g.a_tile));
+            for (int t = 0; t < tpc; ++t)
+              bulk_g2s(sA + (size_t)t * g.a_tile, A.Pimg + (size_t)max(list_tile(u, grp, t), 0) * g.a_tile, (uint32_t)g.a_tile, a_full);
+          } else {
+            mbar_expect_tx(a_full, (uint32_t)(tpc * g.a_tile));
+            for (int t = 0; t < tpc; ++t)
+              bulk_g2s(sA + (size_t)t * g.a_tile, A.Pimg + ((size_t)grp * tpc + t) * g.a_tile, (uint32_t)g.a_tile, a_full);
+          }
         }
         __syncwarp();
         const unsigned char* src = A.Bimg + (size_t)cbu * g.b_chunk + (kPair ? (size_t)crank * (g.b_chunk / 2) : 0);
@@ -542,7 +715,8 @@
           const int kp_t = kSinglePart ? 1 : g.kp;
           for (int pp = 0; pp < kp_t; ++pp, ++bstep) {
             const int st = bstep % g.stages;
-            const uint32_t bytes = kPair ? (uint32_t)(g.b_chunk / 2) : (uint32_t)(pp == kp_t - 1 ? g.part_last_bytes : g.part_bytes);
+            uint32_t bytes = kPair ? (uint32_t)(g.b_chunk / 2) : (uint32_t)(pp == kp_t - 1 ? g.part_last_bytes : g.part_bytes);
+            if constexpr (kScr) bytes = kPair ? (uint32_t)(g.b_hi / 2) : (uint32_t)g.b_hi;
             mbar_wait(&b_empty[st], ((bstep / g.stages) & 1) ^ 1);
             if (elect_one()) {
               mbar_expect_tx(&b_full[st], bytes);
@@ -555,7 +729,7 @@
     }
   } else if (warp == EPI_WARPS) {
     if constexpr (kFastEpi) {
-      constexpr bool kMix = kFix == 2 || kFix == 6;
+      constexpr bool kMix = kFix == 2 || kFix == 6 || kScr || kList;
       constexpr uint32_t kStages = kPair ? 4u : 2u;
       constexpr uint32_t kKx = kS / 8, kK16 = kS / 16, kK32 = kS / 32;
       constexpr uint32_t kNrow = 2 * kS + 16, kALbo = TM * 16;
@@ -592,8 +766,8 @@
       const uint32_t Bx_hi = lo_of(sb0 + kKx * kBLbo, zaddr - (sb0 + kKx * kBLbo));
       const uint32_t Bx_lo = lo_of(sb0 + (2 * kKx + 1) * kBLbo, zaddr - (sb0 + (2 * kKx + 1) * kBLbo));
       uint32_t it_n = 0, cc = 0, st = 0, stph = 0;
-      for (int64_t item = item0; item < A.n_items; item += item_step) {
-        const int u = (int)(item / groups_it);
+      for (int64_t item = item0; item < (kList ? n_list : A.n_items); item += item_step) {
+        const int u = kList ? A.list_items[item].x : (int)(item / groups_it);
         if (!user_in_pass(A.gate, sc.use_mix, (int)(A.users.offsets[u + 1] - A.users.offsets[u]))) continue;
         const uint32_t it = it_n++;
         const int nchunks = __shfl_sync(0xffffffffu, user_chunks(A.users.offsets, u, kHch, cb0, A.max_chunks, hsplit), 0);
@@ -635,7 +809,9 @@
             if (elect_one()) {
 #pragma unroll
               for (int s2 = 0; s2 < (int)kK16; ++s2) mmaH(d_t, mk(ah + s2 * kAStep), mk(bh + s2 * kBStep), idN, s2 != 0);
-              if constexpr (kMix) {
+              if constexpr (kScr) {
+                mmaH(d_t, mk(E_mx + t * kExtBuf), mk(bh + kK16 * kBStep), idN, 1);
+              } else if constexpr (kMix) {
                 mmaH(d_t, mk(E_mx + t * kExtBuf), mk(bh + kK16 * kBStep), idN, 1);
                 constexpr uint32_t b8h = ((kKx + 2) * kBLbo) >> 4, b8l = ((kKx + 2 + kKx / 2) * kBLbo) >> 4;
 #pragma unroll
@@ -800,8 +976,9 @@
       if constexpr (kPair) mbar_arrive_cluster(bar, 0);
       else mbar_arrive(bar);
     };
-    for (int64_t item = item0; item < A.n_items; item += item_step) {
-      const int u = (int)(item / groups_it), grp = kPair ? 2 * (int)(item % groups_it) + (int)crank : (int)(item % groups_it);
+    for (int64_t item = item0; item < (kList ? n_list : A.n_items); item += item_step) {
+      const int u = kList ? A.list_items[item].x : (int)(item / groups_it);
+      const int grp = kList ? A.list_items[item].y + (int)crank : (kPair ? 2 * (int)(item % groups_it) + (int)crank : (int)(item % groups_it));
       const int64_t hb = A.users.offsets[u];
       const int H = (int)(A.users.offsets[u + 1] - hb);
       if (!user_in_pass(A.gate, sc.use_mix, H)) continue;
@@ -816,11 +993,17 @@
           if (g.km || kGeo) hm_cos[i] = cosf((A.cat.center_lat + hm_la[i]) * 0.017453292519943295f);
       }
       float clat[TPC], clon[TPC], ccos[TPC], sumE[TPC], sumES[TPC], sumL[TPC];
+      float sumEA[TPC];
       int64_t jid[TPC];
       bool excl[TPC];
 #pragma unroll
       for (int t = 0; t < TPC; ++t) {
-        jid[t] = t < tpc ? A.poi_begin + ((int64_t)grp * tpc + t) * TM + r : A.poi_end;
+        if constexpr (kList) {
+          const int tl = list_tile(u, grp, t);
+          jid[t] = tl >= 0 ? A.poi_begin + (int64_t)tl * TM + r : A.poi_end;
+        } else {
+          jid[t] = t < tpc ? A.poi_begin + ((int64_t)grp * tpc + t) * TM + r : A.poi_end;
+        }
         const bool v = jid[t] < A.poi_end;
         clat[t] = (v && (geo || kGeo)) ? __ldg(A.cat.coords + 2 * (jid[t] - A.cat.row_base)) : 0.f;
         clon[t] = (v && (geo || kGeo)) ? __ldg(A.cat.coords + 2 * (jid[t] - A.cat.row_base) + 1) : 0.f;
@@ -831,6 +1014,7 @@
         sumES[t] = 0.f;
         sumL[t] = 0.f;
         excl[t] = false;
+        if constexpr (kScr) sumEA[t] = 0.f;
       }
       epi_bar();
       if constexpr (kFastEpi) {
@@ -948,6 +1132,7 @@
             const float e = (hvalid && !same) ? ex2_approx(a2) : 0.f;
             sumE[t] += e;
             sumES[t] = fmaf(e, S, sumES[t]);
+            if constexpr (kScr) sumEA[t] = fmaf(e, fabsf(S), sumEA[t]);
             excl[t] = excl[t] || (hvalid && same);
           }
           fph ^= 1u;
@@ -1124,13 +1309,15 @@
           comb[((part - 1) * kCombA + 1) * kCombT * TM + t2 * TM + r] = sumES[t2];
           comb[((part - 1) * kCombA + 2) * kCombT * TM + t2 * TM + r] = excl[t2] ? 1.f : 0.f;
           if constexpr (kGeo) comb[((part - 1) * kCombA + 3) * kCombT * TM + t2 * TM + r] = sumL[t2];
+          if constexpr (kScr) comb[((part - 1) * kCombA + 3) * kCombT * TM + t2 * TM + r] = sumEA[t2];
         }
       }
       epi_bar();
       if (part == 0) {
 #pragma unroll
         for (int t2 = 0; t2 < TPC; ++t2) {
-          float E = sumE[t2], ES = sumES[t2], Lg = sumL[t2];
+          float E = sumE[t2], ES = sumES[t2], Lg = sumL[t2], EA = 0.f;
+          if constexpr (kScr) EA = sumEA[t2];
           bool ex = excl[t2];
           if (t2 < kCombT) {
 #pragma unroll
@@ -1139,7 +1326,22 @@
               ES += comb[(q * kCombA + 1) * kCombT * TM + t2 * TM + r];
               ex = ex || comb[(q * kCombA + 2) * kCombT * TM + t2 * TM + r] != 0.f;
               if constexpr (kGeo) Lg += comb[(q * kCombA + 3) * kCombT * TM + t2 * TM + r];
+              if constexpr (kScr) EA += comb[(q * kCombA + 3) * kCombT * TM + t2 * TM + r];
             }
+          }
+          if constexpr (kScr) {
+            const bool valid = jid[t2] < A.poi_end;
+            const float pw = powf(E, beta), score = ES / pw;
+            const float alpha = valid ? __ldg(A.alpha + (jid[t2] - A.poi_begin)) : 0.f;
+            const float B = screen_bound(score, E, ES, EA, pw, alpha, __ldg(A.ubc + u), H, beta);
+            const float lb = B < INFINITY ? __fsub_rd(score, B) : -INFINITY;
+            const float ub = (B < INFINITY ? __fadd_ru(score, B) : INFINITY) + 0.f;
+            const bool rankable = valid && !(A.exclude && ex);
+            kreg[t2] = rankable ? make_key(lb, (int)jid[t2]) : 0ull;
+            if (!small_k) keys[t2 * TM + r] = kreg[t2];
+            const unsigned m = __reduce_max_sync(0xffffffffu, rankable ? f2ord(ub) : 0u);
+            if (lane == 0 && m != 0u) atomicMax(A.tile_ub + (size_t)u * A.n_tiles_pad + (size_t)grp * tpc + t2, m);
+            continue;
           }
           float score = ES / powf(E, beta);
           const bool valid = jid[t2] < A.poi_end;
@@ -1217,8 +1419,9 @@
   bool two_pass;
   bool pair;
   tc::Geo gp, gsp;
+  bool screen;
   int groups, n_tiles_pad;
-  size_t hdr, pimg, pimg2, total;
+  size_t hdr, pimg, pimg2, alpha, total;
 };
 
 static bool plan_layout(const NaisParams& p, int64_t poi_begin, int64_t poi_end, int precision, PlanLayout& L) {
@@ -1260,8 +1463,38 @@
   o += al256((size_t)L.n_tiles_pad * L.g.a_tile);
   L.pimg2 = o;
   if (L.two_pass) o += al256((size_t)L.n_tiles_pad * L.g.a_tile);
+  L.screen = L.g.mix && L.g.D == 64 && L.g.hid == 64 && L.g.nrow == 144 && L.g.kp == 1 && L.g.hch == 2 && L.g.stages == 2 && !L.g.km;
+  L.alpha = o;
+  if (L.screen) o += al256((size_t)L.n_tiles_pad * tc::TM * 4);
   L.total = o;
   return true;
+}
+
+struct ScreenWs {
+  size_t ubc, tile_ub, tile_list, tile_count, items, tau, list_n, total;
+};
+static ScreenWs screen_ws(int n_users, const PlanLayout& L, int k) {
+  ScreenWs s;
+  size_t o = 0;
+  s.ubc = o;
+  o += al256((size_t)n_users * 16);
+  s.tile_ub = o;
+  o += al256((size_t)n_users * L.n_tiles_pad * 4);
+  s.tile_list = o;
+  o += al256((size_t)n_users * L.n_tiles_pad * 4);
+  s.tile_count = o;
+  o += al256((size_t)n_users * 4);
+  s.items = o;
+  o += al256((size_t)n_users * L.groups * 8);
+  s.tau = o;
+  o += al256((size_t)n_users * k * 8);
+  s.list_n = o;
+  o += 256;
+  s.total = o;
+  return s;
+}
+static inline bool screen_requested(const PlanLayout& L, int precision) {
+  return L.screen && !(precision & (NAIS_PREC_NO_SCREEN | NAIS_PREC_FLAG_GENERIC));
 }
 
 static inline size_t call_keys_bytes(int n_users, int groups, int k) { return al256((size_t)n_users * groups * k * 8); }
@@ -1306,7 +1539,8 @@
   PlanLayout L;
   if (!plan_layout(p, poi_begin, poi_end, precision, L)) return 0;
   const int64_t max_chunks = (L.g.hch == 2 ? (nnz + n_users) / 2 : nnz * L.g.hsplit) + 2;
-  return 256 + al256((size_t)max_chunks * L.g.b_chunk) + call_keys_bytes(n_users, L.groups, k) + call_scratch_bytes(n_users, L.groups, k);
+  return 256 + al256((size_t)max_chunks * L.g.b_chunk) + call_keys_bytes(n_users, L.groups, k) + call_scratch_bytes(n_users, L.groups, k) +
+         (screen_requested(L, precision) ? screen_ws(n_users, L, k).total : 0);
 }
 size_t fullrank_tc_call_workspace_bytes(const NaisParams& p, int n_users, int64_t nnz, int64_t poi_begin, int64_t poi_end, int k,
                                         int precision) {
@@ -1370,6 +1604,12 @@
     tc::pack_candidates_kernel<<<L.n_tiles_pad, 256, 0, stream>>>(p, cat, poi_begin, poi_end, L.gs, hdr, base + L.pimg2);
     NAIS_COUNT_LAUNCH(1);
   }
+  if (L.screen) {
+    const int64_t rows = (int64_t)L.n_tiles_pad * tc::TM;
+    tc::candidate_norms_kernel<<<(unsigned)((rows + 255) / 256), 256, 0, stream>>>(p, cat, poi_begin, poi_end, rows,
+                                                                                   reinterpret_cast<float*>(base + L.alpha));
+    NAIS_COUNT_LAUNCH(1);
+  }
   e = cudaGetLastError();
   return e == cudaSuccess ? 0 : (int)e;
 }
@@ -1415,6 +1655,12 @@
   return gg.hch == 2 ? tc::fullrank_tc_kernel<false, 2, 0, 64, true> : tc::fullrank_tc_kernel<false, 1, 0, 64, true>;
 }
 static int geo_extra_smem(const tc::Geo& gg) { return (gg.kp == 1 ? 3 * tc::TPC * tc::TM * 4 : 0) + (gg.km ? 0 : tc::HMETA * 4); }
+
+static MainKernel pick_screen_kernel(const tc::Geo& gg, bool list) {
+  if (gg.pair) return list ? tc::fullrank_tc_kernel<true, 2, 10, 64> : tc::fullrank_tc_kernel<true, 2, 8, 64>;
+  return list ? tc::fullrank_tc_kernel<true, 2, 9, 64> : tc::fullrank_tc_kernel<true, 2, 7, 64>;
+}
+static int screen_extra_smem() { return 3 * tc::TPC * tc::TM * 4; }
 
 static int run_1(const NaisParams& p, const NaisCatalog& cat, const NaisUsers& users, int64_t poi_begin, int64_t poi_end, int k,
                  int exclude, int precision, const void* plan, size_t plan_bytes, unsigned long long* out_keys, float* out_score,
@@ -1430,13 +1676,17 @@
   const unsigned char* pbase = reinterpret_cast<const unsigned char*>(plan);
   const unsigned char* hdr = pbase + L.hdr;
   const size_t keys_bytes = call_keys_bytes(users.n_users, L.groups, k), scratch_bytes = call_scratch_bytes(users.n_users, L.groups, k);
-  if (ws_bytes < 256 + keys_bytes + scratch_bytes + (size_t)L.g.b_chunk) return NAIS_ERR_WORKSPACE;
+  const bool screen = screen_requested(L, precision) && !geo && !all_scores && !score_in;
+  const ScreenWs sw = screen_ws(users.n_users, L, k);
+  const size_t screen_bytes = screen ? sw.total : 0;
+  if (ws_bytes < 256 + keys_bytes + scratch_bytes + screen_bytes + (size_t)L.g.b_chunk) return NAIS_ERR_WORKSPACE;
   unsigned char* base = reinterpret_cast<unsigned char*>(ws);
   int* pass_flags = reinterpret_cast<int*>(base);
-  const size_t bimg_bytes = (ws_bytes - 256 - keys_bytes - scratch_bytes) / 256 * 256;
+  const size_t bimg_bytes = (ws_bytes - 256 - keys_bytes - scratch_bytes - screen_bytes) / 256 * 256;
   unsigned char* bimg = base + 256;
   unsigned long long* keys = reinterpret_cast<unsigned long long*>(base + 256 + bimg_bytes);
   unsigned long long* scratch = reinterpret_cast<unsigned long long*>(base + 256 + bimg_bytes + keys_bytes);
+  unsigned char* sbase = base + 256 + bimg_bytes + keys_bytes + scratch_bytes;
   const int64_t max_chunks = (int64_t)(bimg_bytes / L.g.b_chunk);
   cudaError_t e;
   if (L.two_pass) {
@@ -1483,8 +1733,8 @@
                                                    bad_index_flag());
     NAIS_COUNT_LAUNCH(1);
   }
-  auto run = [&](const tc::Geo& gg, const unsigned char* pimg, int gate) -> int {
-    tc::MainArgs A;
+  auto run = [&](const tc::Geo& gg, const unsigned char* pimg, int gate, int mode = 0) -> int {
+    tc::MainArgs A = {};
     A.p = p;
     A.cat = cat;
     A.users = users;
@@ -1506,8 +1756,16 @@
     A.gate = gate;
     A.pass_flags = pass_flags;
     A.geo = geo ? *geo : GeoMixArgs{};
-    MainKernel kern = geo ? pick_geo_kernel(gg) : pick_kernel(gg, generic);
-    const int smem = gg.smem_bytes + (geo ? geo_extra_smem(gg) : 0);
+    A.alpha = reinterpret_cast<const float*>(pbase + L.alpha);
+    A.ubc = reinterpret_cast<const float4*>(sbase + sw.ubc);
+    A.tile_ub = reinterpret_cast<unsigned*>(sbase + sw.tile_ub);
+    A.n_tiles_pad = L.n_tiles_pad;
+    A.tile_list = reinterpret_cast<const int*>(sbase + sw.tile_list);
+    A.tile_count = reinterpret_cast<const int*>(sbase + sw.tile_count);
+    A.list_items = reinterpret_cast<const int2*>(sbase + sw.items);
+    A.list_n = reinterpret_cast<const int*>(sbase + sw.list_n);
+    MainKernel kern = mode ? pick_screen_kernel(gg, mode == 2) : (geo ? pick_geo_kernel(gg) : pick_kernel(gg, generic));
+    const int smem = gg.smem_bytes + (geo ? geo_extra_smem(gg) : 0) + (mode == 1 ? screen_extra_smem() : 0);
     cudaError_t e2 = cudaFuncSetAttribute(kern, cudaFuncAttributeMaxDynamicSharedMemorySize, smem);
     if (e2 != cudaSuccess) return (int)e2;
     if (gg.pair) {
@@ -1515,7 +1773,7 @@
       cudaLaunchConfig_t cfg = {};
       cfg.gridDim = dim3(2 * pairs);
       cfg.blockDim = dim3(tc::THREADS);
-      cfg.dynamicSmemBytes = gg.smem_bytes;
+      cfg.dynamicSmemBytes = smem;
       cfg.stream = stream;
       cudaLaunchAttribute at[1];
       at[0].id = cudaLaunchAttributeClusterDimension;
@@ -1534,7 +1792,29 @@
     e2 = cudaGetLastError();
     return e2 == cudaSuccess ? 0 : (int)e2;
   };
-  if (L.two_pass) {
+  const int mix_gate = L.two_pass ? 1 : -1;
+  if (screen) {
+    tc::screen_bounds_kernel<<<users.n_users, 256, 0, stream>>>(p, users, hdr, reinterpret_cast<float4*>(sbase + sw.ubc),
+                                                                reinterpret_cast<unsigned*>(sbase + sw.tile_ub), L.n_tiles_pad,
+                                                                reinterpret_cast<int*>(sbase + sw.list_n));
+    NAIS_COUNT_LAUNCH(1);
+    rc = run(g1, pbase + L.pimg, mix_gate, 1);
+    if (rc) return rc;
+    unsigned long long* tau = reinterpret_cast<unsigned long long*>(sbase + sw.tau);
+    rc = launch_topk_merge_keys_multi(keys, scratch, (int64_t)L.groups * k, k, users.n_users, L.groups, k, tau, nullptr, nullptr, stream);
+    if (rc) return rc;
+    const int n_tiles = (int)((poi_end - poi_begin + tc::TM - 1) / tc::TM);
+    tc::screen_compact_kernel<<<users.n_users, 256, 0, stream>>>(
+        users, hdr, mix_gate, k, tau, reinterpret_cast<const unsigned*>(sbase + sw.tile_ub), L.n_tiles_pad, n_tiles, L.groups,
+        g1.pair, keys, reinterpret_cast<int*>(sbase + sw.tile_list), reinterpret_cast<int*>(sbase + sw.tile_count),
+        reinterpret_cast<int2*>(sbase + sw.items), reinterpret_cast<int*>(sbase + sw.list_n));
+    NAIS_COUNT_LAUNCH(1);
+    e = cudaGetLastError();
+    if (e != cudaSuccess) return (int)e;
+    rc = run(g1, pbase + L.pimg, mix_gate, 2);
+    if (rc) return rc;
+    if (L.two_pass) rc = run(g2, pbase + L.pimg2, 0);
+  } else if (L.two_pass) {
     rc = run(g1, pbase + L.pimg, 1);
     if (rc) return rc;
     rc = run(g2, pbase + L.pimg2, 0);
```

Measured after the change: 11850, median of 6. 4.8% lower.
